# adolliou/euispice_coreg

Measured on AMD Instinct MI355X. Metric: lag-points/sec (whole node) on 2048² grid, 60×60 CRVAL sweep; argmax-shift match, higher is better.
Workload: dtype f64; 1 GPU; headline: Carrington 'fa' 2048x2048 grid lon(200,300) lat(-20,20), 60x60 CRVAL lags arange(-30,30,1) arcsec, small 2048^2 HRIEUV-like, ref 3072^2 FSI-like, order 2, solar_r 1.004; lag_points=3600, parallelism=single GPU, no collective, resident=True, sweeps_in_flight=2, small_stored_f32=True, use_lds=True

## Files before the change

### euispice_coreg_amd/_lib.py

```python
from __future__ import annotations

import ctypes as C
import os

import numpy as np

_HERE = os.path.dirname(os.path.abspath(__file__))
LIB_PATH = os.environ.get("COREG_HIP_LIB", os.path.join(_HERE, "libcoreg_hip.so"))

COREG_OK = 0
COREG_EINVAL, COREG_EHIP, COREG_ESTATE, COREG_ENOTIMPL, COREG_ENOMEM = -1, -2, -3, -4, -5
COREG_F32, COREG_F64 = 0, 1
PROJ_TAN, PROJ_CAR = 0, 1
METHOD_CORRELATION, METHOD_RESIDUS = 0, 1
CDELT_INTENDED, CDELT_REFERENCE = 0, 1


class CoregError(RuntimeError):
    def __init__(self, code, msg):
        super().__init__(f"libcoreg_hip error {code}: {msg}")
        self.code = code


class Wcs2d(C.Structure):
# ... 20 lines not shown
                ("lat0", C.c_double), ("lat1", C.c_double), ("n_lat", C.c_int32),
                ("lat_cos", C.POINTER(C.c_float)), ("lat_sin", C.POINTER(C.c_float))]


class Stats(C.Structure):
    _fields_ = [("sweep_kernel_ms", C.c_double), ("precompute_ms", C.c_double), ("total_gpu_ms", C.c_double),
                ("n_lags", C.c_int64), ("n_grid_points", C.c_int64), ("n_active_points", C.c_int64),
                ("n_sweep_launches", C.c_int64), ("small_is_f32", C.c_int32), ("used_lds", C.c_int32)]


class FitsPixels(C.Structure):
    _fields_ = [("data", C.c_void_p), ("bitpix", C.c_int32), ("reserved", C.c_int32), ("bscale", C.c_double),
                ("bzero", C.c_double)]


class FitsTiled(C.Structure):
    _fields_ = [("heap", C.c_void_p), ("heap_bytes", C.c_int64), ("tile_offset", C.c_void_p), ("tile_nbytes", C.c_void_p),
                ("n_tiles", C.c_int32), ("zbitpix", C.c_int32), ("naxis1", C.c_int32), ("naxis2", C.c_int32),
                ("ztile1", C.c_int32), ("ztile2", C.c_int32), ("blocksize", C.c_int32), ("bytepix", C.c_int32),
                ("quantize", C.c_int32), ("dither0", C.c_int32), ("has_blank", C.c_int32), ("blank", C.c_int32),
                ("zscale", C.c_void_p), ("zzero", C.c_void_p), ("zscale0", C.c_double), ("zzero0", C.c_double),
                ("bscale", C.c_double), ("bzero", C.c_double)]


def _is_tiled(img):
    return hasattr(img, "tile_nbytes") and hasattr(img, "ztile") and getattr(img, "on_gpu", False)


def _fits_tiled(ci):
    off = np.ascontiguousarray(ci.tile_offset, dtype=np.int64)
    nb = np.ascontiguousarray(ci.tile_nbytes, dtype=np.int32)
    keep = [off, nb, ci._heap]
    zs = zz = None
    if ci.zscale is not None and ci.zzero is not None:
        zs = np.ascontiguousarray(ci.zscale, dtype=np.float64)
        zz = np.ascontiguousarray(ci.zzero, dtype=np.float64)
        keep += [zs, zz]
    t = FitsTiled(ci._heap.ctypes.data, int(ci._heap.size), off.ctypes.data, nb.ctypes.data, int(ci.n_tiles), int(ci.zbitpix),
                  int(ci.shape[1]), int(ci.shape[0]), int(ci.ztile[0]), int(ci.ztile[1]), int(ci.blocksize), int(ci.bytepix),
                  int(ci.quantize), int(ci.dither0), int(bool(ci.has_blank)), int(ci.blank),
                  zs.ctypes.data if zs is not None else None, zz.ctypes.data if zz is not None else None,
                  float(ci.zscale0), float(ci.zzero0), float(ci.bscale), float(ci.bzero))
    return t, keep


def decode_tiled_host(ci, out):
    t, keep = _fits_tiled(ci)
    status = np.zeros(ci.n_tiles, dtype=np.int32)
    rc = load_library().coreg_decode_tiled_host(C.byref(t), out.ctypes.data, COREG_F32 if out.dtype == np.float32 else COREG_F64,
                                                status.ctypes.data)
    if rc != COREG_OK:
        raise CoregError(rc, "coreg_decode_tiled_host: bad arguments (unsupported tiling / codec parameters)")
    del keep
    return status


def encode_tiled_host(pixels, tile, bytepix=4, blocksize=32, quantize=0, dither0=1, scale=1.0):
    a = np.ascontiguousarray(pixels)
    if a.ndim != 2:
        raise ValueError("image must be 2-D")
    ny, nx = a.shape
    tx, ty = int(tile[0]), int(tile[1])
    nt = (-(-nx // tx)) * (-(-ny // ty))
    if a.dtype == np.float32:
        dt = COREG_F32
    elif a.dtype == np.float64:
        dt = COREG_F64
    elif a.dtype == np.int32:
        dt = 2
    else:
        raise TypeError("pixels must be float32, float64 or int32 (stored integers)")
    is_float = dt != 2
    n_blocks = nt * (-(-(tx * ty) // int(blocksize)) + 1)
    cap = a.size * int(bytepix) + n_blocks + 8 * nt + 64
    heap = np.empty(cap, dtype=np.uint8)
    nbytes = np.zeros(nt, dtype=np.int32)
    offs = np.zeros(nt, dtype=np.int64)
    zs = np.zeros(nt, dtype=np.float64) if is_float else None
    zz = np.zeros(nt, dtype=np.float64) if is_float else None
    used = C.c_longlong(0)
    rc = load_library().coreg_encode_tiled_host(a.ctypes.data, dt, ny, nx, tx, ty, int(bytepix), int(blocksize), int(quantize),
                                                int(dither0), float(scale), heap.ctypes.data, cap, nbytes.ctypes.data,
                                                offs.ctypes.data, zs.ctypes.data if is_float else None,
                                                zz.ctypes.data if is_float else None, C.byref(used))
    if rc != COREG_OK:
        raise CoregError(rc, "coreg_encode_tiled_host: bad arguments, or a tile's range does not fit 32-bit integers at "
                             "this scale")
    return heap[:used.value].copy(), nbytes, offs, zs, zz


def _is_raw(img):
    return hasattr(img, "bitpix") and hasattr(img, "ptr")


def _fits_pixels(raw) -> FitsPixels:
    if len(raw.shape) != 2:
        raise ValueError("image must be 2-D")
    return FitsPixels(raw.ptr, int(raw.bitpix), 0, float(raw.bscale), float(raw.bzero))


_P = C.c_void_p
_WP = C.POINTER(Wcs2d)
SYMBOLS = [
    ("coreg_version", C.c_char_p, []),
    ("coreg_create", C.c_int, [C.POINTER(_P), C.c_int]),
    ("coreg_destroy", None, [_P]),
    ("coreg_last_error", C.c_char_p, [_P]),
    ("coreg_set_stream", C.c_int, [_P, _P]),
    ("coreg_synchronize", C.c_int, [_P]),
    ("coreg_set_small", C.c_int, [_P, _P, C.c_int32, C.c_int32]),
    ("coreg_set_small_f32", C.c_int, [_P, _P, C.c_int32, C.c_int32]),
    ("coreg_set_small_fits", C.c_int, [_P, C.POINTER(FitsPixels), C.c_int32, C.c_int32]),
    ("coreg_prepare_reference_carrington_fits", C.c_int,
     [_P, C.POINTER(FitsPixels), C.c_int32, C.c_int32, _WP, C.POINTER(CarrGrid), C.c_double, C.c_int]),
    ("coreg_prepare_reference_helioprojective_fits", C.c_int,
     [_P, C.POINTER(FitsPixels), C.c_int32, C.c_int32, _WP, _WP, C.c_int]),
    ("coreg_set_small_tiled", C.c_int, [_P, C.POINTER(FitsTiled)]),
    ("coreg_prepare_reference_carrington_tiled", C.c_int,
     [_P, C.POINTER(FitsTiled), _WP, C.POINTER(CarrGrid), C.c_double, C.c_int]),
    ("coreg_prepare_reference_helioprojective_tiled", C.c_int, [_P, C.POINTER(FitsTiled), _WP, _WP, C.c_int]),
    ("coreg_decode_tiled_host", C.c_int, [C.POINTER(FitsTiled), _P, C.c_int, _P]),
    ("coreg_encode_tiled_host", C.c_int, [_P, C.c_int, C.c_int, C.c_int, C.c_int, C.c_int, C.c_int, C.c_int, C.c_int, C.c_int,
                                          C.c_double, _P, C.c_longlong, _P, _P, _P, _P, C.POINTER(C.c_longlong)]),
    ("coreg_threshold_small", C.c_int, [_P, C.c_int, C.c_double, C.c_int, C.c_double, C.POINTER(C.c_longlong)]),
    ("coreg_set_reference_on_grid", C.c_int, [_P, _P, C.c_int, C.c_int32, C.c_int32]),
    ("coreg_prepare_reference_carrington", C.c_int,
     [_P, _P, C.c_int32, C.c_int32, _WP, C.POINTER(CarrGrid), C.c_double, C.c_int]),
    ("coreg_prepare_reference_helioprojective", C.c_int, [_P, _P, C.c_int32, C.c_int32, _WP, _WP, C.c_int]),
    ("coreg_prepare_reference_carrington_f32", C.c_int,
     [_P, _P, C.c_int32, C.c_int32, _WP, C.POINTER(CarrGrid), C.c_double, C.c_int]),
    ("coreg_prepare_reference_helioprojective_f32", C.c_int, [_P, _P, C.c_int32, C.c_int32, _WP, _WP, C.c_int]),
    ("coreg_set_small_from_device", C.c_int, [_P, _P, C.c_int, C.c_int32, C.c_int32]),
    ("coreg_prepare_reference_carrington_from_device", C.c_int,
     [_P, _P, C.c_int, C.c_int32, C.c_int32, _WP, C.POINTER(CarrGrid), C.c_double, C.c_int]),
    ("coreg_prepare_reference_helioprojective_from_device", C.c_int,
     [_P, _P, C.c_int, C.c_int32, C.c_int32, _WP, _WP, C.c_int]),
    ("coreg_get_reference_on_grid", C.c_int, [_P, _P, C.c_int]),
    ("coreg_resample_carrington", C.c_int, [_P, _WP, C.POINTER(CarrGrid), C.c_double, C.c_int, _P]),
    ("coreg_resample_helioprojective", C.c_int, [_P, _WP, _WP, C.c_int, _P]),
    ("coreg_resample_helioprojective_f64", C.c_int, [_P, _WP, _WP, C.c_int, _P]),
    ("coreg_sweep_carrington", C.c_int,
     [_P, _WP, C.POINTER(CarrGrid), C.c_double, C.POINTER(Lags), C.c_int, C.c_int, C.c_int, C.c_int64, C.c_int64, _P,
      C.c_int]),
    ("coreg_sweep_helioprojective", C.c_int,
     [_P, _WP, _WP, C.POINTER(Lags), C.c_int, C.c_int, C.c_int, C.c_int64, C.c_int64, _P, C.c_int]),
    ("coreg_sums_size", C.c_int, [_P, C.POINTER(C.c_int64)]),
    ("coreg_copy_sums", C.c_int, [_P, _P, C.c_int]),
    ("coreg_finalize_sums", C.c_int, [_P, _P, C.c_int, _P, C.c_int]),
    ("coreg_get_pivots", C.c_int, [_P, C.POINTER(C.c_double)]),
    ("coreg_set_pivots", C.c_int, [_P, C.POINTER(C.c_double)]),
    ("coreg_last_stats", C.c_int, [_P, C.POINTER(Stats)]),
    ("coreg_last_visit_counts", C.c_int, [_P, C.POINTER(C.c_int64)]),
    ("coreg_last_tap_fix", C.c_int, [_P, C.POINTER(C.c_int64)]),
    ("coreg_set_option", C.c_int, [_P, C.c_char_p, C.c_int64]),
    ("coreg_shift_header", C.c_int,
     [_WP, C.c_double, C.c_double, C.c_double, C.c_double, C.c_double, C.c_int, _WP]),
    ("coreg_homography", C.c_int, [_WP, _WP, C.POINTER(C.c_double)]),
    ("coreg_lag_homography", C.c_int,
     [_WP, _WP, C.POINTER(Lags), C.POINTER(C.c_int32), C.c_int, C.POINTER(C.c_double)]),
    ("coreg_carrington_origin", C.c_int, [_WP, C.POINTER(C.c_double), C.POINTER(C.c_double)]),
    ("coreg_car_map", C.c_int, [_WP, _WP, C.c_int64, _P, _P, _P, _P]),
    ("coreg_wcslib_pixel_to_pixel", C.c_int, [_WP, _WP, C.c_int64, _P, _P, _P, _P, _P, _P]),
    ("coreg_car_tile_margin", C.c_int, [_WP, _WP, C.c_int32, C.c_double, C.POINTER(C.c_double)]),
    ("coreg_nansum_planes_be", C.c_int, [_P, C.c_int32, C.c_int64, _P, C.c_int32, _P]),
    ("coreg_fit_gaussian2d", C.c_int,
     [C.c_int32, _P, _P, _P, _P, _P, _P, C.c_int32, C.c_double, C.c_double, C.c_double, C.c_int32, _P,
      C.POINTER(C.c_int32), C.POINTER(C.c_int32)]),
    ("coreg_set_context_frames", C.c_int, [_P, C.c_int32, C.c_int32, C.c_int32, C.c_int, _WP, C.POINTER(_P)]),
    ("coreg_context_frame_from_small", C.c_int, [_P, C.c_int32]),
    ("coreg_sweep_context", C.c_int,
     [_P, _WP, _WP, C.POINTER(C.c_int32), C.POINTER(Lags), C.c_int, C.c_int, C.c_int, C.c_int, C.c_double, C.c_int,
      C.c_double, C.c_int64, C.c_int64, _P, C.c_int]),
    ("coreg_context_lag_headers", C.c_int,
     [_WP, _WP, C.c_double, C.c_double, C.c_double, C.c_double, C.c_double, C.c_int, _WP, _WP, _WP]),
    ("coreg_device_count", C.c_int, []),
    ("coreg_physical_device_count", C.c_int, []),
    ("coreg_multi_create", C.c_int, [C.POINTER(_P), C.c_int, C.POINTER(C.c_int)]),
    ("coreg_multi_destroy", None, [_P]),
    ("coreg_multi_size", C.c_int, [_P]),
    ("coreg_multi_handle", _P, [_P, C.c_int]),
    ("coreg_multi_last_error", C.c_char_p, [_P]),
    ("coreg_multi_collective", C.c_char_p, [_P]),
    ("coreg_multi_rccl_status", C.c_char_p, [_P]),
    ("coreg_multi_last_mode", C.c_int, [_P]),
    ("coreg_multi_set_option", C.c_int, [_P, C.c_char_p, C.c_int64]),
    ("coreg_multi_set_small", C.c_int, [_P, _P, C.c_int, C.c_int32, C.c_int32]),
    ("coreg_multi_set_small_fits", C.c_int, [_P, C.POINTER(FitsPixels), C.c_int32, C.c_int32]),
    ("coreg_multi_prepare_reference_carrington_fits", C.c_int,
     [_P, C.POINTER(FitsPixels), C.c_int32, C.c_int32, _WP, C.POINTER(CarrGrid), C.c_double, C.c_int]),
    ("coreg_multi_prepare_reference_helioprojective_fits", C.c_int,
     [_P, C.POINTER(FitsPixels), C.c_int32, C.c_int32, _WP, _WP, C.c_int]),
    ("coreg_multi_set_small_tiled", C.c_int, [_P, C.POINTER(FitsTiled)]),
    ("coreg_multi_prepare_reference_carrington_tiled", C.c_int,
     [_P, C.POINTER(FitsTiled), _WP, C.POINTER(CarrGrid), C.c_double, C.c_int]),
    ("coreg_multi_prepare_reference_helioprojective_tiled", C.c_int, [_P, C.POINTER(FitsTiled), _WP, _WP, C.c_int]),
    ("coreg_multi_threshold_small", C.c_int, [_P, C.c_int, C.c_double, C.c_int, C.c_double, C.POINTER(C.c_longlong)]),
    ("coreg_multi_set_reference_on_grid", C.c_int, [_P, _P, C.c_int, C.c_int32, C.c_int32]),
    ("coreg_multi_prepare_reference_carrington", C.c_int,
     [_P, _P, C.c_int, C.c_int32, C.c_int32, _WP, C.POINTER(CarrGrid), C.c_double, C.c_int]),
    ("coreg_multi_prepare_reference_helioprojective", C.c_int, [_P, _P, C.c_int, C.c_int32, C.c_int32, _WP, _WP, C.c_int]),
    ("coreg_multi_sweep_carrington", C.c_int,
     [_P, _WP, C.POINTER(CarrGrid), C.c_double, C.POINTER(Lags), C.c_int, C.c_int, C.c_int, _P]),
    ("coreg_multi_sweep_helioprojective", C.c_int, [_P, _WP, _WP, C.POINTER(Lags), C.c_int, C.c_int, C.c_int, _P]),
    ("coreg_multi_last_stats", C.c_int, [_P, C.c_int, C.POINTER(Stats)]),
    ("coreg_multi_plan", C.c_int,
     [C.c_int32, C.c_int32, C.c_int64, C.c_int32, C.c_int32, C.POINTER(C.c_int32), C.POINTER(C.c_int32),
      C.POINTER(C.c_int32), C.POINTER(C.c_int32)]),
]

_lib = None


def _preload_torch_hip_runtime():
    import importlib.util
    import sys
    if "torch" in sys.modules or os.environ.get("COREG_NO_TORCH_PRELOAD", "0") == "1":
        return
    try:
        spec = importlib.util.find_spec("torch")
    except (ImportError, ValueError):
        return
    if spec is None or not spec.submodule_search_locations:
        return
    libdir = os.path.join(list(spec.submodule_search_locations)[0], "lib")
    cand = os.path.join(libdir, "libamdhip64.so")
    if os.path.exists(cand):
        try:
            C.CDLL(cand, mode=C.RTLD_GLOBAL)
        except OSError:
            return
        rccl = os.path.join(libdir, "librccl.so")
        if os.path.exists(rccl):
            os.environ.setdefault("COREG_RCCL_LIB", rccl)


def load_library():
    global _lib
    if _lib is not None:
        return _lib
    _preload_torch_hip_runtime()
    if not os.path.exists(LIB_PATH):
        raise ImportError(
            f"{LIB_PATH} not found: the HIP extension has not been built. "
            "Run `python -c 'import __graft_entry__ as g; g.build()'` at the repo root "
            "(hipcc --offload-arch=gfx950). There is no CPU fallback.")
    lib = C.CDLL(LIB_PATH)
    for name, restype, argtypes in SYMBOLS:
        fn = getattr(lib, name)
        fn.restype = restype
        fn.argtypes = argtypes
    _lib = lib
    return lib


_UNIT_TO_DEG = {"deg": 1.0, "arcsec": 1.0 / 3600.0, "arcmin": 1.0 / 60.0, "rad": 180.0 / np.pi, "mas": 1.0 / 3.6e6}


def unit_to_deg(unit) -> float:
    u = str(unit).strip()
    if u not in _UNIT_TO_DEG:
        raise ValueError(f"unsupported CUNIT {unit!r}")
    return _UNIT_TO_DEG[u]


def wcs_from_header(hdr, carrington=False) -> Wcs2d:
    w = Wcs2d()
    if "ZNAXIS1" in hdr:
        w.naxis1, w.naxis2 = int(hdr["ZNAXIS1"]), int(hdr["ZNAXIS2"])
    else:
        w.naxis1, w.naxis2 = int(hdr.get("NAXIS1", 0)), int(hdr.get("NAXIS2", 0))
    w.crpix1, w.crpix2 = float(hdr["CRPIX1"]), float(hdr["CRPIX2"])
    w.crval1, w.crval2 = float(hdr["CRVAL1"]), float(hdr["CRVAL2"])
    w.cdelt1, w.cdelt2 = float(hdr["CDELT1"]), float(hdr["CDELT2"])
    w.pc1_1, w.pc1_2 = float(hdr.get("PC1_1", 1.0)), float(hdr.get("PC1_2", 0.0))
    w.pc2_1, w.pc2_2 = float(hdr.get("PC2_1", 0.0)), float(hdr.get("PC2_2", 1.0))
    w.crota = float(hdr["CROTA"] if "CROTA" in hdr else hdr.get("CROTA2", 0.0))
    u1 = hdr.get("CUNIT1", "deg")
    if str(u1).strip() != str(hdr.get("CUNIT2", u1)).strip():
        raise ValueError("CUNIT1 and CUNIT2 must be equal")
    w.unit_to_deg = unit_to_deg(u1)
    if str(hdr.get("CTYPE1", "")).strip().upper().endswith("-CAR"):
        w.proj = PROJ_CAR
        w.lonpole = float(hdr["LONPOLE"]) if "LONPOLE" in hdr else float("nan")
    else:
        w.proj = PROJ_TAN
        w.lonpole = float(hdr.get("LONPOLE", 180.0))
    w.latpole = float(hdr["LATPOLE"]) if "LATPOLE" in hdr else float("nan")
    if carrington:
        w.dsun_obs = float(hdr["DSUN_OBS"])
        w.crln_obs = float(hdr["CRLN_OBS"])
        w.crlt_obs = float(hdr["CRLT_OBS"])
    return w


def _dptr(a):
    return a.ctypes.data_as(C.POINTER(C.c_double))


class LagSet:

    def __init__(self, crval1, crval2, cdelt1, cdelt2, crota):
        def arr(v):
            return np.ascontiguousarray(np.atleast_1d(np.asarray([0.0] if v is None else v, dtype=np.float64)))

        self.arrays = [arr(crval1), arr(crval2), arr(cdelt1), arr(cdelt2), arr(crota)]
        a = self.arrays
# ... 176 lines not shown

    def get_reference_on_grid(self, shape, dtype):
        out = np.empty(shape, dtype=dtype)
        dt = COREG_F32 if out.dtype == np.float32 else COREG_F64
        self._chk(self._lib.coreg_get_reference_on_grid(self._h, out.ctypes.data, dt))
        return out

    def resample_carrington(self, hdr, grid: Grid, solar_r, order=2):
        w = wcs_from_header(hdr, carrington=True)
        out = np.empty((grid.n_lat, grid.n_lon), dtype=np.float64)
        self._chk(self._lib.coreg_resample_carrington(self._h, C.byref(w), C.byref(grid.c), float(solar_r), int(order),
                                                      out.ctypes.data))
        return out

    def resample_helioprojective(self, hdr_target, hdr, order=2, dtype=np.float32):
        wt, w = wcs_from_header(hdr_target), wcs_from_header(hdr)
        out = np.empty((wt.naxis2, wt.naxis1), dtype=dtype)
        fn = self._lib.coreg_resample_helioprojective if out.dtype == np.float32 else \
            self._lib.coreg_resample_helioprojective_f64
        self._chk(fn(self._h, C.byref(wt), C.byref(w), int(order), out.ctypes.data))
        return out

    def sweep_carrington(self, hdr_small, grid: Grid, solar_r, lags: LagSet, order=2, method=METHOD_CORRELATION,
                         cdelt_semantics=CDELT_INTENDED, lag_begin=0, lag_end=None, out_dev_ptr=None):
        lag_end = lags.size if lag_end is None else int(lag_end)
        w = wcs_from_header(hdr_small, carrington=True)
        if out_dev_ptr is None:
            out = np.empty(lag_end - lag_begin, dtype=np.float64)
            ptr, on_dev = out.ctypes.data, 0
        else:
            out, ptr, on_dev = None, int(out_dev_ptr), 1
        self._chk(self._lib.coreg_sweep_carrington(self._h, C.byref(w), C.byref(grid.c), float(solar_r),
                                                   C.byref(lags.c), int(order), int(method), int(cdelt_semantics),
                                                   int(lag_begin), lag_end, _P(ptr), on_dev))
        return out

    def sweep_helioprojective(self, hdr_target, hdr_small, lags: LagSet, order=2, method=METHOD_CORRELATION,
                              cdelt_semantics=CDELT_INTENDED, lag_begin=0, lag_end=None, out_dev_ptr=None):
        lag_end = lags.size if lag_end is None else int(lag_end)
        wt, w = wcs_from_header(hdr_target), wcs_from_header(hdr_small)
        if out_dev_ptr is None:
            out = np.empty(lag_end - lag_begin, dtype=np.float64)
            ptr, on_dev = out.ctypes.data, 0
        else:
            out, ptr, on_dev = None, int(out_dev_ptr), 1
        self._chk(self._lib.coreg_sweep_helioprojective(self._h, C.byref(wt), C.byref(w), C.byref(lags.c), int(order),
                                                        int(method), int(cdelt_semantics), int(lag_begin), lag_end,
                                                        _P(ptr), on_dev))
        return out

    def set_context_frames(self, frames, headers, dtype=None):
        frames = list(frames)
        if len(frames) != len(headers) or not frames:
            raise ValueError("one header per frame, at least one frame")

        def stored(f):
            if _is_tiled(f):
                return np.float32 if int(f.zbitpix) == -32 else np.float64
            if _is_raw(f):
                return np.float32 if int(f.bitpix) == -32 else np.float64
            return np.float32 if np.asarray(f).dtype == np.float32 else np.float64
        if dtype is None:
            dtype = np.float32 if all(stored(f) == np.float32 for f in frames) else np.float64
        dtype = np.dtype(dtype)
        shape = tuple(frames[0].shape)
        if any(tuple(f.shape) != shape for f in frames) or len(shape) != 2:
            raise ValueError("all frames must be 2-D images of one shape")
        hdrs = (Wcs2d * len(frames))(*[wcs_from_header(hh) for hh in headers])
        host = []
        ptrs = (_P * len(frames))()
        for k, f in enumerate(frames):
            if _is_tiled(f) or _is_raw(f):
                continue
            a = np.ascontiguousarray(f, dtype=dtype)
            host.append(a)
            ptrs[k] = a.ctypes.data
        self._chk(self._lib.coreg_set_context_frames(self._h, len(frames), shape[0], shape[1],
                                                     COREG_F32 if dtype == np.float32 else COREG_F64, hdrs, ptrs))
        for k, f in enumerate(frames):
            if _is_tiled(f) or _is_raw(f):
                self.set_small(f)
                self._chk(self._lib.coreg_context_frame_from_small(self._h, k))
        self._context_frames = (len(frames), shape, dtype)

    def sweep_context(self, hdr_target, hdr_small, col_frame, lags: LagSet, order=2, method=METHOD_CORRELATION,
                      cdelt_semantics=CDELT_INTENDED, vmin=None, vmax=None, lag_begin=0, lag_end=None, out_dev_ptr=None):
        lag_end = lags.size if lag_end is None else int(lag_end)
        wt, w = wcs_from_header(hdr_target), wcs_from_header(hdr_small)
        cf = np.ascontiguousarray(col_frame, dtype=np.int32)
        if cf.size != w.naxis1:
            raise ValueError("col_frame needs one entry per raster column")
        if out_dev_ptr is None:
            out = np.empty(lag_end - lag_begin, dtype=np.float64)
            ptr, on_dev = out.ctypes.data, 0
        else:
            out, ptr, on_dev = None, int(out_dev_ptr), 1
        self._chk(self._lib.coreg_sweep_context(
            self._h, C.byref(wt), C.byref(w), cf.ctypes.data_as(C.POINTER(C.c_int32)), C.byref(lags.c), int(order),
            int(method), int(cdelt_semantics), int(vmin is not None), float(0.0 if vmin is None else vmin),
            int(vmax is not None), float(0.0 if vmax is None else vmax), int(lag_begin), lag_end, _P(ptr), on_dev))
        return out

    def set_point_shard(self, rank, world):
        self.set_option("shard_world", int(world))
        self.set_option("shard_rank", int(rank))

    def sums_size(self) -> int:
        n = C.c_int64(0)
        self._chk(self._lib.coreg_sums_size(self._h, C.byref(n)))
        return int(n.value)

    def copy_sums(self, dst_ptr=None):
        if dst_ptr is not None:
            self._chk(self._lib.coreg_copy_sums(self._h, _P(int(dst_ptr)), 1))
            return None
        out = np.empty(self.sums_size(), dtype=np.float64)
        self._chk(self._lib.coreg_copy_sums(self._h, out.ctypes.data, 0))
        return out

    def finalize_sums(self, sums, n_out, out_dev_ptr=None):
        if isinstance(sums, np.ndarray):
            sums = np.ascontiguousarray(sums, dtype=np.float64)
            sptr, s_dev = sums.ctypes.data, 0
        else:
            sptr, s_dev = int(sums), 1
        if out_dev_ptr is None:
            out = np.empty(int(n_out), dtype=np.float64)
            self._chk(self._lib.coreg_finalize_sums(self._h, _P(sptr), s_dev, out.ctypes.data, 0))
            return out
        self._chk(self._lib.coreg_finalize_sums(self._h, _P(sptr), s_dev, _P(int(out_dev_ptr)), 1))
        return None

    def get_pivots(self):
        p = (C.c_double * 2)()
        self._chk(self._lib.coreg_get_pivots(self._h, p))
        return float(p[0]), float(p[1])

    def set_pivots(self, pivot_ref, pivot_small):
        p = (C.c_double * 2)(float(pivot_ref), float(pivot_small))
        self._chk(self._lib.coreg_set_pivots(self._h, p))

    def last_stats(self) -> dict:
        s = Stats()
        self._chk(self._lib.coreg_last_stats(self._h, C.byref(s)))
        return {f: getattr(s, f) for f, _ in Stats._fields_}

    def last_visit_counts(self) -> dict:
        c = (C.c_int64 * 6)()
        self._chk(self._lib.coreg_last_visit_counts(self._h, c))
        return {"visits": c[0], "lds": c[1], "interior": c[2], "all_finite": c[3], "refined_lag_points": c[4],
                "flagged_not_refined": c[5]}


    def last_tap_fix(self) -> dict:
        c = (C.c_int64 * 3)()
        self._chk(self._lib.coreg_last_tap_fix(self._h, c))
        return {"samples": c[0], "lag_points": c[1], "overflow": bool(c[2])}


class _HandleView(CoregHandle):

    def __init__(self, lib, ptr):
        self._lib = lib
        self._h = _P(ptr)
        self.reference_tag = None

    def close(self):
        self._h = None


MULTI_MODES = {0: "none", 1: "blocks", 2: "slices", 3: "points", 4: "combos"}


def device_count() -> int:
    return max(0, int(load_library().coreg_device_count()))


def physical_device_count() -> int:
    return max(0, int(load_library().coreg_physical_device_count()))


def multi_plan(n_crval1, n_crval2, n_inner, world, per_combo_launch=True):
    mode, gc, g1, g2 = C.c_int32(), C.c_int32(), C.c_int32(), C.c_int32()
    rc = load_library().coreg_multi_plan(int(n_crval1), int(n_crval2), int(n_inner), int(world), int(per_combo_launch),
                                         C.byref(mode), C.byref(gc), C.byref(g1), C.byref(g2))
    if rc != COREG_OK:
        raise CoregError(rc, "coreg_multi_plan: bad arguments")
    return MULTI_MODES[mode.value], gc.value, g1.value, g2.value


class MultiHandle:

    def __init__(self, n_devices=0, device_ids=None):
        self._lib = load_library()
        self._m = _P()
        ids = None
        if device_ids is not None:
            ids = (C.c_int * len(device_ids))(*[int(d) for d in device_ids])
            n_devices = len(device_ids)
        rc = self._lib.coreg_multi_create(C.byref(self._m), int(n_devices), ids)
        if rc != COREG_OK:
            self._m = None
            raise CoregError(rc, "coreg_multi_create failed (no HIP device visible?)")
        self.reference_tag = None
        self.size = int(self._lib.coreg_multi_size(self._m))
        self.primary = _HandleView(self._lib, self._lib.coreg_multi_handle(self._m, 0))

    def close(self):
        if getattr(self, "_m", None):
            self.primary.close()
            self._lib.coreg_multi_destroy(self._m)
            self._m = None

    def __del__(self):
        try:
            self.close()
        except Exception:
            pass

    def __enter__(self):
        return self

    def __exit__(self, *exc):
        self.close()

    def _chk(self, rc):
        if rc != COREG_OK:
            raise CoregError(rc, self._lib.coreg_multi_last_error(self._m).decode("utf-8", "replace"))

    @property
    def collective(self) -> str:
        return self._lib.coreg_multi_collective(self._m).decode()

    @property
    def rccl_status(self) -> str:
        return self._lib.coreg_multi_rccl_status(self._m).decode()

    @property
    def last_mode(self) -> str:
        return MULTI_MODES[int(self._lib.coreg_multi_last_mode(self._m))]

    def handle(self, k) -> CoregHandle:
        ptr = self._lib.coreg_multi_handle(self._m, int(k))
        if not ptr:
            raise IndexError(k)
        return _HandleView(self._lib, ptr)

    def set_option(self, name, value):
        self._chk(self._lib.coreg_multi_set_option(self._m, name.encode(), int(value)))

    def synchronize(self):
        for k in range(self.size):
            self.handle(k).synchronize()

    @staticmethod
    def _pixels(img):
        img = np.asarray(img)
        if img.ndim != 2:
            raise ValueError("image must be 2-D")
        if img.dtype == np.float32:
            return np.ascontiguousarray(img), COREG_F32
        return np.ascontiguousarray(img, dtype=np.float64), COREG_F64

    def set_small(self, img):
        if _is_tiled(img):
            t, keep = _fits_tiled(img)
            self._chk(self._lib.coreg_multi_set_small_tiled(self._m, C.byref(t)))
            return
        if _is_raw(img):
            px = _fits_pixels(img)
            self._chk(self._lib.coreg_multi_set_small_fits(self._m, C.byref(px), img.shape[0], img.shape[1]))
            return
        img, dt = self._pixels(img)
        self._chk(self._lib.coreg_multi_set_small(self._m, img.ctypes.data, dt, img.shape[0], img.shape[1]))

    def threshold_small(self, vmin=None, vmax=None) -> int:
        n = C.c_longlong(0)
        self._chk(self._lib.coreg_multi_threshold_small(self._m, int(vmin is not None), float(vmin or 0.0),
                                                        int(vmax is not None), float(vmax or 0.0), C.byref(n)))
        return int(n.value)

    def set_reference_on_grid(self, ref):
        ref = np.ascontiguousarray(ref)
        if ref.ndim != 2 or ref.dtype not in (np.float32, np.float64):
            raise ValueError("reference on grid must be a 2-D float32/float64 array")
        self.reference_tag = None
        self._chk(self._lib.coreg_multi_set_reference_on_grid(
            self._m, ref.ctypes.data, COREG_F32 if ref.dtype == np.float32 else COREG_F64, ref.shape[0], ref.shape[1]))

    def prepare_reference_carrington(self, large, hdr_large, grid: Grid, solar_r, order=2):
        w = wcs_from_header(hdr_large, carrington=True)
        self.reference_tag = None
        if _is_tiled(large):
            t, keep = _fits_tiled(large)
            self._chk(self._lib.coreg_multi_prepare_reference_carrington_tiled(self._m, C.byref(t), C.byref(w),
                                                                               C.byref(grid.c), float(solar_r), int(order)))
            return
        if _is_raw(large):
            px = _fits_pixels(large)
            self._chk(self._lib.coreg_multi_prepare_reference_carrington_fits(
                self._m, C.byref(px), large.shape[0], large.shape[1], C.byref(w), C.byref(grid.c), float(solar_r),
                int(order)))
            return
        large, dt = self._pixels(large)
        self._chk(self._lib.coreg_multi_prepare_reference_carrington(
            self._m, large.ctypes.data, dt, large.shape[0], large.shape[1], C.byref(w), C.byref(grid.c), float(solar_r),
# ... 234 lines not shown
```

### euispice_coreg_amd/csrc/abi_host.hpp

```cpp
#pragma once
extern "C" {
int coreg_shift_header(const coreg_wcs2d* ref, double d_crval1, double d_crval2, double d_cdelt1, double d_cdelt2,
                       double d_crota, int cdelt_semantics, coreg_wcs2d* out) {
    if (!ref || !out) return COREG_EINVAL;
    return shift_header(*ref, d_crval1, d_crval2, d_cdelt1, d_cdelt2, d_crota, cdelt_semantics, out);
}

int coreg_car_map(const coreg_wcs2d* from, const coreg_wcs2d* to, int64_t n, const double* px, const double* py,
                  double* ox, double* oy) {
    if (!from || !to || n < 0 || (n > 0 && (!px || !py || !ox || !oy))) return COREG_EINVAL;
    if (from->proj != COREG_PROJ_CAR || to->proj != COREG_PROJ_CAR) return COREG_EINVAL;
    CarMapHost m;
    if (m.init(*from, *to)) return 1;
    for (int64_t i = 0; i < n; ++i) m.apply(px[i], py[i], &ox[i], &oy[i]);
    return COREG_OK;
}

int coreg_last_visit_counts(coreg_handle* h, int64_t* counts6) {
    int64_t* counts5 = counts6;
    if (!h || !counts5) return COREG_EINVAL;
    RETCHK(bind_device(h));
    HIPCHK(hipStreamSynchronize(h->stream));
    long long info[8] = {0, 0, 0, 0, 0, 0, 0, 0};
    if (h->tile_info.p) HIPCHK(hipMemcpy(info, h->tile_info.p, 7 * sizeof(long long), hipMemcpyDeviceToHost));
    for (int k = 0; k < 4; ++k) counts5[k] = info[3 + k];
    long long refined[2] = {0, 0};
    if (h->counters.p) HIPCHK(hipMemcpy(refined, h->counters.p, sizeof(refined), hipMemcpyDeviceToHost));
    counts5[4] = refined[0];
    counts6[5] = refined[1];
    return COREG_OK;
}

int coreg_last_tap_fix(coreg_handle* h, int64_t* counts3) {
    if (!h || !counts3) return COREG_EINVAL;
    for (int k = 0; k < 3; ++k) counts3[k] = h->tap_last[k];
    return COREG_OK;
}

int coreg_car_tile_margin(const coreg_wcs2d* hdr_target, const coreg_wcs2d* hdr_shifted, int32_t tile_w,
                          double tile_abs_lat_rad, double* margin_px) {
    if (!hdr_target || !hdr_shifted || !margin_px || tile_w < 1 || tile_w > kTilePts) return COREG_EINVAL;
    if (hdr_target->proj != COREG_PROJ_CAR || hdr_shifted->proj != COREG_PROJ_CAR) return COREG_EINVAL;
    CarMapHost m;
    if (m.init(*hdr_target, *hdr_shifted)) return 1;
    *margin_px = car_tile_margin(car_box_c(*hdr_target, *hdr_shifted, tile_w), tile_abs_lat_rad + car_pole_sep(m.r));
    return COREG_OK;
}

int coreg_homography(const coreg_wcs2d* from, const coreg_wcs2d* to, double* h9) {
    if (!from || !to || !h9) return COREG_EINVAL;
    if (from->proj != COREG_PROJ_TAN || to->proj != COREG_PROJ_TAN) return COREG_ENOTIMPL;
    homography(*from, *to, h9);
    return COREG_OK;
}

int coreg_lag_homography(const coreg_wcs2d* hdr_target, const coreg_wcs2d* hdr_small, const coreg_lags* lags,
                         const int32_t idx[5], int cdelt_semantics, double* h9) {
    if (!hdr_target || !hdr_small || !lags || !idx || !h9) return COREG_EINVAL;
    if (hdr_target->proj != COREG_PROJ_TAN || hdr_small->proj != COREG_PROJ_TAN) return COREG_ENOTIMPL;
    if (idx[0] < 0 || idx[0] >= lags->n_crval1 || idx[1] < 0 || idx[1] >= lags->n_crval2 || idx[2] < 0 ||
        idx[2] >= lags->n_cdelt1 || idx[3] < 0 || idx[3] >= lags->n_cdelt2 || idx[4] < 0 || idx[4] >= lags->n_crota)
        return COREG_EINVAL;
    coreg_wcs2d hc;
    if (shift_header(*hdr_small, 0.0, 0.0, lags->cdelt1[idx[2]], lags->cdelt2[idx[3]], lags->crota[idx[4]],
                     cdelt_semantics, &hc))
        return 1;
    HomographyFamily fam;
    fam.init(*hdr_target, *hdr_small, lags->crval1, lags->n_crval1, lags->crval2, lags->n_crval2);
    fam.get(HomographyFamily::combo(hc), idx[0], idx[1], h9);
    return COREG_OK;
}

int coreg_wcslib_pixel_to_pixel(const coreg_wcs2d* from, const coreg_wcs2d* to, int64_t n, const double* px,
                                const double* py, double* ox, double* oy, double* lng, double* lat) {
    if (!from || !to || n < 0 || (n > 0 && (!px || !py || !ox || !oy))) return COREG_EINVAL;
    if (from->proj == COREG_PROJ_CAR && to->proj == COREG_PROJ_CAR) {
        WcslibCar a, b;
        a.init(*from);
        b.init(*to);
        if (!a.valid || !b.valid) return COREG_EINVAL;
        for (int64_t i = 0; i < n; ++i) {
            double l, t;
            a.p2s(px[i], py[i], &l, &t);
            if (lng) lng[i] = l;
            if (lat) lat[i] = t;
            b.s2p(l, t, &ox[i], &oy[i]);
        }
        return COREG_OK;
    }
    if (from->proj != COREG_PROJ_TAN || to->proj != COREG_PROJ_TAN) return COREG_ENOTIMPL;
    WcslibTan a, b;
    a.init(*from);
    b.init(*to);
    for (int64_t i = 0; i < n; ++i) {
        double l, t;
        a.p2s(px[i], py[i], &l, &t);
        if (lng) lng[i] = l;
        if (lat) lat[i] = t;
        b.s2p(ang2pipi_deg(l), ang2pipi_deg(t), &ox[i], &oy[i]);
    }
    return COREG_OK;
}

int coreg_carrington_origin(const coreg_wcs2d* hdr, double* x0, double* y0) {
    if (!hdr || !x0 || !y0) return COREG_EINVAL;
    carr_origin(*hdr, x0, y0);
    return COREG_OK;
}

int coreg_nansum_planes_be(const void* cube, int32_t bitpix, int64_t n_pixels, const int64_t* plane_index, int32_t n_sel,
                           double* out) {
    if (!cube || !out || n_pixels < 0 || n_sel < 0 || (n_sel > 0 && !plane_index) || (bitpix != -32 && bitpix != -64))
        return COREG_EINVAL;
    for (int k = 0; k < n_sel; ++k)
        if (plane_index[k] < 0) return COREG_EINVAL;
    auto work = [&](int64_t lo, int64_t hi) {
        for (int64_t p = lo; p < hi; ++p) out[p] = 0.0;
        for (int k = 0; k < n_sel; ++k) {
            if (bitpix == -32) {
                const uint32_t* src = (const uint32_t*)cube + (size_t)plane_index[k] * (size_t)n_pixels;
                for (int64_t p = lo; p < hi; ++p) {
                    const uint32_t u = __builtin_bswap32(src[p]);
                    float f;
                    std::memcpy(&f, &u, sizeof(f));
                    const double v = (double)f;
                    out[p] += (v != v) ? 0.0 : v;
                }
            } else {
                const uint64_t* src = (const uint64_t*)cube + (size_t)plane_index[k] * (size_t)n_pixels;
                for (int64_t p = lo; p < hi; ++p) {
                    const uint64_t u = __builtin_bswap64(src[p]);
                    double v;
                    std::memcpy(&v, &u, sizeof(v));
                    out[p] += (v != v) ? 0.0 : v;
                }
            }
        }
    };
    parallel_for(n_pixels, (unsigned)std::min<int64_t>(12, n_pixels * std::max(n_sel, 1) / (1 << 18)), 0, work);
    return COREG_OK;
}

int coreg_fit_gaussian2d(int32_t m, const double* x, const double* y, const double* z, const double* p0,
                         const double* lb, const double* ub, int32_t jac, double ftol, double xtol, double gtol,
                         int32_t max_nfev, double* popt, int32_t* nfev, int32_t* status) {
    if (!x || !y || !z || !p0 || !lb || !ub || !popt || !status || m < 1 || m > coregfit::MMAX) return COREG_EINVAL;
    coregfit::Problem P{m, x, y, z};
    int n = 0;
    const int st = coregfit::fit(P, p0, lb, ub, jac != 0, ftol > 0 ? ftol : 1e-8, xtol > 0 ? xtol : 1e-8,
                                 gtol > 0 ? gtol : 1e-8, max_nfev, popt, &n, nullptr);
    if (st == -2) return COREG_EINVAL;
    if (nfev) *nfev = n;
    *status = st;
    return COREG_OK;
}

}
```

### euispice_coreg_amd/csrc/abi_sweeps.hpp

```cpp
#pragma once
namespace {
struct SweepCall {
    const coreg_lags* lags = nullptr;
    LagDims d;
    int order = 0, method = 0, sem = 0;
    long long lag_begin = 0, lag_end = 0, n_out = 0;
    double* corr_out = nullptr;
    int out_on_device = 0;
    double* out_dev = nullptr;
    long long row() const { return (long long)d.n2 * d.nc; }
    int i1_lo() const { return (int)(lag_begin / row()); }
    int i1_hi() const { return (int)((lag_end - 1) / row()); }
};

template <typename OwnChecks>
int open_sweep(coreg_handle* h, ComboRange combo, OwnChecks own_checks, const coreg_lags* lags, int order, int method,
               int sem, int64_t lag_begin, int64_t lag_end, int grid_w, int grid_h, const char* grid_what,
               double* corr_out, int out_on_device, SweepCall* call) {
    if (method != COREG_METHOD_CORRELATION && method != COREG_METHOD_RESIDUS)
        return fail(h, COREG_ENOTIMPL, "method must be COREG_METHOD_CORRELATION or COREG_METHOD_RESIDUS");
    RETCHK(check_order(h, order));
    RETCHK(own_checks());
    RETCHK(check_lags(h, lags, &call->d, lag_begin, lag_end, combo));
    RETCHK(bind_device_nowait(h));
    if (h->ref.p && (h->gW != grid_w || h->gH != grid_h))
        return fail(h, COREG_EINVAL, std::string("reference-on-grid shape differs from ") + grid_what);
    call->lags = lags;
    call->order = order;
    call->method = method;
    call->sem = sem;
    call->lag_begin = lag_begin;
    call->lag_end = lag_end;
    call->n_out = lag_end - lag_begin;
    call->corr_out = corr_out;
    call->out_on_device = out_on_device;
    return begin_sweep(h, call->n_out, corr_out, out_on_device, &call->out_dev);
}

int close_sweep(coreg_handle* h, const SweepCall& call) {
    return end_sweep(h, call.n_out, call.corr_out, call.out_on_device, call.out_dev);
}

int close_empty_sweep(coreg_handle* h, const SweepCall& call) {
    RETCHK(fill_nan(h, call.out_dev, call.n_out));
    return close_sweep(h, call);
}

template <typename MapAt>
Geometry local_geometry(const coreg_wcs2d& target, const SweepCall& call, MapAt at) {
    const coreg_lags& l = *call.lags;
    int e1[3], e2[3];
    extreme_lags(l.crval1, call.d.n1, e1);
    extreme_lags(l.crval2, call.d.n2, e2);
    const double v1 = l.crval1[e1[1]], v2 = l.crval2[e2[1]];
    const double s1 = lag_step(l.crval1, call.d.n1), s2 = lag_step(l.crval2, call.d.n2);
    const double u = target.naxis1 * 0.5, v = target.naxis2 * 0.5;
    double x0, y0, xi, yi, xj, yj, xa, ya, xb, yb;
    Geometry g;
    if (!at(v1, v2, u, v, &x0, &y0) || !at(v1, v2, u + 1, v, &xi, &yi) || !at(v1, v2, u, v + 1, &xj, &yj) ||
        !at(v1 + s1, v2, u, v, &xa, &ya) || !at(v1, v2 + s2, u, v, &xb, &yb))
        return g;
    g.dx_di = xi - x0;
    g.dy_di = yi - y0;
    g.dx_dj = xj - x0;
    g.dy_dj = yj - y0;
    g.ax = xa - x0;
    g.ay = ya - y0;
    g.bx = xb - x0;
    g.by = yb - y0;
    return g;
}

Plan plan_sweep(coreg_handle* h, const Geometry& geo, const SweepCall& call) {
    return choose_plan(h, geo, call.i1_hi() - call.i1_lo() + 1, call.d.n2, h->opt_use_lds ? lds_window_elems(h) : (1LL << 40));
}

bool combo_slots(const SweepCall& call, const coreg_wcs2d& small, const Plan& plan, long long c, coreg_wcs2d* hc,
                 SlotList* slots) {
    const long long first = (call.lag_begin - c + call.d.nc - 1) / call.d.nc;
    if (first * call.d.nc + c >= call.lag_end) return false;
    int i3, i4, i5;
    call.d.inner(c, &i3, &i4, &i5);
    if (shift_header(small, 0.0, 0.0, call.lags->cdelt1[i3], call.lags->cdelt2[i4], call.lags->crota[i5], call.sem, hc))
        return false;
    build_slots(call.d, c, call.lag_begin, call.lag_end, plan.sw, plan.sh, slots);
    return slots->n_batches > 0;
}

template <int MODE>
int precompute(coreg_handle* h, const PrecomputeArgs& pa, int n_tiles, int n_groups, int n_batches, bool launch = true) {
    if (launch) RETCHK(launch_precompute<MODE>(h, pa, n_tiles, n_groups, n_batches));
    h->last_precompute = [pa, n_tiles, n_groups, n_batches](coreg_handle* hh) {
        return launch_precompute<MODE>(hh, pa, n_tiles, n_groups, n_batches);
    };
    return COREG_OK;
}

int finalize_pending(coreg_handle* h, const coreg_handle::PendingFinalize& pf, long long* refine_count, double* out_dev,
                     FinalizeArgs* f) {
    *f = FinalizeArgs{};
    RETCHK(fill_refine(h, &f->refine, pf.refine.mode, pf.refine.order, pf.refine.lane_params, pf.refine.car_inv,
                       pf.n_slots));
    f->refine.enabled = pf.refine.enabled;
    f->refine_count = refine_count;
    f->partials = h->sums.as<double>() + pf.slot_off;
    f->n_groups = 1;
    f->n_slots = pf.n_slots;
    f->part_stride = h->sums_slots;
    f->out_index = h->fin_outidx.as<long long>() + pf.slot_off;
    f->lag_begin = pf.lag_begin;
    f->out = out_dev;
    f->residus = pf.residus;
    f->n_required = (long long)h->gW * h->gH;
    hipLaunchKernelGGL(k_finalize, dim3((unsigned)((pf.n_slots + kFinSlots - 1) / kFinSlots)),
                       dim3(kFinSlots * kFinLanes), 0, h->stream, *f);
    return COREG_OK;
}
}

extern "C" {
int coreg_sweep_carrington(coreg_handle* h, const coreg_wcs2d* hdr_small, const coreg_carr_grid* grid, double solar_r,
                           const coreg_lags* lags, int order, int method, int cdelt_semantics, int64_t lag_begin,
                           int64_t lag_end, double* corr_out, int out_on_device) {
    if (!h) return COREG_EINVAL;
    const ComboRange combo = take_combo_range(h);
    trace("sweep_carrington: enter");
    if (!hdr_small || !grid) return fail(h, COREG_EINVAL, "sweep_carrington: null header/grid");
    auto own_checks = [&] {
        RETCHK(check_wcs(h, hdr_small, true));
        RETCHK(check_grid(h, grid));
        if (!std::isfinite(solar_r) || !(solar_r > 0.0)) return fail(h, COREG_EINVAL, "solar_r must be positive");
        return COREG_OK;
    };
    SweepCall call;
    RETCHK(open_sweep(h, combo, own_checks, lags, order, method, cdelt_semantics, lag_begin, lag_end, grid->n_lon,
                      grid->n_lat, "the Carrington grid", corr_out, out_on_device, &call));
    if (call.n_out == 0) return close_sweep(h, call);
    const LagDims& d = call.d;

    CarrDev cd;
    std::memset(&cd, 0, sizeof(cd));
    RETCHK(upload_carr_tables(h, *grid, *hdr_small, &cd));

    Geometry geo;
    {
        const CarrCommon c0 = carr_common(*hdr_small, solar_r);
        const int ic = grid->n_lon / 2, jc = grid->n_lat / 2;
        double a0, a1, b0, b1, c0x, c0y;
        carr_term_host(h->tabs, c0, ic, jc, &a0, &a1);
        carr_term_host(h->tabs, c0, std::min(ic + 1, grid->n_lon - 1), jc, &b0, &b1);
        carr_term_host(h->tabs, c0, ic, std::min(jc + 1, grid->n_lat - 1), &c0x, &c0y);
        geo.dx_di = b0 - a0;
        geo.dy_di = b1 - a1;
        geo.dx_dj = c0x - a0;
        geo.dy_dj = c0y - a1;
        const double s1 = lag_step(lags->crval1, d.n1), s2 = lag_step(lags->crval2, d.n2);
        geo.ax = c0.cr * s1 / hdr_small->cdelt1;
        geo.ay = c0.sr * s1 / hdr_small->cdelt2;
        geo.bx = c0.sr * s2 / hdr_small->cdelt1;
        geo.by = c0.cr * s2 / hdr_small->cdelt2;
    }
    const Plan plan = plan_sweep(h, geo, call);
    PrecomputeArgs pa;
    int n_tiles;
    RETCHK(setup_precompute(h, plan, method, &pa, &n_tiles));

    struct Launch {
        size_t slot_off;
        int n_batches;
        CarrCommon cc;
        double f0lo, f0hi, f1lo, f1hi;
    };
    std::vector<Launch> launches;
    std::vector<double> params;
    std::vector<long long> outidx;
    SlotList slots;
    for (long long c = 0; c < d.nc; ++c) {
        coreg_wcs2d hc;
        if (!combo_slots(call, *hdr_small, plan, c, &hc, &slots)) continue;
        const size_t ns = slots.i1.size();
        Launch L;
        L.slot_off = outidx.size();
        L.n_batches = slots.n_batches;
        L.cc = carr_common(hc, solar_r);
        const size_t pbase = params.size();
        params.resize(pbase + 2 * ns);
        double x0min = 1e300, x0max = -1e300, y0min = 1e300, y0max = -1e300;
        const double roll = hc.crota * kDeg2Rad;
        const double rc = std::cos(roll), rs = std::sin(roll);
        const double nan = std::numeric_limits<double>::quiet_NaN();
        for (size_t s = 0; s < ns; ++s) {
            if (slots.outidx[s] < 0) {
                params[pbase + s] = nan;
                params[pbase + ns + s] = nan;
                continue;
            }
            const double v1 = hdr_small->crval1 + lags->crval1[slots.i1[s]];
            const double v2 = hdr_small->crval2 + lags->crval2[slots.i2[s]];
            const double dx = rc * v1 + rs * v2;
            const double dy = -rs * v1 + rc * v2;
            const double x0 = (hc.crpix1 - 1) - dx / hc.cdelt1;
            const double y0 = (hc.crpix2 - 1) - dy / hc.cdelt2;
            params[pbase + s] = x0;
            params[pbase + ns + s] = y0;
            x0min = std::min(x0min, x0);
            x0max = std::max(x0max, x0);
            y0min = std::min(y0min, y0);
            y0max = std::max(y0max, y0);
        }
        outidx.insert(outidx.end(), slots.outidx.begin(), slots.outidx.end());
        L.f0lo = -x0max;
        L.f0hi = (double)(h->sW - 1) - x0min;
        L.f1lo = -y0max;
        L.f1hi = (double)(h->sH - 1) - y0min;
        launches.push_back(L);
    }
    if (launches.empty()) return close_empty_sweep(h, call);
    RETCHK(upload_plan(h, params, outidx, call.out_dev, call.n_out));
    RETCHK(prepare_sharded(h, outidx.size(), call.n_out, lag_begin));
    for (const Launch& L : launches) {
        set_carr_common(&cd, L.cc);
        pa.carr = cd;
        pa.f0lo = L.f0lo;
        pa.f0hi = L.f0hi;
        pa.f1lo = L.f1lo;
        pa.f1hi = L.f1hi;
        {
            const double dm1 = L.cc.dist - 1.0;
            pa.tile_skip = (h->opt_tile_skip && dm1 > 0.0) ? 1 : 0;
            const double per_rad = pa.tile_skip ? (1.0 / dm1 + 1.0 / (dm1 * dm1)) * kRad2Deg * 3600.0 : 0.0;
            pa.lip_x = per_rad / std::fabs(L.cc.cdelt1) * (1.0 + 1e-9);
            pa.lip_y = per_rad / std::fabs(L.cc.cdelt2) * (1.0 + 1e-9);
            pa.dlon = grid->n_lon > 1 ? (std::fabs(grid->lon1 - grid->lon0) / (grid->n_lon - 1) * 1.001 + 1e-4) * kDeg2Rad : 0.0;
            pa.dlat = grid->n_lat > 1 ? (std::fabs(grid->lat1 - grid->lat0) / (grid->n_lat - 1) * 1.001 + 1e-4) * kDeg2Rad : 0.0;
        }
        RETCHK(precompute<MODE_TRANSLATE>(h, pa, n_tiles, pick_groups(h, L.n_batches, n_tiles), L.n_batches));
        RETCHK(launch_sweep(h, MODE_TRANSLATE, order, method, h->lane_params.as<double>() + 2 * L.slot_off,
                            h->out_index.as<long long>() + L.slot_off, L.n_batches, n_tiles, lag_begin, call.out_dev,
// ... 521 lines not shown
```

### euispice_coreg_amd/csrc/host_plan.hpp

```cpp
#pragma once
namespace {
template <typename Fn>
void parallel_for(long long n, unsigned max_threads, long long grain, Fn fn) {
    if (n <= 0) return;
    const long long nt_max = std::max<long long>(1, std::min(max_threads, std::thread::hardware_concurrency()));
    if (grain <= 0) grain = (n + nt_max - 1) / nt_max;
    const long long nt = std::min(nt_max, (n + grain - 1) / grain);
    if (nt <= 1) {
        fn(0ll, n);
        return;
    }
    std::atomic<long long> next(0);
    auto worker = [&] {
        for (long long lo = next.fetch_add(grain); lo < n; lo = next.fetch_add(grain)) fn(lo, std::min(n, lo + grain));
    };
    std::vector<std::thread> th;
    for (long long t = 1; t < nt; ++t) th.emplace_back(worker);
    worker();
    for (auto& x : th) x.join();
}

struct LagDims {
    int n1, n2, n3, n4, n5;
    long long nc;
    long long c0;
    long long total() const { return (long long)n1 * n2 * nc; }
    void inner(long long c, int* i3, int* i4, int* i5) const {
        const long long g = c + c0;
        *i5 = (int)(g % n5);
        *i4 = (int)((g / n5) % n4);
        *i3 = (int)(g / ((long long)n5 * n4));
    }
};

struct ComboRange {
    long long begin = 0, end = 0;
};
ComboRange take_combo_range(coreg_handle* h) {
    ComboRange r;
    r.begin = h->opt_combo_begin;
    r.end = h->opt_combo_end;
    h->opt_combo_begin = h->opt_combo_end = 0;
    return r;
}
int check_lags(coreg_handle* h, const coreg_lags* l, LagDims* d, int64_t begin, int64_t end, ComboRange combo = ComboRange()) {
    if (!l || !l->crval1 || !l->crval2 || !l->cdelt1 || !l->cdelt2 || !l->crota)
        return fail(h, COREG_EINVAL, "lags: null array");
    if (l->n_crval1 < 1 || l->n_crval2 < 1 || l->n_cdelt1 < 1 || l->n_cdelt2 < 1 || l->n_crota < 1)
        return fail(h, COREG_EINVAL, "lags: every axis needs at least one value");
    d->n1 = l->n_crval1;
    d->n2 = l->n_crval2;
    d->n3 = l->n_cdelt1;
    d->n4 = l->n_cdelt2;
    d->n5 = l->n_crota;
    d->nc = (long long)d->n3 * d->n4 * d->n5;
    d->c0 = 0;
    {
        const long long cb = combo.begin, ce = combo.end;
        if (cb != 0 || ce != 0) {
            if (cb < 0 || ce <= cb || ce > d->nc)
                return fail(h, COREG_EINVAL, "combo_begin/combo_end outside [0, n_cdelt1 * n_cdelt2 * n_crota]");
            d->c0 = cb;
            d->nc = ce - cb;
        }
    }
    if (begin < 0 || end > d->total() || begin > end)
        return fail(h, COREG_EINVAL, "lag_begin/lag_end outside [0, n_lags]");
    const double* ax[5] = {l->crval1, l->crval2, l->cdelt1, l->cdelt2, l->crota};
    const int32_t na[5] = {l->n_crval1, l->n_crval2, l->n_cdelt1, l->n_cdelt2, l->n_crota};
    for (int k = 0; k < 5; ++k)
        for (int32_t i = 0; i < na[k]; ++i)
            if (!std::isfinite(ax[k][i])) return fail(h, COREG_EINVAL, "lags: a non-finite value");
    return COREG_OK;
}

static int check_wcs(coreg_handle* h, const coreg_wcs2d* w, bool carrington_transform) {
    const char* why = wcs_problem(*w, carrington_transform);
    return why ? fail(h, COREG_EINVAL, why) : COREG_OK;
}
static bool too_many(long long a, long long b) { return a * b > 2147483647ll; }
static int check_grid(coreg_handle* h, const coreg_carr_grid* g) {
    if (g->n_lon >= 1 && g->n_lat >= 1 && too_many(g->n_lon, g->n_lat))
        return fail(h, COREG_EINVAL, "Carrington grid: more than 2^31 - 1 points");
    const char* why = grid_problem(*g);
    return why ? fail(h, COREG_EINVAL, why) : COREG_OK;
}

struct Geometry {
    double dx_di = 1, dx_dj = 0, dy_di = 0, dy_dj = 1;
    double ax = 0, ay = 0, bx = 0, by = 0;
};
struct Plan {
    int tile_w = 32;
    int sw = 16, sh = 16;
    double window = 0;
    double win_w = 0, win_h = 0;
};

Plan choose_plan(coreg_handle* h, const Geometry& g, int m1, int n2, long long lds_elems) {
    Plan best, fallback;
    double best_cost = std::numeric_limits<double>::max(), fb_win = std::numeric_limits<double>::max();
    const int sw_hi = h->opt_patch_w > 0 ? std::min<int>((int)h->opt_patch_w, kBlock) : kBlock;
    for (int tw = 4; tw <= 256; tw *= 2) {
        if (h->opt_tile_w > 0 && tw != h->opt_tile_w) continue;
        const int th = kTilePts / tw;
        if (th < 1) continue;
        const double tex = tw * std::fabs(g.dx_di) + th * std::fabs(g.dx_dj);
        const double tey = tw * std::fabs(g.dy_di) + th * std::fabs(g.dy_dj);
        for (int sw = 1; sw <= std::min(m1, sw_hi); ++sw) {
            int sh = std::min(n2, kBlock / sw);
            if (sh < 1) break;
            const int cols = (m1 + sw - 1) / sw, rows = (n2 + sh - 1) / sh;
            sh = (n2 + rows - 1) / rows;
            const int sw2 = (m1 + cols - 1) / cols;
            const double ex = tex + sw2 * std::fabs(g.ax) + sh * std::fabs(g.bx) + 6.0;
            const double ey = tey + sw2 * std::fabs(g.ay) + sh * std::fabs(g.by) + 6.0;
            const double win = (ex + 1.0) * ey;
            if (win < fb_win) {
                fb_win = win;
                fallback.tile_w = tw;
                fallback.sw = sw2;
                fallback.sh = sh;
                fallback.window = win;
                fallback.win_w = ex + 1.0;
                fallback.win_h = ey;
            }
            if (win > 0.94 * (double)lds_elems) continue;
            const double cost = (double)cols * rows * (1.0 + 0.08 * win / (double)lds_elems);
            if (cost < best_cost) {
                best_cost = cost;
                best.tile_w = tw;
                best.sw = sw2;
                best.sh = sh;
                best.window = win;
                best.win_w = ex + 1.0;
                best.win_h = ey;
            }
        }
    }
    const Plan& r = best_cost < std::numeric_limits<double>::max() ? best : fallback;
    if (std::getenv("COREG_DEBUG_PLAN"))
        std::fprintf(stderr, "[coreg plan] tile %d x %d, lag patch %d x %d, window estimate %.0f (%.1f x %.1f) of %lld elements; "
                     "geometry d/di (%.3f, %.3f) d/dj (%.3f, %.3f) lag1 (%.3f, %.3f) lag2 (%.3f, %.3f)\n", r.tile_w,
                     kTilePts / r.tile_w, r.sw, r.sh, r.window, r.win_w, r.win_h, lds_elems, g.dx_di, g.dy_di, g.dx_dj, g.dy_dj, g.ax, g.ay,
                     g.bx, g.by);
    return r;
}

void extreme_lags(const double* v, int n, int out[3]) {
    int lo = 0, hi = 0;
    for (int i = 1; i < n; ++i) {
        if (v[i] < v[lo] || v[lo] != v[lo]) lo = i;
        if (v[i] > v[hi] || v[hi] != v[hi]) hi = i;
    }
    const double mid = 0.5 * (v[lo] + v[hi]);
    int m = lo;
    for (int i = 0; i < n; ++i)
        if (std::fabs(v[i] - mid) < std::fabs(v[m] - mid)) m = i;
    out[0] = lo;
    out[1] = m;
    out[2] = hi;
}

double lag_step(const double* v, int n) {
    if (n < 2) return 0.0;
    double lo = v[0], hi = v[0];
    for (int i = 1; i < n; ++i) {
        lo = std::min(lo, v[i]);
        hi = std::max(hi, v[i]);
    }
    return (hi - lo) / (double)(n - 1);
}

struct SlotList {
    std::vector<int> i1, i2;
    std::vector<long long> outidx;
    int n_batches = 0;
};

void build_slots(const LagDims& d, long long c, long long begin, long long end, int sw, int sh, SlotList* s) {
    s->i1.clear();
    s->i2.clear();
    s->outidx.clear();
    s->n_batches = 0;
    {
        const size_t cap = (size_t)((d.n1 + sw - 1) / sw + 1) * ((d.n2 + sh - 1) / sh) * kBlock;
        s->i1.reserve(cap);
        s->i2.reserve(cap);
        s->outidx.reserve(cap);
    }
    const long long row = (long long)d.n2 * d.nc;
    const int i1_lo = (int)(begin / row);
    const int i1_hi = (int)((end - 1) / row);
    const int m1 = i1_hi - i1_lo + 1;
    for (int p1 = 0; p1 * sw < m1; ++p1)
        for (int p2 = 0; p2 * sh < d.n2; ++p2) {
            bool any = false;
            const size_t at = s->i1.size();
            for (int t = 0; t < kBlock; ++t) {
                int lx = t % sw, ly = t / sw;
                bool valid = ly < sh;
                if (!valid) lx = ly = 0;
                int i1 = i1_lo + p1 * sw + lx, i2 = p2 * sh + ly;
                if (i1 > i1_hi) {
                    i1 = i1_hi;
                    valid = false;
                }
                if (i2 > d.n2 - 1) {
                    i2 = d.n2 - 1;
                    valid = false;
                }
                const long long idx = ((long long)i1 * d.n2 + i2) * d.nc + c;
                if (idx < begin || idx >= end) valid = false;
                s->i1.push_back(i1);
                s->i2.push_back(i2);
                s->outidx.push_back(valid ? idx : -1);
                any |= valid;
            }
            if (!any) {
                s->i1.resize(at);
                s->i2.resize(at);
                s->outidx.resize(at);
            } else {
                s->n_batches++;
            }
        }
}

int pick_groups(coreg_handle* h, int n_batches, int n_tiles) {
    if (h->opt_shard_world > 1) {
        const long long per_rank = 8 * std::max<long long>(1, std::llround(256.0 / (8.0 * n_batches)));
        return (int)std::min<long long>(per_rank * h->opt_shard_world, 1000 / (8 * h->opt_shard_world) * 8 * h->opt_shard_world);
    }
    long long g = h->opt_n_groups > 0 ? h->opt_n_groups : (4096 + n_batches - 1) / n_batches;
    (void)n_tiles;
    g = std::max<long long>(8, std::min<long long>(h->opt_n_groups > 0 ? 1000 : 256, ((g + 7) / 8) * 8));
    return (int)g;
}

void pick_taper(const coreg_handle* h, int n_groups, int n_batches, int* tmin, int* tfrac) {
    *tmin = (int)h->opt_taper_min;
    if (h->opt_taper_frac >= 0) {
        *tfrac = (int)h->opt_taper_frac;
        return;
    }
    const double rounds = (double)n_groups * n_batches / 256.0;
    *tfrac = (rounds >= (double)h->opt_taper_rounds && n_groups >= 128 && h->opt_shard_world <= 1) ? 512 : 0;
}

template <int MODE>
int launch_precompute(coreg_handle* h, const PrecomputeArgs& a, int n_tiles, int n_groups, int n_batches) {
    EventPair* ev = next_event(h, h->ev_pre, h->ev_pre_used);
    if (!ev) return fail(h, COREG_EHIP, "hipEventCreate failed");
    int tmin, tfrac;
    pick_taper(h, n_groups, n_batches, &tmin, &tfrac);
    PrecomputeArgs b = a;
    b.prologue = h->pending_prologue;
    const bool with_prologue = b.prologue.src != nullptr;
    std::memset(&h->pending_prologue, 0, sizeof(h->pending_prologue));
    HIPCHK(hipEventRecord(ev->a, h->stream));
    if (h->ref_dtype == COREG_F32)
        hipLaunchKernelGGL((k_precompute<MODE, float>), dim3(n_tiles), dim3(256), 0, h->stream, b);
    else
        hipLaunchKernelGGL((k_precompute<MODE, double>), dim3(n_tiles), dim3(256), 0, h->stream, b);
    (void)with_prologue;
    hipLaunchKernelGGL(k_tile_list, dim3(1), dim3(1024), 0, h->stream, (const int*)a.tile_count, n_tiles, n_groups,
                       h->tile_list.as<int>(), h->tile_cum.as<int>(), h->group_first.as<int>(),
                       h->tile_info.as<long long>(), tmin, tfrac);
    ev->b_is_next_sweep = true;
    ev->next_sweep_index = h->ev_sweep_used;
    HIPCHK(hipGetLastError());
    return COREG_OK;
}

int reserve_tiles(coreg_handle* h, int n_tiles) {
    const size_t pts = (size_t)n_tiles * kTilePts + (size_t)(kPointGroups + 1) * kChunk;
    HIPCHK(h->pts.reserve(pts * sizeof(Pt)));
    HIPCHK(h->tile_count.reserve(n_tiles * sizeof(int)));
    HIPCHK(h->tile_list.reserve(n_tiles * sizeof(int)));
    HIPCHK(h->tile_cum.reserve((n_tiles + 1) * sizeof(int)));
    HIPCHK(h->group_first.reserve(2 * 1024 * sizeof(int) + 64));
    HIPCHK(h->tile_info.reserve(8 * sizeof(long long)));
    HIPCHK(h->tile_bbox.reserve((size_t)n_tiles * 4 * sizeof(double)));
    return COREG_OK;
}

int setup_precompute(coreg_handle* h, const Plan& plan, int method, PrecomputeArgs* a, int* n_tiles) {
    std::memset(a, 0, sizeof(*a));
    a->tile_w = plan.tile_w;
    a->tile_h = kTilePts / plan.tile_w;
    a->tiles_x = (h->gW + a->tile_w - 1) / a->tile_w;
    a->tiles_y = (h->gH + a->tile_h - 1) / a->tile_h;
    *n_tiles = a->tiles_x * a->tiles_y;
    RETCHK(reserve_tiles(h, *n_tiles));
    a->ref = h->ref.p;
    a->gw = h->gW;
    a->gh = h->gH;
    a->pivot_a = h->pivots.as<double>();
    a->pts = h->pts.as<Pt>();
    a->tile_count = h->tile_count.as<int>();
    a->tile_bbox = h->tile_bbox.as<double>();
    a->residus = method == COREG_METHOD_RESIDUS ? 1 : 0;
    return COREG_OK;
}

long long lds_window_elems(const coreg_handle* h);

int pick_pitch(const coreg_handle* h, const Plan& plan, long long lds_elems, int order = 2) {
    if (h->opt_pitch == 0 || !h->opt_use_lds) return 0;
    static const int kPitches[] = {89, 121, 153, 185, 217};
    if (h->opt_pitch > 0) {
        for (int p : kPitches)
            if (p == h->opt_pitch) return p;
        return 0;
    }
    for (int p : kPitches)
        if ((double)p >= plan.win_w + (order > 2 ? 4.0 : 2.0) &&
            (double)p * (plan.win_h + (order > 2 ? 2.0 : 0.0)) <= 0.985 * (double)lds_elems)
            return p;
    return 0;
}

}
```

### euispice_coreg_amd/csrc/host_state.hpp

```cpp
#pragma once
namespace {

struct DevBuf {
    void* p = nullptr;
    size_t cap = 0;
    hipError_t reserve(size_t bytes) {
        if (bytes <= cap) return hipSuccess;
        if (p) {
            hipError_t e = hipFree(p);
            if (e != hipSuccess) return e;
            p = nullptr;
            cap = 0;
        }
        const size_t want = bytes + bytes / 4 + 256;
        hipError_t e = hipMalloc(&p, want);
        if (e != hipSuccess) return e;
        cap = want;
        return hipSuccess;
    }
    void release() {
        if (p) (void)hipFree(p);
        p = nullptr;
        cap = 0;
    }
    template <typename T>
    T* as() const {
        return (T*)p;
    }
};

struct PinBuf {
    void* p = nullptr;
    size_t cap = 0;
    hipError_t reserve(size_t bytes) {
        if (bytes <= cap) return hipSuccess;
        if (p) (void)hipHostFree(p);
        p = nullptr;
        cap = 0;
        const size_t want = bytes + bytes / 2 + 4096;
        hipError_t e = hipHostMalloc(&p, want, hipHostMallocDefault);
        if (e != hipSuccess) return e;
        cap = want;
        return hipSuccess;
    }
    void release() {
        if (p) (void)hipHostFree(p);
        p = nullptr;
        cap = 0;
    }
};

enum SrcKind {
    SRC_HOST = 0,
    SRC_PINNED = 1,
    SRC_DEVICE = 2,
};

struct PixFmt {
    int bitpix = 0;
    bool f32 = false;
    double bscale = 1.0, bzero = 0.0;
    bool raw() const { return bitpix != 0; }
    bool scaled() const { return bscale != 1.0 || bzero != 0.0; }
    size_t elem() const { return raw() ? (size_t)(bitpix < 0 ? -bitpix : bitpix) / 8 : (f32 ? 4 : 8); }
    bool swap_only() const { return bitpix == -32 && !scaled(); }
    static PixFmt native(bool is_f32) {
        PixFmt f;
        f.f32 = is_f32;
        return f;
    }
};

constexpr int kMaxDevices = 64;
std::mutex g_attr_mutex;

struct EventPair {
    hipEvent_t a = nullptr, b = nullptr;
    bool b_is_next_sweep = false;
    size_t next_sweep_index = 0;
};

}

struct KeptTapLists {
    DevBuf all;
    ~KeptTapLists() { all.release(); }
};
struct FixLaunch {
    std::vector<BorderFixArgs> border;
    std::vector<ParityFixArgs> parity;
    TapFixArgs tap = {};
    bool have_tap = false;
    int tap_segs = 0, tap_mode = 0;
    long long tap_count = 0;
    std::shared_ptr<KeptTapLists> kept;
    bool small_f32 = true;
    bool empty() const { return border.empty() && parity.empty() && !have_tap; }
};

struct ContextState;

struct coreg_handle {
    int device = 0;
    hipStream_t stream = nullptr;
    bool own_stream = false;
    std::string err;

    ContextState* ctx = nullptr;

    DevBuf small;
    int sW = 0, sH = 0;
    bool small_f32 = false;
    DevBuf ref;
    int gW = 0, gH = 0;
    int ref_dtype = -1;
    DevBuf pivots, red_sum, red_cnt;
    DevBuf t_sin_lon, t_cos_lon, t_cos_lat, t_sin_lat;
    CarrTables tabs;
    std::vector<double> tabs_key;
    PinBuf pin_img[2];
    hipEvent_t ev_img[2] = {nullptr, nullptr};
    int pin_img_next = 0;
    DevBuf pts, tile_count, tile_list, tile_cum, group_first, tile_info, tile_bbox;
    DevBuf rf_fix_slab;
    DevBuf counters;
    DevBuf lane_params, out_index, partials, out_dev, tmp_img;
    DevBuf up_f64, up_flag;
    DevBuf up_raw;
    DevBuf rice_blob, rice_rand, dec_img;
    PrologueArgs pending_prologue = {};
    DevBuf bbox_buf;
    hipStream_t aux_stream = nullptr;
    hipStream_t up_stream = nullptr;
    hipEvent_t ev_small = nullptr, ev_main = nullptr;
    bool small_pending = false;
    DevBuf red_sum_up, red_cnt_up;
    int64_t opt_overlap_upload = 1;
    int64_t opt_tap_nan_filter = 2;
    int64_t opt_async_upload = 0;
    std::thread up_thread;
    std::mutex up_m;
    std::condition_variable up_cv;
    std::function<hipError_t()> up_job;
    bool up_has = false, up_stop = false, up_busy = false;
    hipError_t up_rc = hipSuccess;
    PinBuf pin_small[2];
    hipEvent_t ev_pin_small[2] = {nullptr, nullptr};
    int pin_small_next = 0;
    std::map<std::vector<double>, std::vector<int>> border_cache;
    std::map<std::vector<double>, std::vector<unsigned char>> flags_cache;
    DevBuf border_flags, fix_partial;
    DevBuf border_dev;
    PinBuf pin_border;
    int64_t opt_border_fix = 1;
    int64_t opt_tap_fix = 1, opt_tap_cap = 1 << 24;
    DevBuf tap_count, tap_segq, tap_list, tap_skip, tap_seg_slot, tap_seg_begin, tap_pixel, tap_xw, tap_yw;
    long long tap_last[3] = {0, 0, 0};
    int64_t opt_shard_world = 1, opt_shard_rank = 0;
    int64_t opt_combo_begin = 0, opt_combo_end = 0;
    DevBuf sums;
    long long sums_slots = 0;
    struct PendingFinalize {
        long long slot_off, n_slots, lag_begin;
        const long long* outidx_dev;
        int residus;
        RefineArgs refine;
        std::function<int(coreg_handle*)> replay_precompute;
        FixLaunch fixes;
    };
    std::function<int(coreg_handle*)> last_precompute;
    DevBuf rf_flags, rf_pivots, rf_list, rf_head, rf_partial;
    std::vector<PendingFinalize> pending_fin;
    DevBuf fin_outidx;
    long long pending_n_out = 0;

    int64_t opt_crop_reference = 1;
    int64_t opt_taper_min = 128, opt_taper_frac = -1, opt_taper_rounds = 6;
    int64_t opt_use_lds = 1, opt_clean_path = 1, opt_refine = 1, opt_refine_cond_log10 = 5, opt_tile_w = 0, opt_n_groups = 0, opt_lds_bytes = (159 * 1024 * kPointGroups) / 4, opt_patch_w = 0, opt_h_series = 1, opt_h_incr = 1, opt_tile_skip = 1, opt_pitch = -1;

    coreg_stats stats;
    bool stats_pending = false;
    PinBuf pin_info;
    std::vector<EventPair> ev_sweep, ev_pre;
    size_t ev_sweep_used = 0, ev_pre_used = 0;
    hipEvent_t ev_t1 = nullptr;
    hipEvent_t ev_end[2] = {nullptr, nullptr};
    PinBuf pin_plan[2];
    int plan_slot = 0;
    bool plan_open = false;
};
```

### euispice_coreg_amd/csrc/host_sweep_io.hpp

```cpp
#pragma once
namespace {
int collect_stats(coreg_handle* h);

void reset_stats(coreg_handle* h, long long n_grid_points, long long n_lags) {
    std::memset(&h->stats, 0, sizeof(h->stats));
    h->stats.small_is_f32 = h->small_f32 ? 1 : 0;
    h->stats.n_grid_points = n_grid_points;
    h->stats.n_lags = n_lags;
}

int begin_sweep(coreg_handle* h, long long n_out, double* corr_out, int out_on_device, double** out_dev) {
    h->stats_pending = false;
    h->pending_fin.clear();
    h->sums_slots = 0;
    h->pending_n_out = 0;
    h->tap_last[0] = h->tap_last[1] = h->tap_last[2] = 0;
    std::memset(&h->pending_prologue, 0, sizeof(h->pending_prologue));
    if (h->plan_open) {
        h->plan_open = false;
        RETCHK(bind_device(h));
        HIPCHK(hipStreamSynchronize(h->stream));
    }
    if (!h->small.p) return fail(h, COREG_ESTATE, "coreg_set_small has not been called");
    if (!h->ref.p) return fail(h, COREG_ESTATE, "no reference image on the target grid");
    if (!corr_out && n_out > 0) return fail(h, COREG_EINVAL, "corr_out is null");
    h->ev_sweep_used = 0;
    h->ev_pre_used = 0;
    reset_stats(h, (long long)h->gW * h->gH, n_out);
    if (out_on_device) {
        *out_dev = corr_out;
    } else {
        HIPCHK(h->out_dev.reserve((size_t)std::max<long long>(n_out, 1) * sizeof(double)));
        *out_dev = h->out_dev.as<double>();
    }
    return COREG_OK;
}

int fill_nan(coreg_handle* h, double* out_dev, long long n_out) {
    if (n_out > 0) {
        hipLaunchKernelGGL(k_fill, dim3((unsigned)((n_out + 255) / 256)), dim3(256), 0, h->stream, out_dev,
                           (long long)n_out, std::numeric_limits<double>::quiet_NaN());
        HIPCHK(hipGetLastError());
    }
    return COREG_OK;
}

int collect_stats(coreg_handle* h) {
    if (!h->stats_pending) return COREG_OK;
    HIPCHK(hipStreamSynchronize(h->stream));
    h->stats_pending = false;
    if (h->tile_info.p && h->stats.n_sweep_launches > 0) {
        long long info[3] = {0, 0, 0};
        HIPCHK(hipMemcpy(info, h->tile_info.p, sizeof(info), hipMemcpyDeviceToHost));
        h->stats.n_active_points = info[1];
    }
    float ms = 0.f;
    for (size_t i = 0; i < h->ev_sweep_used; ++i) {
        HIPCHK(hipEventElapsedTime(&ms, h->ev_sweep[i].a, h->ev_sweep[i].b));
        h->stats.sweep_kernel_ms += ms;
    }
    for (size_t i = 0; i < h->ev_pre_used; ++i) {
        const EventPair& e = h->ev_pre[i];
        if (e.b_is_next_sweep && e.next_sweep_index >= h->ev_sweep_used) continue;
        HIPCHK(hipEventElapsedTime(&ms, e.a, e.b_is_next_sweep ? h->ev_sweep[e.next_sweep_index].a : e.b));
        h->stats.precompute_ms += ms;
    }
    if (h->ev_pre_used > 0) {
        HIPCHK(hipEventElapsedTime(&ms, h->ev_pre[0].a, h->ev_t1));
        h->stats.total_gpu_ms = ms;
    }
    return COREG_OK;
}

int end_sweep(coreg_handle* h, long long n_out, double* corr_out, int out_on_device, double* out_dev) {
    h->ev_t1 = h->ev_end[h->plan_slot];
    HIPCHK(hipEventRecord(h->ev_t1, h->stream));
    h->plan_slot ^= 1;
    h->plan_open = false;
    if (!out_on_device && n_out > 0)
        HIPCHK(hipMemcpyAsync(corr_out, out_dev, (size_t)n_out * sizeof(double), hipMemcpyDeviceToHost, h->stream));
    h->stats_pending = true;
    trace("end_sweep: everything issued");
    if (!out_on_device) HIPCHK(hipStreamSynchronize(h->stream));
    trace("end_sweep: map on the host");
    return COREG_OK;
}

long long lds_window_elems(const coreg_handle* h) {
    const size_t lds_min = (size_t)(kPointGroups - 1) * kNumSums * kBlock * sizeof(double);
    return (long long)(std::max(lds_min, (size_t)h->opt_lds_bytes) / sizeof(double));
}

int upload_plan(coreg_handle* h, const std::vector<double>& params, const std::vector<long long>& outidx,
                double* out_dev, long long n_out) {
    const size_t bytes = params.size() * sizeof(double) + outidx.size() * sizeof(long long);
    HIPCHK(h->lane_params.reserve(params.size() * sizeof(double)));
    HIPCHK(h->out_index.reserve(outidx.size() * sizeof(long long)));
    PinBuf& pin = h->pin_plan[h->plan_slot];
    HIPCHK(hipEventSynchronize(h->ev_end[h->plan_slot]));
    h->plan_open = true;
    HIPCHK(pin.reserve(bytes));
    std::memcpy(pin.p, params.data(), params.size() * sizeof(double));
    std::memcpy((char*)pin.p + params.size() * sizeof(double), outidx.data(), outidx.size() * sizeof(long long));
    void* src_dev = nullptr;
    HIPCHK(hipHostGetDevicePointer(&src_dev, pin.p, 0));
    PrologueArgs& p = h->pending_prologue;
    p.src = (const double*)src_dev;
    p.dst_params = h->lane_params.as<double>();
    p.n_params = (long long)params.size();
    p.dst_outidx = h->out_index.as<long long>();
    p.n_outidx = (long long)outidx.size();
    p.out = out_dev;
    p.n_out = n_out;
    HIPCHK(h->counters.reserve(8 * sizeof(long long)));
    p.refine_count = h->counters.as<long long>();
    return COREG_OK;
}

int prepare_sharded(coreg_handle* h, size_t total_slots, long long n_out, long long lag_begin) {
    h->pending_fin.clear();
    h->sums_slots = 0;
    h->pending_n_out = n_out;
    (void)lag_begin;
    if (h->opt_shard_world <= 1) return COREG_OK;
    h->sums_slots = (long long)total_slots;
    HIPCHK(h->sums.reserve(std::max<size_t>(1, total_slots) * kNumSums * sizeof(double)));
    HIPCHK(h->fin_outidx.reserve(std::max<size_t>(1, total_slots) * sizeof(long long)));
    const PrologueArgs& pr = h->pending_prologue;
    if (!pr.src || (size_t)pr.n_outidx < total_slots) return fail(h, COREG_ESTATE, "prepare_sharded: no plan staged");
    HIPCHK(hipMemcpyAsync(h->fin_outidx.p, (const char*)h->pin_plan[h->plan_slot].p + (size_t)pr.n_params * sizeof(double),
                          total_slots * sizeof(long long), hipMemcpyHostToDevice, h->stream));
    return COREG_OK;
}

}
```

### euispice_coreg_amd/csrc/host_sweep_launch.hpp

```cpp
#pragma once
namespace {
int launch_sweep(coreg_handle* h, int mode, int order, int method, const double* params_dev,
                 const long long* outidx_dev, int n_batches, int n_tiles, long long lag_begin, double* out_dev,
                 const LaunchU* car_inv = nullptr, const BorderFix* fix = nullptr, long long sums_off = 0,
                 int pitch_sel = 0) {
    const long long n_slots = (long long)n_batches * kBlock;
    const int n_groups = pick_groups(h, n_batches, n_tiles);
    const bool sharded = h->opt_shard_world > 1;
    const int g_per = sharded ? n_groups / (int)h->opt_shard_world : n_groups;
    const int g_lo = sharded ? g_per * (int)h->opt_shard_rank : 0;
    const bool fixing = fix && (!fix->items.empty() || fix->tap_segs > 0) && (!sharded || h->opt_shard_rank == 0);
    HIPCHK(h->partials.reserve((size_t)(g_per + (fixing ? 1 : 0)) * kNumSums * n_slots * sizeof(double)));

    SweepArgs a;
    a.img = h->small.p;
    a.W = h->sW;
    a.H = h->sH;
    a.pts = h->pts.as<Pt>();
    a.tile_count = h->tile_count.as<int>();
    a.tile_list = h->tile_list.as<int>();
    a.tile_cum = h->tile_cum.as<int>();
    a.group_first = h->group_first.as<int>();
    a.tile_info = h->tile_info.as<long long>();
    a.tile_bbox = h->tile_bbox.as<double>();
    a.lane_params = params_dev;
    a.n_slots = n_slots;
    a.n_batches = n_batches;
    a.n_groups = n_groups;
    a.group_lo = g_lo;
    a.partials = h->partials.as<double>();
    a.pivots = h->pivots.as<double>();
    a.use_lds = h->opt_use_lds ? 1 : 0;
    a.clean_path = h->opt_clean_path ? 1 : 0;
    const size_t lds_min = (size_t)(kPointGroups - 1) * kNumSums * kBlock * sizeof(double);
    const size_t lds_bytes = std::max(lds_min, a.use_lds ? (size_t)h->opt_lds_bytes : 0);
    a.lds_elems = (int)(lds_bytes / sizeof(double));
    std::memset(&a.car_inv, 0, sizeof(a.car_inv));
    if (car_inv) a.car_inv = *car_inv;
    a.car_inv.order_rt = order;
    a.car_inv.h_incr = (int)h->opt_h_incr;

    const dim3 grid((unsigned)((long long)g_per * n_batches)), block(kSweepThreads);
    RETCHK(join_small(h));
    trace("launch_sweep: launching k_sweep");
    EventPair* ev = next_event(h, h->ev_sweep, h->ev_sweep_used);
    if (!ev) return fail(h, COREG_EHIP, "hipEventCreate failed");
#define SWP(M, O, TS, R, Q, P)                                                                                       \
    do {                                                                                                              \
        {                                                                                                             \
             \
             \
            static size_t attr_bytes[kMaxDevices] = {0};                                                              \
            std::lock_guard<std::mutex> lock(g_attr_mutex);                                                           \
            size_t& ab = attr_bytes[h->device % kMaxDevices];                                                         \
            if (lds_bytes > 48 * 1024 && lds_bytes > ab) {                                                            \
                HIPCHK(hipFuncSetAttribute((const void*)(k_sweep<M, O, TS, R, Q, P>),                                 \
                                           hipFuncAttributeMaxDynamicSharedMemorySize, (int)lds_bytes));              \
                ab = lds_bytes;                                                                                       \
            }                                                                                                         \
        }                                                                                                             \
        HIPCHK(hipEventRecord(ev->a, h->stream));                                                                     \
        hipLaunchKernelGGL((k_sweep<M, O, TS, R, Q, P>), grid, block, lds_bytes, h->stream, a);                       \
        HIPCHK(hipEventRecord(ev->b, h->stream));                                                                     \
    } while (0)
#define SW(M, O, TS, R, Q) SWP(M, O, TS, R, Q, 0)
#define SW_Q(M, O, TS, R)                                        \
    do {                                                         \
        if (method == COREG_METHOD_RESIDUS) SW(M, O, TS, R, true); \
        else SW(M, O, TS, R, false);                             \
    } while (0)
#define SW_T(M, O, R)                           \
    do {                                        \
        if (h->small_f32) SW_Q(M, O, float, R); \
        else SW_Q(M, O, double, R);             \
    } while (0)
    if (mode == MODE_TRANSLATE && order == 2 && h->small_f32 && method != COREG_METHOD_RESIDUS && pitch_sel > 0) {
        switch (pitch_sel) {
            case 89: SWP(MODE_TRANSLATE, 2, float, false, false, 89); break;
            case 121: SWP(MODE_TRANSLATE, 2, float, false, false, 121); break;
            case 153: SWP(MODE_TRANSLATE, 2, float, false, false, 153); break;
            case 185: SWP(MODE_TRANSLATE, 2, float, false, false, 185); break;
            case 217: SWP(MODE_TRANSLATE, 2, float, false, false, 217); break;
            default: SW(MODE_TRANSLATE, 2, float, false, false); break;
        }
    } else if (mode == MODE_TRANSLATE && order == 2 && !h->small_f32 && method != COREG_METHOD_RESIDUS &&
               (pitch_sel == 89 || pitch_sel == 121 || pitch_sel == 153)) {
        if (pitch_sel == 89) SWP(MODE_TRANSLATE, 2, double, false, false, 89);
        else if (pitch_sel == 121) SWP(MODE_TRANSLATE, 2, double, false, false, 121);
        else SWP(MODE_TRANSLATE, 2, double, false, false, 153);
    } else if ((mode == MODE_HOMOGRAPHY_SERIES || mode == MODE_HOMOGRAPHY) && order == 2 && h->small_f32 &&
               method != COREG_METHOD_RESIDUS && (pitch_sel == 89 || pitch_sel == 121)) {
        if (mode == MODE_HOMOGRAPHY_SERIES) {
            if (pitch_sel == 89) SWP(MODE_HOMOGRAPHY_SERIES, 2, float, true, false, 89);
            else SWP(MODE_HOMOGRAPHY_SERIES, 2, float, true, false, 121);
        } else {
            if (pitch_sel == 89) SWP(MODE_HOMOGRAPHY, 2, float, true, false, 89);
            else SWP(MODE_HOMOGRAPHY, 2, float, true, false, 121);
        }
    } else if (mode == MODE_TRANSLATE && order == 3 && h->small_f32 && method != COREG_METHOD_RESIDUS &&
               (pitch_sel == 89 || pitch_sel == 121 || pitch_sel == 153)) {
        if (pitch_sel == 89) SWP(MODE_TRANSLATE, 3, float, false, false, 89);
        else if (pitch_sel == 121) SWP(MODE_TRANSLATE, 3, float, false, false, 121);
        else SWP(MODE_TRANSLATE, 3, float, false, false, 153);
    } else if (mode == MODE_TRANSLATE) {
        if (order == 2) SW_T(MODE_TRANSLATE, 2, false);
        else if (order == 1) SW_T(MODE_TRANSLATE, 1, false);
        else if (order == 3) SW_T(MODE_TRANSLATE, 3, false);
        else SW_T(MODE_TRANSLATE, ORDER_RT, false);
    } else if (mode == MODE_CAR) {
        if (order == 2) SW_T(MODE_CAR, 2, true);
        else if (order == 1) SW_T(MODE_CAR, 1, true);
        else SW_T(MODE_CAR, ORDER_RT, true);
    } else if (mode == MODE_HOMOGRAPHY_SERIES && (order == 1 || order == 2 || order == 3)) {
        if (order == 2) SW_T(MODE_HOMOGRAPHY_SERIES, 2, true);
        else if (order == 3) SW_T(MODE_HOMOGRAPHY_SERIES, 3, true);
        else SW_T(MODE_HOMOGRAPHY_SERIES, 1, true);
    } else {
        if (order == 2) SW_T(MODE_HOMOGRAPHY, 2, true);
        else if (order == 1) SW_T(MODE_HOMOGRAPHY, 1, true);
        else if (order == 3) SW_T(MODE_HOMOGRAPHY, 3, true);
        else SW_T(MODE_HOMOGRAPHY, ORDER_RT, true);
    }
#undef SWP
#undef SW_Q
#undef SW_T
#undef SW
    HIPCHK(hipGetLastError());
    h->stats.n_sweep_launches++;
    h->stats.used_lds = a.use_lds;

    FixLaunch fl;
    fl.small_f32 = h->small_f32;
    if (fix && (!fix->items.empty() || fix->tap_segs > 0)) {
        BorderFixArgs b = {};
        b.img = h->small.p;
        b.W = h->sW;
        b.H = h->sH;
        b.ref = h->ref.p;
        b.ref_f32 = h->ref_dtype == COREG_F32 ? 1 : 0;
        b.gw = h->gW;
        b.order = order;
        b.round_f32 = mode == MODE_TRANSLATE ? 0 : 1;
        b.residus = method == COREG_METHOD_RESIDUS ? 1 : 0;
        b.pivots = h->pivots.as<double>();
        b.n_slots = n_slots;
        for (const BorderFix::Item& it : fix->items) {
            b.slot = it.slot;
            b.dropped = h->border_dev.as<int>() + it.first;
            b.n_dropped = it.n;
            b.hom = params_dev;
            if (it.flags_off >= 0) {
                ParityFixArgs p = {};
                p.img = b.img;
                p.W = b.W;
                p.H = b.H;
                p.ref = b.ref;
                p.ref_f32 = b.ref_f32;
                p.flags = h->border_flags.as<unsigned char>() + it.flags_off;
                p.gw = h->gW;
                p.gh = h->gH;
                p.order = order;
                p.round_f32 = b.round_f32;
                p.residus = b.residus;
                p.pivots = b.pivots;
                p.hom = params_dev;
                p.n_slots = n_slots;
                p.slot = it.slot;
                p.n_partial = 256;
                if (h->fix_partial.reserve((size_t)p.n_partial * kNumSums * sizeof(double)) != hipSuccess)
                    return fail(h, COREG_EHIP, "hipMalloc failed (parity fix)");
                p.partial = h->fix_partial.as<double>();
                fl.parity.push_back(p);
            }
            if (it.n == 0) continue;
            fl.border.push_back(b);
        }
        if (fix->tap_segs > 0) {
            TapFixArgs t = fix->tap;
            t.img = b.img;
            t.W = b.W;
            t.H = b.H;
            t.ref = b.ref;
            t.ref_f32 = b.ref_f32;
            t.gw = h->gW;
            t.order = order;
            t.round_f32 = b.round_f32;
            t.residus = b.residus;
// ... 89 lines not shown
```

### euispice_coreg_amd/csrc/kernels_common.hpp

```cpp
#pragma once
namespace coreg {

#ifndef COREG_TILE_PTS
#define COREG_TILE_PTS 1024
#endif
#ifndef COREG_POINT_GROUPS
#define COREG_POINT_GROUPS 4
#endif
constexpr int kTilePts = COREG_TILE_PTS;
constexpr int kBlock = 256;
constexpr int kPointGroups = COREG_POINT_GROUPS;
constexpr int kSweepThreads = kBlock * kPointGroups;
constexpr int kChunk = 4;
constexpr int kNumSums = 6;

struct __attribute__((aligned(32))) Pt {
    double b0, b1, a, pad;
};

enum { MODE_TRANSLATE = 0, MODE_HOMOGRAPHY = 1, MODE_HOMOGRAPHY_SERIES = 2, MODE_CAR = 3 };
struct LaunchU {
    double m00, m01, m10, m11, b0, b1;
    int order_rt;
    int h_incr;
    double box_c;
    double pole_sep;
};

__host__ __device__ inline double car_tile_margin(double box_c, double th_abs) {
    if (!(th_abs < 1.5)) return __builtin_inf();
    const double c = cos(th_abs);
    return 1.0 + box_c * 2.0 / (c * c);
}

struct CarrDev {
    const double* sin_lon;
    const double* cos_lon;
    const float* cos_lat;
    const float* sin_lat;
    int n_lon, n_lat;
    double dist, cb, sb, cr, sr, cdelt1, cdelt2;
};

struct H9 {
    double h[9];
};

__device__ __forceinline__ bool carr_term(const CarrDev& c, int i, int j, double& t0, double& t1) {
#pragma clang fp contract(off)
    const double cl = (double)c.cos_lat[j];
    const double y = (double)c.sin_lat[j];
    const double x = cl * c.sin_lon[i];
    const double z = cl * c.cos_lon[i];
    const double zz = z * c.cb + y * c.sb;
    const double yy = y * c.cb - z * c.sb;
    const bool vis = zz >= 0.0;
    const double yr = yy * c.cr - x * c.sr;
    const double xr = x * c.cr + yy * c.sr;
    const double zd = c.dist - zz;
    t0 = atan(xr / zd) * (180.0 / 3.14159265358979323846) * 3600.0 / c.cdelt1;
    t1 = atan(yr / zd) * (180.0 / 3.14159265358979323846) * 3600.0 / c.cdelt2;
    return vis;
}

__device__ __forceinline__ void apply_h(const H9& m, double x, double y, double& ox, double& oy) {
    const double w = fma(m.h[6], x, fma(m.h[7], y, m.h[8]));
    double r = __builtin_amdgcn_rcp(w);
    r = fma(r, fma(-w, r, 1.0), r);
    ox = fma(m.h[0], x, fma(m.h[1], y, m.h[2])) * r;
    oy = fma(m.h[3], x, fma(m.h[4], y, m.h[5])) * r;
}

__device__ __forceinline__ void apply_h_series(const H9& m, double x, double y, double& ox, double& oy) {
    const double eps = fma(m.h[6], x, m.h[7] * y);
    const double q = fma(eps, eps, -eps);
    const double xn = fma(m.h[0], x, fma(m.h[1], y, m.h[2]));
    const double yn = fma(m.h[3], x, fma(m.h[4], y, m.h[5]));
    ox = fma(xn, q, xn);
    oy = fma(yn, q, yn);
}
__device__ __forceinline__ void apply_car(const H9& m, const LaunchU& u, double phi, double theta, double& ox, double& oy) {
    double sp, cp, st, ct;
    sincos(phi, &sp, &cp);
    sincos(theta, &st, &ct);
    const double n0 = ct * cp, n1 = ct * sp, n2 = st;
    const double q0 = fma(m.h[0], n0, fma(m.h[1], n1, m.h[2] * n2));
    const double q1 = fma(m.h[3], n0, fma(m.h[4], n1, m.h[5] * n2));
    const double q2 = fma(m.h[6], n0, fma(m.h[7], n1, m.h[8] * n2));
    const double p = atan2(q1, q0);
    const double t = atan2(q2, sqrt(fma(q0, q0, q1 * q1)));
    ox = fma(u.m00, p, fma(u.m01, t, u.b0));
    oy = fma(u.m10, p, fma(u.m11, t, u.b1));
}
__device__ __forceinline__ void apply_car_vec(const H9& m, const LaunchU& u, double n0, double n1, double n2, double& ox,
                                              double& oy) {
    const double q0 = fma(m.h[0], n0, fma(m.h[1], n1, m.h[2] * n2));
    const double q1 = fma(m.h[3], n0, fma(m.h[4], n1, m.h[5] * n2));
    const double q2 = fma(m.h[6], n0, fma(m.h[7], n1, m.h[8] * n2));
    const double p = atan2(q1, q0);
    const double t = atan2(q2, sqrt(fma(q0, q0, q1 * q1)));
    ox = fma(u.m00, p, fma(u.m01, t, u.b0));
    oy = fma(u.m10, p, fma(u.m11, t, u.b1));
}
template <int MODE>
__device__ __forceinline__ void apply_map(const H9& m, const LaunchU& u, double x, double y, double& ox, double& oy) {
    if (MODE == MODE_CAR) apply_car(m, u, x, y, ox, oy);
    else if (MODE == MODE_HOMOGRAPHY_SERIES) apply_h_series(m, x, y, ox, oy);
    else apply_h(m, x, y, ox, oy);
}

template <int ORDER>
struct Spline;
template <>
struct Spline<2> {
    static constexpr int N = 3;
    static __device__ __forceinline__ void eval(double c, int& start, double w[3]) {
        const double f = floor(c + 0.5);
        const double t = c - f;
        const double u = t * t;
        w[1] = 0.75 - u;
        w[0] = fma(0.5, u, fma(-0.5, t, 0.125));
        w[2] = w[0] + t;
        start = (int)f - 1;
    }
};
template <int ORDER>
__device__ __forceinline__ void spline_weights_t(double t, double* w);
template <>
__device__ __forceinline__ void spline_weights_t<2>(double t, double* w) {
    const double u = t * t;
    w[1] = 0.75 - u;
    w[0] = fma(0.5, u, fma(-0.5, t, 0.125));
    w[2] = w[0] + t;
}
template <>
__device__ __forceinline__ void spline_weights_t<1>(double t, double* w) {
    w[0] = 1.0 - t;
    w[1] = t;
}

__device__ __forceinline__ void spline_weights6_o3(double y, double* w) {
    const double z = 1.0 - y;
    const double y2 = y * y, z2 = z * z;
    w[0] = z2 * z;
    w[1] = fma(3.0 * y2, y - 2.0, 4.0);
    w[2] = fma(3.0 * z2, z - 2.0, 4.0);
    w[3] = ((6.0 - w[0]) - w[1]) - w[2];
}
template <>
__device__ __forceinline__ void spline_weights_t<3>(double y, double* w) {
    spline_weights6_o3(y, w);
#pragma unroll
    for (int k = 0; k < 4; ++k) w[k] *= (1.0 / 6.0);
}
template <>
struct Spline<3> {
    static constexpr int N = 4;
    static __device__ __forceinline__ void eval(double c, int& start, double w[4]) {
        const double f = floor(c);
        spline_weights_t<3>(c - f, w);
        start = (int)f - 1;
    }
};

template <>
struct Spline<1> {
    static constexpr int N = 2;
// ... 202 lines not shown
```

### euispice_coreg_amd/csrc/kernels_prepare.hpp

```cpp
#pragma once
namespace coreg {
template <typename T>
__global__ void __launch_bounds__(256) k_sum_finite(const T* __restrict__ v, long long n, double* part_sum,
                                                    long long* part_cnt) {
    __shared__ double ss[256];
    __shared__ long long sc[256];
    double s = 0.0;
    long long c = 0;
    for (long long i = (long long)blockIdx.x * 256 + threadIdx.x; i < n; i += (long long)gridDim.x * 256) {
        const double x = (double)v[i];
        if (isfinite(x)) {
            s += x;
            ++c;
        }
    }
    ss[threadIdx.x] = s;
    sc[threadIdx.x] = c;
    __syncthreads();
    for (int o = 128; o > 0; o >>= 1) {
        if ((int)threadIdx.x < o) {
            ss[threadIdx.x] += ss[threadIdx.x + o];
            sc[threadIdx.x] += sc[threadIdx.x + o];
        }
        __syncthreads();
// ... 3 lines not shown
        part_cnt[blockIdx.x] = sc[0];
    }
}
__global__ void k_mean_final(const double* part_sum, const long long* part_cnt, int n, double* mean_out) {
    if (threadIdx.x == 0 && blockIdx.x == 0) {
        double s = 0.0;
        long long c = 0;
        for (int i = 0; i < n; ++i) {
            s += part_sum[i];
            c += part_cnt[i];
        }
        mean_out[0] = c > 0 ? s / (double)c : 0.0;
    }
}

__global__ void __launch_bounds__(256) k_f32_exact(const double* __restrict__ v, long long n, int* flag) {
    int bad = 0;
    for (long long i = (long long)blockIdx.x * 256 + threadIdx.x; i < n; i += (long long)gridDim.x * 256) {
        const double x = v[i];
        if (x == x && (double)(float)x != x) bad = 1;
    }
    if (bad) atomicOr(flag, 1);
}
__global__ void __launch_bounds__(256) k_f64_to_f32(const double* __restrict__ v, long long n, float* __restrict__ out) {
    for (long long i = (long long)blockIdx.x * 256 + threadIdx.x; i < n; i += (long long)gridDim.x * 256)
        out[i] = (float)v[i];
}

__global__ void __launch_bounds__(256) k_fits_swap32(unsigned int* __restrict__ v, long long n) {
    for (long long i = (long long)blockIdx.x * 256 + threadIdx.x; i < n; i += (long long)gridDim.x * 256)
        v[i] = __builtin_bswap32(v[i]);
}
__global__ void __launch_bounds__(256) k_fits_to_f64(const void* __restrict__ raw, int bitpix, int scaled, double bscale,
                                                     double bzero, long long n, double* __restrict__ out) {
#pragma clang fp contract(off)
    for (long long i = (long long)blockIdx.x * 256 + threadIdx.x; i < n; i += (long long)gridDim.x * 256) {
        double x;
        switch (bitpix) {
            case 8: x = (double)((const unsigned char*)raw)[i]; break;
            case 16: x = (double)(short)__builtin_bswap16(((const unsigned short*)raw)[i]); break;
            case 32: x = (double)(int)__builtin_bswap32(((const unsigned int*)raw)[i]); break;
            case 64: x = (double)(long long)__builtin_bswap64(((const unsigned long long*)raw)[i]); break;
            case -32: x = (double)__uint_as_float(__builtin_bswap32(((const unsigned int*)raw)[i])); break;
            default: x = __longlong_as_double((long long)__builtin_bswap64(((const unsigned long long*)raw)[i])); break;
        }
        if (scaled) x = x * bscale + bzero;
        out[i] = x;
    }
}

template <typename T>
__global__ void __launch_bounds__(256) k_threshold(T* __restrict__ v, long long n, int has_min, double vmin, int has_max,
                                                   double vmax) {
    for (long long i = (long long)blockIdx.x * 256 + threadIdx.x; i < n; i += (long long)gridDim.x * 256) {
        const double x = fabs((double)v[i]);
        if ((has_min && x < vmin) || (has_max && x > vmax)) v[i] = (T)__builtin_nan("");
    }
}

__global__ void k_fill(double* p, long long n, double v) {
    const long long i = (long long)blockIdx.x * blockDim.x + threadIdx.x;
    if (i < n) p[i] = v;
}

struct ResampleArgs {
    const void* img;
    int W, H;
    int gw, gh;
    CarrDev carr;
    double x0, y0;
    H9 hom;
    void* out;
    int order_rt;
    Crop crop;
    double* bbox;
    LaunchU car_fwd, car_inv;
};
template <int MODE>
__device__ __forceinline__ bool resample_coord(const ResampleArgs& a, long long idx, double& nx, double& ny) {
    const int i = (int)(idx % a.gw), j = (int)(idx / a.gw);
    bool ok = true;
    if (MODE == MODE_TRANSLATE) {
        double t0, t1;
        ok = carr_term(a.carr, i, j, t0, t1);
        nx = a.x0 + t0;
        ny = a.y0 + t1;
    } else if (MODE == MODE_CAR) {
        const double phi = fma(a.car_fwd.m00, (double)i, fma(a.car_fwd.m01, (double)j, a.car_fwd.b0));
        const double theta = fma(a.car_fwd.m10, (double)i, fma(a.car_fwd.m11, (double)j, a.car_fwd.b1));
        apply_car(a.hom, a.car_inv, phi, theta, nx, ny);
    } else {
        apply_h(a.hom, (double)i, (double)j, nx, ny);
    }
    if (!ok) nx = __builtin_nan("");
    return (nx >= 0.0) & (nx <= (double)(a.W - 1)) & (ny >= 0.0) & (ny <= (double)(a.H - 1));
}
template <int MODE>
__global__ void __launch_bounds__(256) k_resample_bbox(const ResampleArgs a) {
    __shared__ double red[4][4];
    const double inf = __builtin_inf();
    double mnx = inf, mxx = -inf, mny = inf, mxy = -inf;
    const long long n = (long long)a.gw * a.gh;
    for (long long idx = (long long)blockIdx.x * 256 + threadIdx.x; idx < n; idx += (long long)gridDim.x * 256) {
        double nx, ny;
        if (resample_coord<MODE>(a, idx, nx, ny)) {
            mnx = fmin(mnx, nx);
            mxx = fmax(mxx, nx);
            mny = fmin(mny, ny);
            mxy = fmax(mxy, ny);
        }
    }
    for (int o = 32; o > 0; o >>= 1) {
        mnx = fmin(mnx, __shfl_xor(mnx, o));
        mxx = fmax(mxx, __shfl_xor(mxx, o));
        mny = fmin(mny, __shfl_xor(mny, o));
        mxy = fmax(mxy, __shfl_xor(mxy, o));
    }
    const int lane = threadIdx.x & 63, wave = threadIdx.x >> 6;
    if (lane == 0) {
        red[wave][0] = mnx;
        red[wave][1] = mxx;
        red[wave][2] = mny;
        red[wave][3] = mxy;
    }
    __syncthreads();
    if (threadIdx.x == 0) {
        double* o = a.bbox + (size_t)blockIdx.x * 4;
        o[0] = fmin(fmin(red[0][0], red[1][0]), fmin(red[2][0], red[3][0]));
        o[1] = fmax(fmax(red[0][1], red[1][1]), fmax(red[2][1], red[3][1]));
        o[2] = fmin(fmin(red[0][2], red[1][2]), fmin(red[2][2], red[3][2]));
        o[3] = fmax(fmax(red[0][3], red[1][3]), fmax(red[2][3], red[3][3]));
    }
}
template <int MODE, int ORDER, typename TS, typename TO>
__global__ void __launch_bounds__(256) k_resample(const ResampleArgs a) {
    const long long idx = (long long)blockIdx.x * 256 + threadIdx.x;
    if (idx >= (long long)a.gw * a.gh) return;
    double nx, ny;
    bool inb = resample_coord<MODE>(a, idx, nx, ny);
    double v = __builtin_nan("");
    if (inb) {
        if constexpr (ORDER == ORDER_RT) v = spline_global_rt<TS>((const TS*)a.img, a.W, a.H, nx, ny, a.order_rt, inb, a.crop);
        else v = spline_global<ORDER, TS>((const TS*)a.img, a.W, a.H, nx, ny, inb, a.crop);
    }
    ((TO*)a.out)[idx] = (TO)v;
}

struct PrologueArgs {
    const double* src;
    double* dst_params;
    long long n_params;
    long long* dst_outidx;
    long long n_outidx;
    double* out;
    long long n_out;
    long long* refine_count;
};
__device__ __forceinline__ void run_prologue(const PrologueArgs& p) {
    if (!p.src) return;
    if (blockIdx.x == 0 && threadIdx.x == 0 && p.refine_count) p.refine_count[0] = p.refine_count[1] = 0;
    const long long stride = (long long)gridDim.x * blockDim.x;
    const long long i0 = (long long)blockIdx.x * blockDim.x + threadIdx.x;
    for (long long i = i0; i < p.n_params; i += stride) p.dst_params[i] = p.src[i];
    const long long* __restrict__ src_idx = (const long long*)(p.src + p.n_params);
    for (long long i = i0; i < p.n_outidx; i += stride) p.dst_outidx[i] = src_idx[i];
    const double nan = __builtin_nan("");
    for (long long i = i0; i < p.n_out; i += stride) p.out[i] = nan;
}

struct PrecomputeArgs {
    PrologueArgs prologue;
    const void* ref;
    int gw, gh;
    int tile_w, tile_h;
    int tiles_x, tiles_y;
    CarrDev carr;
    LaunchU car_fwd;
    double f0lo, f0hi, f1lo, f1hi;
    int residus;
    int tile_skip;
    double lip_x, lip_y;
    double dlon, dlat;
    const double* pivot_a;
    Pt* pts;
    int* tile_count;
    double* tile_bbox;
};
template <int MODE, typename TA>
__global__ void __launch_bounds__(256) k_precompute(const PrecomputeArgs a) {
    __shared__ int wave_cnt[4];
    __shared__ double red[4][4];
    run_prologue(a.prologue);
    const int tile = blockIdx.x;
    const int tx = tile % a.tiles_x, ty = tile / a.tiles_x;
    const int lane = threadIdx.x & 63, wave = threadIdx.x >> 6;
    const double pivot = a.pivot_a[0];
    const double inf = __builtin_inf();
    if (MODE == MODE_TRANSLATE && a.tile_skip) {
        __shared__ int s_skip;
        const int i0 = tx * a.tile_w, j0 = ty * a.tile_h;
        const int i1 = min(i0 + a.tile_w, a.gw) - 1, j1 = min(j0 + a.tile_h, a.gh) - 1;
        if (threadIdx.x == 0) {
            const int ic = (i0 + i1) / 2, jc = (j0 + j1) / 2;
            double t0, t1;
            carr_term(a.carr, ic, jc, t0, t1);
            const double ang = (double)max(ic - i0, i1 - ic) * a.dlon + (double)max(jc - j0, j1 - jc) * a.dlat;
            const double m0 = a.lip_x * ang + 1.0, m1 = a.lip_y * ang + 1.0;
            s_skip = (t0 + m0 < a.f0lo) || (t0 - m0 > a.f0hi) || (t1 + m1 < a.f1lo) || (t1 - m1 > a.f1hi);
        }
        __syncthreads();
        if (s_skip) {
            if (threadIdx.x == 0) a.tile_count[tile] = 0;
            return;
        }
    }
    double mn0 = inf, mx0 = -inf, mn1 = inf, mx1 = -inf;
    int base_pos = 0;
    const size_t tbase = (size_t)tile * kTilePts;
    for (int r = 0; r < kTilePts / 256; ++r) {
        const int k = r * 256 + threadIdx.x;
        const int gi = tx * a.tile_w + (k % a.tile_w);
        const int gj = ty * a.tile_h + (k / a.tile_w);
        bool valid = (gi < a.gw) & (gj < a.gh);
        double b0 = 0.0, b1 = 0.0, av = 0.0;
        if (valid) {
            av = (double)((const TA*)a.ref)[(size_t)gj * a.gw + gi];
            if (MODE == MODE_TRANSLATE) {
                valid = carr_term(a.carr, gi, gj, b0, b1);
            } else if (MODE == MODE_CAR) {
                b0 = fma(a.car_fwd.m00, (double)gi, fma(a.car_fwd.m01, (double)gj, a.car_fwd.b0));
                b1 = fma(a.car_fwd.m10, (double)gi, fma(a.car_fwd.m11, (double)gj, a.car_fwd.b1));
            } else {
                b0 = (double)gi;
                b1 = (double)gj;
            }
            valid = valid & isfinite(av) & (b0 >= a.f0lo) & (b0 <= a.f0hi) & (b1 >= a.f1lo) & (b1 <= a.f1hi);
        }
        const unsigned long long bal = __ballot(valid);
        const int rank = __popcll(bal & ((1ull << lane) - 1ull));
        if (lane == 0) wave_cnt[wave] = __popcll(bal);
        __syncthreads();
        int off = base_pos;
        for (int w = 0; w < wave; ++w) off += wave_cnt[w];
        const int tot = wave_cnt[0] + wave_cnt[1] + wave_cnt[2] + wave_cnt[3];
        if (valid) {
            Pt pt;
            pt.b0 = b0;
            pt.b1 = b1;
            pt.a = a.residus ? av : av - pivot;
            pt.pad = a.residus ? 1.0 / sqrt(av) : 0.0;
            if (MODE == MODE_CAR) {
                double sp, cp, st, ct;
                sincos(b0, &sp, &cp);
                sincos(b1, &st, &ct);
                pt.b0 = ct * cp;
                pt.b1 = ct * sp;
                pt.pad = st;
            }
            a.pts[tbase + off + rank] = pt;
            mn0 = fmin(mn0, b0);
            mx0 = fmax(mx0, b0);
            mn1 = fmin(mn1, b1);
            mx1 = fmax(mx1, b1);
        }
        base_pos += tot;
        __syncthreads();
    }
    if (MODE != MODE_CAR && !a.residus) {
        static_assert(kChunk >= 3, "run flag + the two chunk sums live in the pads of the chunk's first three points");
        Pt* tp = a.pts + tbase;
        for (int c = threadIdx.x; c < base_pos / kChunk; c += 256) {
            double sa = tp[c * kChunk].a, saa = sa * sa;
            bool run = MODE == MODE_HOMOGRAPHY || MODE == MODE_HOMOGRAPHY_SERIES;
#pragma unroll
            for (int k = 1; k < kChunk; ++k) {
                const double v = tp[c * kChunk + k].a;
                sa += v;
                saa = fma(v, v, saa);
                run = run && tp[c * kChunk + k].b0 == tp[c * kChunk].b0 + (double)k && tp[c * kChunk + k].b1 == tp[c * kChunk].b1;
            }
            tp[c * kChunk].pad = run ? 1.0 : 0.0;
            tp[c * kChunk + 1].pad = sa;
            tp[c * kChunk + 2].pad = saa;
        }
    }
    for (int o = 32; o > 0; o >>= 1) {
        mn0 = fmin(mn0, __shfl_xor(mn0, o));
        mx0 = fmax(mx0, __shfl_xor(mx0, o));
        mn1 = fmin(mn1, __shfl_xor(mn1, o));
        mx1 = fmax(mx1, __shfl_xor(mx1, o));
    }
    if (lane == 0) {
        red[wave][0] = mn0;
        red[wave][1] = mx0;
        red[wave][2] = mn1;
        red[wave][3] = mx1;
    }
    __syncthreads();
    if (threadIdx.x == 0) {
        a.tile_count[tile] = base_pos;
        double* bb = a.tile_bbox + (size_t)tile * 4;
        bb[0] = fmin(fmin(red[0][0], red[1][0]), fmin(red[2][0], red[3][0]));
        bb[1] = fmax(fmax(red[0][1], red[1][1]), fmax(red[2][1], red[3][1]));
        bb[2] = fmin(fmin(red[0][2], red[1][2]), fmin(red[2][2], red[3][2]));
        bb[3] = fmax(fmax(red[0][3], red[1][3]), fmax(red[2][3], red[3][3]));
    }
}

constexpr int kUnitPts = kChunk * kPointGroups;
__host__ __device__ inline long long group_start(int g, long long total, int n_groups, int taper_min, int taper_frac) {
    if (taper_frac <= 0) return (long long)g * total / n_groups;
    const int g0 = n_groups - (int)((long long)n_groups * taper_frac / 1024);
    const int nt = n_groups - 1 - g0;
    if (nt <= 0) return (long long)g * total / n_groups;
    const double m = (double)taper_min / 1024.0;
    auto cum = [&](int k) -> double {
        if (k <= g0) return (double)k;
        const double j = (double)(k - g0);
// ... 89 lines not shown
```

### euispice_coreg_amd/csrc/kernels_sweep.hpp

```cpp
#pragma once
namespace coreg {
struct SweepArgs {
    const void* img;
    int W, H;
    const Pt* pts;
    const int* tile_count;
    const int* tile_list;
    const int* tile_cum;
    const int* group_first;
    long long* tile_info;
    const double* tile_bbox;
    const double* lane_params;
    long long n_slots;
    int n_batches;
    int n_groups;
    int group_lo;
    double* partials;
    const double* pivots;
    int use_lds;
    int clean_path;
    int lds_elems;
    LaunchU car_inv;
};

struct Acc {
    int n;
    double a, b, aa, bb, ab;
};

template <int N>
struct Taps;
template <>
struct Taps<3> {
    double t[9];
    __device__ __forceinline__ void issue(unsigned a0, unsigned a1, unsigned a2) {
        asm volatile(
            "ds_read_b64 %0, %9\n\tds_read_b64 %1, %9 offset:8\n\tds_read_b64 %2, %9 offset:16\n\t"
            "ds_read_b64 %3, %10\n\tds_read_b64 %4, %10 offset:8\n\tds_read_b64 %5, %10 offset:16\n\t"
            "ds_read_b64 %6, %11\n\tds_read_b64 %7, %11 offset:8\n\tds_read_b64 %8, %11 offset:16"
            : "=&v"(t[0]), "=&v"(t[1]), "=&v"(t[2]), "=&v"(t[3]), "=&v"(t[4]), "=&v"(t[5]), "=&v"(t[6]), "=&v"(t[7]),
              "=&v"(t[8])
            : "v"(a0), "v"(a1), "v"(a2));
    }
    __device__ __forceinline__ void wait_after(double& w0, double& w1, double& w2, double& w3, double& w4, double& w5) {
        asm volatile("s_waitcnt lgkmcnt(0)"
                     : "+v"(t[0]), "+v"(t[1]), "+v"(t[2]), "+v"(t[3]), "+v"(t[4]), "+v"(t[5]), "+v"(t[6]), "+v"(t[7]),
                       "+v"(t[8]), "+v"(w0), "+v"(w1), "+v"(w2), "+v"(w3), "+v"(w4), "+v"(w5));
    }
    __device__ __forceinline__ void issue_before(unsigned a0, unsigned a1, unsigned a2, double& fx, double& fy) {
        asm volatile(
            "ds_read_b64 %0, %11\n\tds_read_b64 %1, %11 offset:8\n\tds_read_b64 %2, %11 offset:16\n\t"
            "ds_read_b64 %3, %12\n\tds_read_b64 %4, %12 offset:8\n\tds_read_b64 %5, %12 offset:16\n\t"
            "ds_read_b64 %6, %13\n\tds_read_b64 %7, %13 offset:8\n\tds_read_b64 %8, %13 offset:16"
            : "=&v"(t[0]), "=&v"(t[1]), "=&v"(t[2]), "=&v"(t[3]), "=&v"(t[4]), "=&v"(t[5]), "=&v"(t[6]), "=&v"(t[7]),
              "=&v"(t[8]), "+v"(fx), "+v"(fy)
            : "v"(a0), "v"(a1), "v"(a2));
    }
    __device__ __forceinline__ void wait() {
        asm volatile("s_waitcnt lgkmcnt(0)"
                     : "+v"(t[0]), "+v"(t[1]), "+v"(t[2]), "+v"(t[3]), "+v"(t[4]), "+v"(t[5]), "+v"(t[6]), "+v"(t[7]),
                       "+v"(t[8]));
    }
    template <int P>
    __device__ __forceinline__ void issue_before_imm(unsigned a0, double& fx, double& fy) {
        static_assert(P > 0 && (2 * P + 2) * 8 < 65536, "LDS immediate offsets are 16 bits");
        asm volatile(
            "ds_read_b64 %0, %11\n\tds_read_b64 %1, %11 offset:8\n\tds_read_b64 %2, %11 offset:16\n\t"
            "ds_read_b64 %3, %11 offset:%12\n\tds_read_b64 %4, %11 offset:%13\n\tds_read_b64 %5, %11 offset:%14\n\t"
            "ds_read_b64 %6, %11 offset:%15\n\tds_read_b64 %7, %11 offset:%16\n\tds_read_b64 %8, %11 offset:%17"
            : "=&v"(t[0]), "=&v"(t[1]), "=&v"(t[2]), "=&v"(t[3]), "=&v"(t[4]), "=&v"(t[5]), "=&v"(t[6]), "=&v"(t[7]),
              "=&v"(t[8]), "+v"(fx), "+v"(fy)
            : "v"(a0), "n"(P * 8), "n"(P * 8 + 8), "n"(P * 8 + 16), "n"(2 * P * 8), "n"(2 * P * 8 + 8),
              "n"(2 * P * 8 + 16));
    }
};
template <>
struct Taps<2> {
    double t[4];
    __device__ __forceinline__ void issue(unsigned a0, unsigned a1, unsigned) {
        asm volatile(
            "ds_read_b64 %0, %4\n\tds_read_b64 %1, %4 offset:8\n\t"
            "ds_read_b64 %2, %5\n\tds_read_b64 %3, %5 offset:8"
            : "=&v"(t[0]), "=&v"(t[1]), "=&v"(t[2]), "=&v"(t[3])
            : "v"(a0), "v"(a1));
    }
    __device__ __forceinline__ void issue_before(unsigned a0, unsigned a1, unsigned a2, double&, double&) {
        issue(a0, a1, a2);
    }
    __device__ __forceinline__ void wait_after(double&, double&, double&, double&, double&, double&) { wait(); }
    __device__ __forceinline__ void wait() {
        asm volatile("s_waitcnt lgkmcnt(0)" : "+v"(t[0]), "+v"(t[1]), "+v"(t[2]), "+v"(t[3]));
    }
};

template <>
struct Taps<4> {
    double t[16];
    __device__ __forceinline__ void issue_before(unsigned a0, unsigned a1, unsigned a2, unsigned a3, double& fx,
                                                 double& fy) {
        asm volatile(
            "ds_read_b64 %0, %18\n\tds_read_b64 %1, %18 offset:8\n\tds_read_b64 %2, %18 offset:16\n\t"
            "ds_read_b64 %3, %18 offset:24\n\t"
            "ds_read_b64 %4, %19\n\tds_read_b64 %5, %19 offset:8\n\tds_read_b64 %6, %19 offset:16\n\t"
            "ds_read_b64 %7, %19 offset:24\n\t"
            "ds_read_b64 %8, %20\n\tds_read_b64 %9, %20 offset:8\n\tds_read_b64 %10, %20 offset:16\n\t"
            "ds_read_b64 %11, %20 offset:24\n\t"
            "ds_read_b64 %12, %21\n\tds_read_b64 %13, %21 offset:8\n\tds_read_b64 %14, %21 offset:16\n\t"
            "ds_read_b64 %15, %21 offset:24"
            : "=&v"(t[0]), "=&v"(t[1]), "=&v"(t[2]), "=&v"(t[3]), "=&v"(t[4]), "=&v"(t[5]), "=&v"(t[6]), "=&v"(t[7]),
              "=&v"(t[8]), "=&v"(t[9]), "=&v"(t[10]), "=&v"(t[11]), "=&v"(t[12]), "=&v"(t[13]), "=&v"(t[14]),
              "=&v"(t[15]), "+v"(fx), "+v"(fy)
            : "v"(a0), "v"(a1), "v"(a2), "v"(a3));
    }
    template <int P>
    __device__ __forceinline__ void issue_before_imm(unsigned a0, double& fx, double& fy) {
        static_assert(P > 0 && (3 * P + 3) * 8 < 65536, "LDS immediate offsets are 16 bits");
        asm volatile(
            "ds_read_b64 %0, %18\n\tds_read_b64 %1, %18 offset:8\n\tds_read_b64 %2, %18 offset:16\n\t"
            "ds_read_b64 %3, %18 offset:24\n\t"
            "ds_read_b64 %4, %18 offset:%19\n\tds_read_b64 %5, %18 offset:%20\n\tds_read_b64 %6, %18 offset:%21\n\t"
            "ds_read_b64 %7, %18 offset:%22\n\t"
            "ds_read_b64 %8, %18 offset:%23\n\tds_read_b64 %9, %18 offset:%24\n\tds_read_b64 %10, %18 offset:%25\n\t"
            "ds_read_b64 %11, %18 offset:%26\n\t"
            "ds_read_b64 %12, %18 offset:%27\n\tds_read_b64 %13, %18 offset:%28\n\tds_read_b64 %14, %18 offset:%29\n\t"
            "ds_read_b64 %15, %18 offset:%30"
            : "=&v"(t[0]), "=&v"(t[1]), "=&v"(t[2]), "=&v"(t[3]), "=&v"(t[4]), "=&v"(t[5]), "=&v"(t[6]), "=&v"(t[7]),
              "=&v"(t[8]), "=&v"(t[9]), "=&v"(t[10]), "=&v"(t[11]), "=&v"(t[12]), "=&v"(t[13]), "=&v"(t[14]),
              "=&v"(t[15]), "+v"(fx), "+v"(fy)
            : "v"(a0), "n"(P * 8), "n"(P * 8 + 8), "n"(P * 8 + 16), "n"(P * 8 + 24), "n"(2 * P * 8), "n"(2 * P * 8 + 8),
              "n"(2 * P * 8 + 16), "n"(2 * P * 8 + 24), "n"(3 * P * 8), "n"(3 * P * 8 + 8), "n"(3 * P * 8 + 16),
              "n"(3 * P * 8 + 24));
    }
    __device__ __forceinline__ void wait_after(double* wx, double* wy) {
        asm volatile("s_waitcnt lgkmcnt(0)"
                     : "+v"(t[0]), "+v"(t[1]), "+v"(t[2]), "+v"(t[3]), "+v"(t[4]), "+v"(t[5]), "+v"(t[6]), "+v"(t[7]),
                       "+v"(t[8]), "+v"(t[9]), "+v"(t[10]), "+v"(t[11]), "+v"(t[12]), "+v"(t[13]), "+v"(t[14]),
                       "+v"(t[15]), "+v"(wx[0]), "+v"(wx[1]), "+v"(wx[2]), "+v"(wx[3]), "+v"(wy[0]), "+v"(wy[1]),
                       "+v"(wy[2]), "+v"(wy[3]));
    }
};

template <int PITCH, bool FOLDED = false>
__device__ __forceinline__ double gather_o3(unsigned win, int pitch, double cx, double cy, double offx, double offy) {
    int c0, r0;
    double fx, fy;
    if constexpr (FOLDED) {
        c0 = (int)cx;
        r0 = (int)cy;
        fx = __builtin_amdgcn_fract(cx);
        fy = __builtin_amdgcn_fract(cy);
    } else {
        const double flx = floor(cx), fly = floor(cy);
        c0 = (int)flx + (int)offx;
        r0 = (int)fly + (int)offy;
        fx = cx - flx;
        fy = cy - fly;
    }
    const unsigned a0 = win + 8u * (unsigned)(__mul24(r0, PITCH > 0 ? PITCH : pitch) + c0);
    Taps<4> tp;
    if constexpr (PITCH > 0) {
        tp.template issue_before_imm<PITCH>(a0, fx, fy);
    } else {
        const unsigned a1 = a0 + 8u * (unsigned)pitch;
        const unsigned a2 = a1 + 8u * (unsigned)pitch;
        const unsigned a3 = a2 + 8u * (unsigned)pitch;
// ... 103 lines not shown
        }
        if constexpr (CLEAN) {
            static_assert(!RESID && MODE != MODE_CAR, "no room for the chunk sums in Pt");
            acc.b += bm;
            acc.bb = fma(bm, bm, acc.bb);
            acc.ab = fma(av, bm, acc.ab);
        } else if (RESID) {
            const double d = (av - (ROUND ? v : v + pivot_b)) * (MODE == MODE_CAR ? 1.0 / sqrt(av) : isa);
            if (isfinite(d)) {
                acc.n += 1;
                acc.b += d;
                acc.bb = fma(d, d, acc.bb);
            }
        } else if (isfinite(v)) {
            acc.n += 1;
            acc.a += av;
            acc.b += bm;
            acc.aa = fma(av, av, acc.aa);
            acc.bb = fma(bm, bm, acc.bb);
            acc.ab = fma(av, bm, acc.ab);
        }
        return;
    }
    double nx, ny;
    if (MODE == MODE_TRANSLATE) {
        nx = px0 + b0;
        ny = py0 + b1;
    } else {
        if (MODE == MODE_CAR) apply_car_vec(hm, cu, b0, b1, isa, nx, ny);
        else apply_map<MODE>(hm, cu, b0, b1, nx, ny);
    }
    if (INTERIOR || ((nx >= 0.0) & (nx <= wmax) & (ny >= 0.0) & (ny <= hmax))) {
        int sx, sy;
        double wx[N], wy[N];
        double v = 0.0;
        if constexpr (ORDER == ORDER_RT) {
            if constexpr (LDS) {
                v = spline_lds_rt(win, pitch, ox, oy, nx, ny, cu.order_rt);
            } else {
                bool inb;
                v = spline_global_rt<TS>(img, W, H, nx, ny, cu.order_rt, inb);
            }
        } else if constexpr (LDS && ORDER == 2) {
            v = gather_o2<PITCH>(win, pitch, nx + pxw, ny + pyw);
        } else if constexpr (LDS && ORDER == 3) {
            v = gather_o3<PITCH>(win, pitch, nx, ny, pxw, pyw);
        } else if constexpr (LDS) {
            const double fx = floor(nx + (ORDER == 2 ? 0.5 : 0.0)), fy = floor(ny + (ORDER == 2 ? 0.5 : 0.0));
            const int r0 = (int)fy - (ORDER == 2 ? 1 : 0) - oy;
            const int c0 = (int)fx - (ORDER == 2 ? 1 : 0) - ox;
            const unsigned a0 = win + 8u * (unsigned)(__mul24(r0, pitch) + c0);
            const unsigned a1 = a0 + 8u * (unsigned)pitch;
            const unsigned a2 = a1 + 8u * (unsigned)pitch;
            Taps<N> tp;
            tp.issue(a0, a1, a2);
            Spline<ORDER>::eval(nx, sx, wx);
            Spline<ORDER>::eval(ny, sy, wy);
            tp.wait();
#pragma unroll
            for (int r = 0; r < N; ++r) {
                double row = 0.0;
#pragma unroll
                for (int c = 0; c < N; ++c) row = fma(tp.t[r * N + c], wx[c], row);
                v = fma(row, wy[r], v);
            }
        } else {
            Spline<ORDER>::eval(nx, sx, wx);
            Spline<ORDER>::eval(ny, sy, wy);
            int ix[N], iy[N];
#pragma unroll
            for (int k = 0; k < N; ++k) {
                ix[k] = mirror_tap<ORDER>(sx + k, W);
                iy[k] = mirror_tap<ORDER>(sy + k, H) * W;
            }
#pragma unroll
            for (int r = 0; r < N; ++r) {
                double row = 0.0;
#pragma unroll
                for (int c = 0; c < N; ++c) row = fma((double)img[iy[r] + ix[c]], wx[c], row);
                v = fma(row, wy[r], v);
            }
        }
        double bm;
        if (ROUND) {
            v = (double)(float)v;
            bm = v - pivot_b;
        } else {
            bm = LDS ? v : v - pivot_b;
        }
        if (RESID) {
            const double braw = (ROUND || !LDS) ? v : v + pivot_b;
            const double d = (av - braw) * (MODE == MODE_CAR ? 1.0 / sqrt(av) : isa);
            if (isfinite(d)) {
                acc.n += 1;
                acc.b += d;
                acc.bb = fma(d, d, acc.bb);
            }
        } else if (isfinite(v)) {
            acc.n += 1;
            acc.a += av;
            acc.b += bm;
            acc.aa = fma(av, av, acc.aa);
            acc.bb = fma(bm, bm, acc.bb);
            acc.ab = fma(av, bm, acc.ab);
        }
    }
}

#ifndef COREG_PT_SCALAR
#define COREG_PT_SCALAR 2
#endif
#ifndef COREG_PT_ANCHOR
#define COREG_PT_ANCHOR 1
#endif
typedef unsigned SPt __attribute__((ext_vector_type(8)));
__device__ __forceinline__ SPt spt_load(const Pt* __restrict__ p, double& anchor) {
    SPt r;
#if defined(__HIP_DEVICE_COMPILE__)
#if COREG_PT_ANCHOR
    asm volatile("s_load_dwordx8 %0, %2, 0x0" : "=s"(r), "+v"(anchor) : "s"(p));
#else
    asm volatile("s_load_dwordx8 %0, %1, 0x0" : "=s"(r) : "s"(p));
#endif
#else
    r = (SPt)(0u);
    (void)p;
    (void)anchor;
#endif
    return r;
}
__device__ __forceinline__ void spt_wait(SPt& r) {
#if defined(__HIP_DEVICE_COMPILE__)
    asm volatile("s_waitcnt lgkmcnt(0)" : "+s"(r));
#endif
}
__device__ __forceinline__ double spt_f64(const SPt& r, int i) {
    const unsigned long long u = ((unsigned long long)r[2 * i + 1] << 32) | (unsigned long long)r[2 * i];
    return __builtin_bit_cast(double, u);
}
__device__ __forceinline__ void load_pt_uniform(const Pt* __restrict__ p, Pt& out) {
#if defined(__HIP_DEVICE_COMPILE__) && COREG_PT_SCALAR
    typedef const __attribute__((address_space(4))) double* ConstF64;
    ConstF64 q = (ConstF64)(const double*)p;
    out.b0 = q[0];
    out.b1 = q[1];
    out.a = q[2];
    out.pad = q[3];
#else
    out = *p;
#endif
}

template <int MODE, int ORDER, typename TS, bool LDS, bool ROUND, bool RESID, bool INTERIOR = false, int PITCH = 0,
          bool CLEAN = false>
__device__ __forceinline__ void tile_points(Acc& acc, unsigned win, const TS* __restrict__ img, int pitch,
                                            int ox, int oy, int W, int H, double px0, double py0, double pxw,
                                            double pyw, const H9& hm, const LaunchU& cu, const Pt* __restrict__ pts, int p_begin, int p_end,
                                            double pivot_b, int pg) {
    const double wmax = (double)(W - 1), hmax = (double)(H - 1);
    const int n_full = p_end / kChunk;
#if defined(__HIP_DEVICE_COMPILE__) && COREG_PT_SCALAR == 2
    constexpr bool kIncr = INTERIOR && LDS && ORDER == 2 && !RESID &&
                           (MODE == MODE_HOMOGRAPHY || MODE == MODE_HOMOGRAPHY_SERIES);
    if constexpr (kIncr) {
        if (cu.h_incr) {
            H9 hv = hm;
            hv.h[0] = fma(pxw, hm.h[6], hm.h[0]);
            hv.h[1] = fma(pxw, hm.h[7], hm.h[1]);
            hv.h[2] = MODE == MODE_HOMOGRAPHY_SERIES ? hm.h[2] + pxw : fma(pxw, hm.h[8], hm.h[2]);
            hv.h[3] = fma(pyw, hm.h[6], hm.h[3]);
            hv.h[4] = fma(pyw, hm.h[7], hm.h[4]);
            hv.h[5] = MODE == MODE_HOMOGRAPHY_SERIES ? hm.h[5] + pyw : fma(pyw, hm.h[8], hm.h[5]);
            int c = p_begin / kChunk + pg;
            if (c < n_full) {
                double& anchor = hv.h[7];
                SPt cur = spt_load(pts + c * kChunk, anchor);
                spt_wait(cur);
                for (; c < n_full; c += kPointGroups) {
                    const Pt* __restrict__ q = pts + c * kChunk;
                    const bool run = cur[7] != 0u;
                    double xn = 0.0, yn = 0.0, ww = 0.0;
#pragma unroll
                    for (int k = 0; k < kChunk; ++k) {
                        SPt nxt = spt_load(k + 1 < kChunk ? q + k + 1 : q + kPointGroups * kChunk, anchor);
                        const double x = spt_f64(cur, 0), y = spt_f64(cur, 1);
                        if (k == 0 || !run) {
                            xn = fma(hv.h[0], x, fma(hv.h[1], y, hv.h[2]));
                            yn = fma(hv.h[3], x, fma(hv.h[4], y, hv.h[5]));
                            ww = MODE == MODE_HOMOGRAPHY_SERIES ? fma(hv.h[6], x, hv.h[7] * y)
                                                                : fma(hv.h[6], x, fma(hv.h[7], y, hv.h[8]));
                        } else {
                            xn += hv.h[0];
                            yn += hv.h[3];
                            ww += hv.h[6];
                        }
                        double ux, uy;
                        if (MODE == MODE_HOMOGRAPHY_SERIES) {
                            const double qq = fma(ww, ww, -ww);
                            ux = fma(xn, qq, xn);
                            uy = fma(yn, qq, yn);
                        } else {
                            double r = __builtin_amdgcn_rcp(ww);
                            r = fma(r, fma(-ww, r, 1.0), r);
                            ux = xn * r;
                            uy = yn * r;
                        }
                        point_lag<MODE, ORDER, TS, LDS, ROUND, RESID, INTERIOR, PITCH, CLEAN, true>(
                            acc, win, img, pitch, ox, oy, W, H, wmax, hmax, px0, py0, pxw, pyw, hv, cu, ux, uy,
                            spt_f64(cur, 2), spt_f64(cur, 3), pivot_b);
                        if constexpr (CLEAN) {
                            if (k == 1) acc.a += spt_f64(cur, 3);
                            if (k == 2) acc.aa += spt_f64(cur, 3);
                            if (k == kChunk - 1) acc.n += kChunk;
                        }
                        spt_wait(nxt);
                        cur = nxt;
                    }
                }
            }
            if (pg == n_full % kPointGroups) {
                for (int p = n_full * kChunk; p < p_end; ++p) {
                    Pt pt;
                    load_pt_uniform(pts + p, pt);
                    point_lag<MODE, ORDER, TS, LDS, ROUND, RESID, INTERIOR, PITCH>(acc, win, img, pitch, ox, oy, W, H, wmax,
                                                                                   hmax, px0, py0, pxw, pyw, hm, cu, pt.b0,
                                                                                   pt.b1, pt.a, pt.pad, pivot_b);
                }
            }
            return;
        }
    }
    {
        int c = p_begin / kChunk + pg;
        if (c < n_full) {
            H9 hml = hm;
            double& anchor = MODE == MODE_TRANSLATE ? (INTERIOR && LDS ? pxw : px0) : hml.h[MODE == MODE_CAR ? 0 : 7];
            SPt cur = spt_load(pts + c * kChunk, anchor);
            spt_wait(cur);
            for (; c < n_full; c += kPointGroups) {
                const Pt* __restrict__ q = pts + c * kChunk;
#pragma unroll
                for (int k = 0; k < kChunk; ++k) {
                    SPt nxt = spt_load(k + 1 < kChunk ? q + k + 1 : q + kPointGroups * kChunk, anchor);
                    point_lag<MODE, ORDER, TS, LDS, ROUND, RESID, INTERIOR, PITCH, CLEAN>(
                        acc, win, img, pitch, ox, oy, W, H, wmax, hmax, px0, py0, pxw, pyw, hml, cu, spt_f64(cur, 0),
                        spt_f64(cur, 1), spt_f64(cur, 2), spt_f64(cur, 3), pivot_b);
                    if constexpr (CLEAN) {
                        if (k == 1) acc.a += spt_f64(cur, 3);
                        if (k == 2) acc.aa += spt_f64(cur, 3);
                        if (k == kChunk - 1) acc.n += kChunk;
                    }
                    spt_wait(nxt);
                    cur = nxt;
                }
            }
        }
    }
#else
    for (int c = p_begin / kChunk + pg; c < n_full; c += kPointGroups) {
        const Pt* __restrict__ q = pts + c * kChunk;
        Pt pt[kChunk];
#pragma unroll
        for (int k = 0; k < kChunk; ++k) load_pt_uniform(q + k, pt[k]);
#pragma unroll
        for (int k = 0; k < kChunk; ++k)
            point_lag<MODE, ORDER, TS, LDS, ROUND, RESID, INTERIOR, PITCH, CLEAN>(acc, win, img, pitch, ox, oy, W, H, wmax,
                                                                                  hmax, px0, py0, pxw, pyw, hm, cu, pt[k].b0,
                                                                                  pt[k].b1, pt[k].a, pt[k].pad, pivot_b);
        if constexpr (CLEAN) {
            acc.n += kChunk;
            acc.a += pt[1].pad;
            acc.aa += pt[2].pad;
        }
    }
#endif
    if (pg == n_full % kPointGroups) {
        for (int p = n_full * kChunk; p < p_end; ++p) {
            Pt pt;
            load_pt_uniform(pts + p, pt);
            point_lag<MODE, ORDER, TS, LDS, ROUND, RESID, INTERIOR, PITCH>(acc, win, img, pitch, ox, oy, W, H, wmax, hmax,
                                                                           px0, py0, pxw, pyw, hm, cu, pt.b0, pt.b1, pt.a,
                                                                           pt.pad, pivot_b);
        }
    }
}

template <int MODE, int ORDER, typename TS, bool ROUND, bool RESID, int PITCH = 0>
__global__ void __launch_bounds__(kSweepThreads) k_sweep(const SweepArgs a) {
    extern __shared__ __align__(16) unsigned char lds_raw[];
    double* lds = (double*)lds_raw;
    constexpr int kWaves = kSweepThreads / 64;
    constexpr int kLagWaves = kBlock / 64;
    __shared__ double wred2[2][kLagWaves][4];
    __shared__ int wdirty[2][kWaves];
    constexpr bool kCleanPath = MODE != MODE_CAR && !RESID && ORDER != ORDER_RT && !(ROUND && sizeof(TS) == 8);
    int visit = 0;
    int n_vis = 0, n_vis_lds = 0, n_vis_int = 0, n_vis_clean = 0;

    const int b = blockIdx.x;
    const int slot8 = b & 7;
    const int q = b >> 3;
    const int batch = q % a.n_batches;
    const int group = a.group_lo + (q / a.n_batches) * 8 + slot8;

    const int lane = threadIdx.x & 63, wave = threadIdx.x >> 6;
    const int pg = __builtin_amdgcn_readfirstlane(threadIdx.x / kBlock);
    const long long slot = (long long)batch * kBlock + (threadIdx.x % kBlock);

    double px0 = 0.0, py0 = 0.0;
    H9 hm;
#pragma unroll
    for (int k = 0; k < 9; ++k) hm.h[k] = 0.0;
    if (MODE == MODE_TRANSLATE) {
        px0 = a.lane_params[slot];
        py0 = a.lane_params[a.n_slots + slot];
    } else {
#pragma unroll
        for (int k = 0; k < 9; ++k) hm.h[k] = a.lane_params[(long long)k * a.n_slots + slot];
    }

    const bool pad_lane = MODE == MODE_TRANSLATE ? (px0 != px0) : (hm.h[8] != hm.h[8]);

    Acc acc = {0, 0.0, 0.0, 0.0, 0.0, 0.0};

    const TS* __restrict__ img = (const TS*)a.img;
    const int W = a.W, H = a.H;
    const double inf = __builtin_inf();
    const int u_lo = a.group_first[1024 + group];
    const int u_hi = a.group_first[1024 + group + 1];
    const int n_list = (int)a.tile_info[0];
    const double pivot_b = a.pivots[1];
#if defined(__HIP_DEVICE_COMPILE__)
    const unsigned win = (unsigned)(uintptr_t)(__attribute__((address_space(3))) unsigned char*)lds_raw;
#else
    const unsigned win = 0;
#endif

    for (int tl = a.group_first[group]; tl < n_list && u_lo < u_hi; ++tl) {
        const int ubase = a.tile_cum[tl];
        if (ubase >= u_hi) break;
        const int tile = a.tile_list[tl];
        const int cnt = a.tile_count[tile];
        const int p_begin = max(u_lo - ubase, 0) * kUnitPts;
        const int p_end = min((u_hi - ubase) * kUnitPts, cnt);
        if (p_begin >= p_end) continue;
        const double* bb = a.tile_bbox + (size_t)tile * 4;
        const double bx0 = bb[0], bx1 = bb[1], by0 = bb[2], by1 = bb[3];

        double mnx, mxx, mny, mxy;
        if (MODE == MODE_TRANSLATE) {
            mnx = bx0 + px0;
            mxx = bx1 + px0;
            mny = by0 + py0;
            mxy = by1 + py0;
        } else {
            mnx = inf; mxx = -inf; mny = inf; mxy = -inf;
#pragma unroll
            for (int c = 0; c < 4; ++c) {
                double cx, cy;
                apply_map<MODE>(hm, a.car_inv, (c & 1) ? bx1 : bx0, (c & 2) ? by1 : by0, cx, cy);
                mnx = fmin(mnx, cx);
                mxx = fmax(mxx, cx);
                mny = fmin(mny, cy);
                mxy = fmax(mxy, cy);
            }
            if (MODE == MODE_CAR) {
                const double margin = car_tile_margin(a.car_inv.box_c, fmax(fabs(by0), fabs(by1)) + a.car_inv.pole_sep);
                mnx -= margin;
                mxx += margin;
                mny -= margin;
                mxy += margin;
            }
        }
        for (int o = 32; o > 0; o >>= 1) {
            mnx = fmin(mnx, __shfl_xor(mnx, o));
            mxx = fmax(mxx, __shfl_xor(mxx, o));
            mny = fmin(mny, __shfl_xor(mny, o));
            mxy = fmax(mxy, __shfl_xor(mxy, o));
        }
        double(*wred)[4] = wred2[visit & 1];
        int* wdirt = wdirty[visit & 1];
        ++visit;
        if (lane == 0 && wave < kLagWaves) {
            wred[wave][0] = mnx;
            wred[wave][1] = mxx;
            wred[wave][2] = mny;
            wred[wave][3] = mxy;
        }
        __syncthreads();
        mnx = fmin(fmin(wred[0][0], wred[1][0]), fmin(wred[2][0], wred[3][0]));
        mxx = fmax(fmax(wred[0][1], wred[1][1]), fmax(wred[2][1], wred[3][1]));
        mny = fmin(fmin(wred[0][2], wred[1][2]), fmin(wred[2][2], wred[3][2]));
        mxy = fmax(fmax(wred[0][3], wred[1][3]), fmax(wred[2][3], wred[3][3]));
        if (!(mxx >= 0.0) || !(mnx <= (double)(W - 1)) || !(mxy >= 0.0) || !(mny <= (double)(H - 1))) continue;
        constexpr double kClear = 1e-9;
        const bool interior = (mnx >= kClear) & (mxx <= (double)(W - 1) - kClear) & (mny >= kClear) &
                              (mxy <= (double)(H - 1) - kClear);
        constexpr bool kWide = ORDER == ORDER_RT || ORDER > 2;
        const int ord = ORDER == ORDER_RT ? a.car_inv.order_rt : ORDER;
        const int ap_lo = kWide ? ord / 2 + 1 : 1;
        const int ap_hi = kWide ? ord - ord / 2 + 1 : 2;
        const int ox = max((int)floor(fmax(mnx, 0.0)) - ap_lo, kWide ? -ap_lo : -1);
        const int oy = max((int)floor(fmax(mny, 0.0)) - ap_lo, kWide ? -ap_lo : -1);
        const int ex = min((int)floor(fmin(mxx, (double)(W - 1))) + ap_hi, kWide ? W - 1 + ap_hi : W);
        const int ey = min((int)floor(fmin(mxy, (double)(H - 1))) + ap_hi, kWide ? H - 1 + ap_hi : H);
        const int ww = ex - ox + 1, wh = ey - oy + 1;
        int pitch = PITCH > 0 ? PITCH : (ww | 1);
        if (PITCH == 0) {
            const int r = pitch & 31;
            const int up = r < 5 ? 5 - r : ((r > 11 && r < 21) ? 21 - r : (r > 27 ? 37 - r : 0));
            if ((long long)(pitch + up) * wh <= (long long)a.lds_elems) pitch += up;
        }
        const long long need = (long long)pitch * wh;
        const bool in_lds = a.use_lds && (need <= (long long)a.lds_elems) && (PITCH == 0 || ww <= PITCH);

        const Pt* __restrict__ pts = a.pts + (size_t)tile * kTilePts;

        bool swept = false;
        ++n_vis;
        {
          if (in_lds) {
            swept = true;
            ++n_vis_lds;
#ifndef COREG_STAGE_ROWS
#define COREG_STAGE_ROWS 8
#endif
#ifndef COREG_STAGE_COLS
#define COREG_STAGE_COLS 1
#endif
            constexpr int kStage = COREG_STAGE_ROWS, kCols = COREG_STAGE_COLS;
            const double scale = ORDER == 2 ? 0.25 : 1.0;
            const int wave_u = __builtin_amdgcn_readfirstlane(wave);
            double poison = 0.0;
            for (int r0 = wave_u; r0 < wh; r0 += kWaves * kStage) {
                for (int c0 = 0; c0 < ww; c0 += 64 * kCols) {
                    int gx[kCols];
#pragma unroll
                    for (int j = 0; j < kCols; ++j) {
                        const int c = c0 + 64 * j + lane;
                        gx[j] = kWide ? mirror_far(ox + min(c, ww - 1), W) : mirror_idx(ox + min(c, ww - 1), W);
                    }
                    TS v[kStage][kCols];
#pragma unroll
                    for (int k = 0; k < kStage; ++k) {
                        const int r = min(r0 + k * kWaves, wh - 1);
                        const int gy = kWide ? mirror_far(oy + r, H) : mirror_idx(oy + r, H);
                        const TS* __restrict__ row = img + (size_t)gy * W;
#pragma unroll
                        for (int j = 0; j < kCols; ++j) v[k][j] = row[gx[j]];
                    }
#pragma unroll
                    for (int j = 0; j < kCols; ++j) {
                        const int c = c0 + 64 * j + lane;
                        if (c < ww) {
#pragma unroll
                            for (int k = 0; k < kStage; ++k) {
                                const int r = r0 + k * kWaves;
                                if (r < wh) {
                                    const double e = (ROUND ? (double)v[k][j] : (double)v[k][j] - pivot_b) * scale;
                                    lds[r * pitch + c] = e;
                                    if (kCleanPath) poison = fma(e, 0.0, poison);
                                }
                            }
                        }
                    }
                }
            }
            if (kCleanPath && interior) {
                const int dirty = __ballot(poison != poison) != 0ull;
                if (lane == 0) wdirt[wave] = dirty;
            }
            __syncthreads();
            bool done = false;
            if constexpr (ORDER != ORDER_RT) {
                if (interior) {
                    done = true;
                    bool clean = false;
                    if constexpr (kCleanPath) clean = a.clean_path && __ballot(wdirt[lane % kWaves] != 0) == 0ull;
                    ++n_vis_int;
                    n_vis_clean += clean ? 1 : 0;
                    if (!pad_lane) {
                        const double offx = (ORDER == 2 ? 0.5 : 0.0) - (double)(ORDER / 2 + ox);
                        const double offy = (ORDER == 2 ? 0.5 : 0.0) - (double)(ORDER / 2 + oy);
                        const double pxw = MODE == MODE_TRANSLATE ? px0 + offx : offx;
                        const double pyw = MODE == MODE_TRANSLATE ? py0 + offy : offy;
                        if (kCleanPath && clean) {
                            tile_points<MODE, ORDER, TS, true, ROUND, RESID, true, PITCH, kCleanPath>(
                                acc, win, img, pitch, ox, oy, W, H, px0, py0, pxw, pyw, hm, a.car_inv, pts, p_begin, p_end,
                                pivot_b, pg);
                        } else {
                            tile_points<MODE, ORDER, TS, true, ROUND, RESID, true, PITCH>(acc, win, img, pitch, ox, oy, W, H,
                                                                                          px0, py0, pxw, pyw, hm, a.car_inv,
                                                                                          pts, p_begin, p_end, pivot_b, pg);
                        }
                    }
                }
            }
            if (!done) {
                const double offx = ORDER == 2 ? 0.5 - (double)(1 + ox) : (ORDER == 3 ? -(double)(1 + ox) : 0.0);
                const double offy = ORDER == 2 ? 0.5 - (double)(1 + oy) : (ORDER == 3 ? -(double)(1 + oy) : 0.0);
                tile_points<MODE, ORDER, TS, true, ROUND, RESID, false, PITCH>(acc, win, img, pitch, ox, oy, W, H, px0, py0,
                                                                               offx, offy, hm, a.car_inv, pts, p_begin,
                                                                               p_end, pivot_b, pg);
            }
          }
        }
        if (!swept) {
            tile_points<MODE, ORDER, TS, false, ROUND, RESID>(acc, win, img, 0, 0, 0, W, H, px0, py0, 0.0, 0.0, hm, a.car_inv, pts,
                                                              p_begin, p_end, pivot_b, pg);
        }
    }

    if (threadIdx.x == 0) {
        atomicAdd((unsigned long long*)a.tile_info + 3, (unsigned long long)n_vis);
        atomicAdd((unsigned long long*)a.tile_info + 4, (unsigned long long)n_vis_lds);
        atomicAdd((unsigned long long*)a.tile_info + 5, (unsigned long long)n_vis_int);
        atomicAdd((unsigned long long*)a.tile_info + 6, (unsigned long long)n_vis_clean);
    }
    __syncthreads();
    const int ls = threadIdx.x % kBlock;
    if (pg > 0) {
        double* st = lds + ((size_t)(pg - 1) * kNumSums) * kBlock + ls;
        st[0] = (double)acc.n;
        st[kBlock] = acc.a;
        st[2 * kBlock] = acc.b;
        st[3 * kBlock] = acc.aa;
        st[4 * kBlock] = acc.bb;
        st[5 * kBlock] = acc.ab;
    }
    __syncthreads();
    if (pg == 0) {
        double sn = (double)acc.n, sa = acc.a, sb = acc.b, saa = acc.aa, sbb = acc.bb, sab = acc.ab;
        for (int g = 0; g < kPointGroups - 1; ++g) {
            const double* st = lds + ((size_t)g * kNumSums) * kBlock + ls;
            sn += st[0];
            sa += st[kBlock];
            sb += st[2 * kBlock];
            saa += st[3 * kBlock];
            sbb += st[4 * kBlock];
            sab += st[5 * kBlock];
        }
        double* out = a.partials + (size_t)(group - a.group_lo) * kNumSums * a.n_slots + slot;
        out[0] = sn;
        out[a.n_slots] = sa;
        out[2 * a.n_slots] = sb;
        out[3 * a.n_slots] = saa;
        out[4 * a.n_slots] = sbb;
        out[5 * a.n_slots] = sab;
    }
}

}
```

### include/coreg_hip.h

```cpp
#ifndef COREG_HIP_H
#define COREG_HIP_H

#include <stdint.h>

#ifdef __cplusplus
extern "C" {
#endif

#define COREG_OK 0
#define COREG_EINVAL (-1)
#define COREG_EHIP (-2)
#define COREG_ESTATE (-3)
#define COREG_ENOTIMPL (-4)
#define COREG_ENOMEM (-5)

#define COREG_F32 0
#define COREG_F64 1
#define COREG_I32 2

#define COREG_PROJ_TAN 0
#define COREG_PROJ_CAR 1

#define COREG_METHOD_CORRELATION 0
#define COREG_METHOD_RESIDUS 1

#define COREG_CDELT_INTENDED 0
#define COREG_CDELT_REFERENCE 1

typedef struct coreg_handle coreg_handle;

typedef struct coreg_wcs2d {
    int32_t naxis1, naxis2;
    double crpix1, crpix2;
    double crval1, crval2;
    double cdelt1, cdelt2;
    double pc1_1, pc1_2, pc2_1, pc2_2;
    double crota;
    double unit_to_deg;
    double lonpole;
    double dsun_obs;
    double crln_obs;
    double crlt_obs;
    double latpole;
    int32_t proj;
    int32_t reserved;
} coreg_wcs2d;

typedef struct coreg_lags {
    const double* crval1; int32_t n_crval1;
    const double* crval2; int32_t n_crval2;
    const double* cdelt1; int32_t n_cdelt1;
    const double* cdelt2; int32_t n_cdelt2;
    const double* crota;  int32_t n_crota;
} coreg_lags;

typedef struct coreg_carr_grid {
    double lon0, lon1; int32_t n_lon;
    double lat0, lat1; int32_t n_lat;
    const float* lat_cos;
    const float* lat_sin;
} coreg_carr_grid;

typedef struct coreg_stats {
    double sweep_kernel_ms;
    double precompute_ms;
    double total_gpu_ms;
    int64_t n_lags;
    int64_t n_grid_points;
    int64_t n_active_points;
    int64_t n_sweep_launches;
    int32_t small_is_f32;
    int32_t used_lds;
} coreg_stats;

const char* coreg_version(void);

int coreg_create(coreg_handle** h, int device);
void coreg_destroy(coreg_handle* h);
const char* coreg_last_error(const coreg_handle* h);

int coreg_set_stream(coreg_handle* h, void* hip_stream);
int coreg_synchronize(coreg_handle* h);

int coreg_set_small(coreg_handle* h, const double* img, int32_t ny, int32_t nx);

int coreg_set_small_f32(coreg_handle* h, const float* img, int32_t ny, int32_t nx);

typedef struct coreg_fits_pixels {
    const void* data;
    int32_t bitpix;
    int32_t reserved;
    double bscale, bzero;
} coreg_fits_pixels;
int coreg_set_small_fits(coreg_handle* h, const coreg_fits_pixels* px, int32_t ny, int32_t nx);
int coreg_prepare_reference_carrington_fits(coreg_handle* h, const coreg_fits_pixels* px, int32_t ny, int32_t nx,
                                            const coreg_wcs2d* hdr_large, const coreg_carr_grid* grid, double solar_r,
                                            int order);
int coreg_prepare_reference_helioprojective_fits(coreg_handle* h, const coreg_fits_pixels* px, int32_t ny, int32_t nx,
                                                 const coreg_wcs2d* hdr_large, const coreg_wcs2d* hdr_small, int order);

typedef struct coreg_fits_tiled {
    const void* heap;
    int64_t heap_bytes;
    const int64_t* tile_offset;
    const int32_t* tile_nbytes;
    int32_t n_tiles;
    int32_t zbitpix;
    int32_t naxis1, naxis2, ztile1, ztile2;
    int32_t blocksize, bytepix;
    int32_t quantize;
    int32_t dither0;
    int32_t has_blank, blank;
    const double* zscale;
    const double* zzero;
    double zscale0, zzero0;
    double bscale, bzero;
} coreg_fits_tiled;
int coreg_set_small_tiled(coreg_handle* h, const coreg_fits_tiled* t);
int coreg_prepare_reference_carrington_tiled(coreg_handle* h, const coreg_fits_tiled* t, const coreg_wcs2d* hdr_large,
                                             const coreg_carr_grid* grid, double solar_r, int order);
int coreg_prepare_reference_helioprojective_tiled(coreg_handle* h, const coreg_fits_tiled* t, const coreg_wcs2d* hdr_large,
                                                  const coreg_wcs2d* hdr_small, int order);
int coreg_decode_tiled_host(const coreg_fits_tiled* t, void* out, int dtype, int32_t* tile_status);
int coreg_encode_tiled_host(const void* pixels, int dtype, int ny, int nx, int tile_x, int tile_y, int bytepix,
                            int blocksize, int quantize, int dither0, double scale, unsigned char* heap,
                            long long heap_cap, int32_t* tile_nbytes, int64_t* tile_offset, double* zscale, double* zzero,
                            long long* heap_used);

int coreg_threshold_small(coreg_handle* h, int has_min, double vmin, int has_max, double vmax, long long* n_finite);

int coreg_set_reference_on_grid(coreg_handle* h, const void* ref, int dtype, int32_t gy, int32_t gx);

int coreg_prepare_reference_carrington(coreg_handle* h, const double* large, int32_t ny, int32_t nx,
                                       const coreg_wcs2d* hdr_large, const coreg_carr_grid* grid, double solar_r,
                                       int order);
int coreg_prepare_reference_helioprojective(coreg_handle* h, const double* large, int32_t ny, int32_t nx,
                                            const coreg_wcs2d* hdr_large, const coreg_wcs2d* hdr_small, int order);
int coreg_prepare_reference_carrington_f32(coreg_handle* h, const float* large, int32_t ny, int32_t nx,
                                           const coreg_wcs2d* hdr_large, const coreg_carr_grid* grid, double solar_r,
                                           int order);
int coreg_prepare_reference_helioprojective_f32(coreg_handle* h, const float* large, int32_t ny, int32_t nx,
                                                const coreg_wcs2d* hdr_large, const coreg_wcs2d* hdr_small, int order);

int coreg_set_small_from_device(coreg_handle* h, const void* dev_img, int dtype, int32_t ny, int32_t nx);
int coreg_prepare_reference_carrington_from_device(coreg_handle* h, const void* dev_large, int dtype, int32_t ny,
                                                   int32_t nx, const coreg_wcs2d* hdr_large,
                                                   const coreg_carr_grid* grid, double solar_r, int order);
int coreg_prepare_reference_helioprojective_from_device(coreg_handle* h, const void* dev_large, int dtype, int32_t ny,
                                                        int32_t nx, const coreg_wcs2d* hdr_large,
                                                        const coreg_wcs2d* hdr_small, int order);

int coreg_get_reference_on_grid(coreg_handle* h, void* out, int dtype);

int coreg_resample_carrington(coreg_handle* h, const coreg_wcs2d* hdr, const coreg_carr_grid* grid, double solar_r,
                              int order, double* out);
int coreg_resample_helioprojective(coreg_handle* h, const coreg_wcs2d* hdr_target, const coreg_wcs2d* hdr,
                                   int order, float* out);
int coreg_resample_helioprojective_f64(coreg_handle* h, const coreg_wcs2d* hdr_target, const coreg_wcs2d* hdr,
                                       int order, double* out);

int coreg_sweep_carrington(coreg_handle* h, const coreg_wcs2d* hdr_small, const coreg_carr_grid* grid,
                           double solar_r, const coreg_lags* lags, int order, int method, int cdelt_semantics,
                           int64_t lag_begin, int64_t lag_end, double* corr_out, int out_on_device);
int coreg_sweep_helioprojective(coreg_handle* h, const coreg_wcs2d* hdr_target, const coreg_wcs2d* hdr_small,
                                const coreg_lags* lags, int order, int method, int cdelt_semantics,
                                int64_t lag_begin, int64_t lag_end, double* corr_out, int out_on_device);

int coreg_sums_size(coreg_handle* h, int64_t* n_doubles);
int coreg_copy_sums(coreg_handle* h, double* dst, int dst_on_device);
int coreg_finalize_sums(coreg_handle* h, const double* sums, int sums_on_device, double* corr_out, int out_on_device);

int coreg_get_pivots(coreg_handle* h, double* pivots2);
int coreg_set_pivots(coreg_handle* h, const double* pivots2);

int coreg_last_stats(coreg_handle* h, coreg_stats* out);

int coreg_last_visit_counts(coreg_handle* h, int64_t* counts6);
int coreg_last_tap_fix(coreg_handle* h, int64_t* counts3);

int coreg_set_option(coreg_handle* h, const char* name, int64_t value);

int coreg_shift_header(const coreg_wcs2d* ref, double d_crval1, double d_crval2, double d_cdelt1, double d_cdelt2,
                       double d_crota, int cdelt_semantics, coreg_wcs2d* out);
int coreg_homography(const coreg_wcs2d* from, const coreg_wcs2d* to, double* h9);
int coreg_lag_homography(const coreg_wcs2d* hdr_target, const coreg_wcs2d* hdr_small, const coreg_lags* lags,
                         const int32_t idx[5], int cdelt_semantics, double* h9);
int coreg_wcslib_pixel_to_pixel(const coreg_wcs2d* from, const coreg_wcs2d* to, int64_t n, const double* px,
                                const double* py, double* ox, double* oy, double* lng, double* lat);
int coreg_carrington_origin(const coreg_wcs2d* hdr, double* x0, double* y0);
int coreg_car_map(const coreg_wcs2d* from, const coreg_wcs2d* to, int64_t n, const double* px, const double* py,
                  double* ox, double* oy);
int coreg_car_tile_margin(const coreg_wcs2d* hdr_target, const coreg_wcs2d* hdr_shifted, int32_t tile_w,
                          double tile_abs_lat_rad, double* margin_px);


int coreg_nansum_planes_be(const void* cube, int32_t bitpix, int64_t n_pixels, const int64_t* plane_index, int32_t n_sel,
                           double* out);

int coreg_fit_gaussian2d(int32_t m, const double* x, const double* y, const double* z, const double* p0,
                         const double* lb, const double* ub, int32_t jac, double ftol, double xtol, double gtol,
                         int32_t max_nfev, double* popt, int32_t* nfev, int32_t* status);


int coreg_set_context_frames(coreg_handle* h, int32_t n_frames, int32_t ny, int32_t nx, int dtype,
                             const coreg_wcs2d* hdrs, const void* const* pixels);
int coreg_context_frame_from_small(coreg_handle* h, int32_t k);
int coreg_sweep_context(coreg_handle* h, const coreg_wcs2d* hdr_target, const coreg_wcs2d* hdr_small,
                        const int32_t* col_frame, const coreg_lags* lags, int order, int method, int cdelt_semantics,
                        int has_min, double vmin, int has_max, double vmax, int64_t lag_begin, int64_t lag_end,
                        double* corr_out, int out_on_device);
int coreg_context_lag_headers(const coreg_wcs2d* hdr_target, const coreg_wcs2d* hdr_small, double d_crval1,
                              double d_crval2, double d_cdelt1, double d_cdelt2, double d_crota, int cdelt_semantics,
                              coreg_wcs2d* ctx, coreg_wcs2d* grid, coreg_wcs2d* shifted);

typedef struct coreg_multi coreg_multi;
int coreg_device_count(void);
int coreg_physical_device_count(void);
int coreg_multi_create(coreg_multi** m, int n_devices, const int* device_ids);
void coreg_multi_destroy(coreg_multi* m);
int coreg_multi_size(const coreg_multi* m);
coreg_handle* coreg_multi_handle(coreg_multi* m, int k);
const char* coreg_multi_last_error(const coreg_multi* m);
const char* coreg_multi_collective(const coreg_multi* m);
const char* coreg_multi_rccl_status(const coreg_multi* m);
int coreg_multi_last_mode(const coreg_multi* m);
int coreg_multi_set_option(coreg_multi* m, const char* name, int64_t value);
int coreg_multi_set_small(coreg_multi* m, const void* img, int dtype, int32_t ny, int32_t nx);
int coreg_multi_set_small_fits(coreg_multi* m, const coreg_fits_pixels* px, int32_t ny, int32_t nx);
int coreg_multi_prepare_reference_carrington_fits(coreg_multi* m, const coreg_fits_pixels* px, int32_t ny, int32_t nx,
                                                  const coreg_wcs2d* hdr_large, const coreg_carr_grid* grid,
                                                  double solar_r, int order);
int coreg_multi_prepare_reference_helioprojective_fits(coreg_multi* m, const coreg_fits_pixels* px, int32_t ny,
                                                       int32_t nx, const coreg_wcs2d* hdr_large,
                                                       const coreg_wcs2d* hdr_small, int order);
int coreg_multi_set_small_tiled(coreg_multi* m, const coreg_fits_tiled* t);
int coreg_multi_prepare_reference_carrington_tiled(coreg_multi* m, const coreg_fits_tiled* t, const coreg_wcs2d* hdr_large,
                                                   const coreg_carr_grid* grid, double solar_r, int order);
int coreg_multi_prepare_reference_helioprojective_tiled(coreg_multi* m, const coreg_fits_tiled* t,
                                                        const coreg_wcs2d* hdr_large, const coreg_wcs2d* hdr_small,
                                                        int order);
int coreg_multi_threshold_small(coreg_multi* m, int has_min, double vmin, int has_max, double vmax, long long* n_finite);
int coreg_multi_set_reference_on_grid(coreg_multi* m, const void* ref, int dtype, int32_t gy, int32_t gx);
int coreg_multi_prepare_reference_carrington(coreg_multi* m, const void* large, int dtype, int32_t ny, int32_t nx,
                                             const coreg_wcs2d* hdr_large, const coreg_carr_grid* grid, double solar_r,
                                             int order);
int coreg_multi_prepare_reference_helioprojective(coreg_multi* m, const void* large, int dtype, int32_t ny, int32_t nx,
                                                  const coreg_wcs2d* hdr_large, const coreg_wcs2d* hdr_small, int order);
int coreg_multi_sweep_carrington(coreg_multi* m, const coreg_wcs2d* hdr_small, const coreg_carr_grid* grid, double solar_r,
                                 const coreg_lags* lags, int order, int method, int cdelt_semantics, double* corr_out);
int coreg_multi_sweep_helioprojective(coreg_multi* m, const coreg_wcs2d* hdr_target, const coreg_wcs2d* hdr_small,
                                      const coreg_lags* lags, int order, int method, int cdelt_semantics, double* corr_out);
int coreg_multi_last_stats(coreg_multi* m, int k, coreg_stats* out);
int coreg_multi_plan(int32_t n_crval1, int32_t n_crval2, int64_t n_inner, int32_t world, int32_t per_combo_launch,
                     int32_t* mode, int32_t* g_combo, int32_t* g1, int32_t* g2);

#ifdef __cplusplus
}
#endif
#endif
```

Baseline: 1.163 million lag-points/s.

## Recut edge lag batches and skip dead lag-waves in sweep kernel

Changes the lag-patch planner to cost each batch by its number of live 64-lane waves and optionally re-tile the ragged edge row and column of the lag plane with differently shaped patches. Live lags are packed at the start of each batch. The kernel appears to use per-batch lag-wave counts to skip dead waves and to shrink the point-group reduction slab. The aim is to cut wasted work on partially filled batches at the lag-plane edges, at the cost of a more complex planner, extra kernel template variants, and a new planning ABI plus a timing script.

```diff
diff --git a/euispice_coreg_amd/_lib.py b/euispice_coreg_amd/_lib.py
--- a/euispice_coreg_amd/_lib.py
+++ b/euispice_coreg_amd/_lib.py
@@ -196,6 +196,10 @@
     ("coreg_last_stats", C.c_int, [_P, C.POINTER(Stats)]),
     ("coreg_last_visit_counts", C.c_int, [_P, C.POINTER(C.c_int64)]),
     ("coreg_last_tap_fix", C.c_int, [_P, C.POINTER(C.c_int64)]),
+    ("coreg_last_plan_counts", C.c_int, [_P, C.POINTER(C.c_int64)]),
+    ("coreg_plan_lag_slots", C.c_int,
+     [C.c_int32, C.c_int32, C.c_int64, C.c_int64, C.POINTER(C.c_double), C.c_int64, C.c_int64, C.POINTER(C.c_int32),
+      C.POINTER(C.c_int64), C.POINTER(C.c_int32), C.POINTER(C.c_int32)]),
     ("coreg_set_option", C.c_int, [_P, C.c_char_p, C.c_int64]),
     ("coreg_shift_header", C.c_int,
      [_WP, C.c_double, C.c_double, C.c_double, C.c_double, C.c_double, C.c_int, _WP]),
@@ -678,6 +682,11 @@
                 "flagged_not_refined": c[5]}
 
 
+    def last_plan_counts(self) -> dict:
+        c = (C.c_int64 * 6)()
+        self._chk(self._lib.coreg_last_plan_counts(self._h, c))
+        return {"batches_by_lag_waves": (c[0], c[1], c[2], c[3]), "lag_waves": c[4], "lane_slots": c[5]}
+
     def last_tap_fix(self) -> dict:
         c = (C.c_int64 * 3)()
         self._chk(self._lib.coreg_last_tap_fix(self._h, c))
diff --git a/euispice_coreg_amd/csrc/abi_host.hpp b/euispice_coreg_amd/csrc/abi_host.hpp
--- a/euispice_coreg_amd/csrc/abi_host.hpp
+++ b/euispice_coreg_amd/csrc/abi_host.hpp
@@ -28,6 +28,46 @@
     if (h->counters.p) HIPCHK(hipMemcpy(refined, h->counters.p, sizeof(refined), hipMemcpyDeviceToHost));
     counts5[4] = refined[0];
     counts6[5] = refined[1];
+    return COREG_OK;
+}
+
+int coreg_last_plan_counts(coreg_handle* h, int64_t* counts6) {
+    if (!h || !counts6) return COREG_EINVAL;
+    for (int k = 0; k < 6; ++k) counts6[k] = h->plan_counts[k];
+    return COREG_OK;
+}
+
+int coreg_plan_lag_slots(int32_t n_crval1, int32_t n_crval2, int64_t lag_begin, int64_t lag_end, const double* geometry8,
+                         int64_t lds_elems, int64_t cap_slots, int32_t* plan3, int64_t* out_index, int32_t* lag_waves,
+                         int32_t* n_batches) {
+    if (n_crval1 < 1 || n_crval2 < 1 || !geometry8 || !plan3 || !n_batches || cap_slots < 0 || lds_elems < 1)
+        return COREG_EINVAL;
+    if (lag_begin < 0 || lag_begin >= lag_end || lag_end > (int64_t)n_crval1 * n_crval2) return COREG_EINVAL;
+    LagDims d = {n_crval1, n_crval2, 1, 1, 1, 1, 0};
+    Geometry g;
+    g.dx_di = geometry8[0];
+    g.dy_di = geometry8[1];
+    g.dx_dj = geometry8[2];
+    g.dy_dj = geometry8[3];
+    g.ax = geometry8[4];
+    g.ay = geometry8[5];
+    g.bx = geometry8[6];
+    g.by = geometry8[7];
+    const int m1 = (int)((lag_end - 1) / n_crval2) - (int)(lag_begin / n_crval2) + 1;
+    const Plan plan = choose_plan(nullptr, g, m1, n_crval2, lds_elems);
+    SlotList slots;
+    build_slots(d, 0, lag_begin, lag_end, plan, &slots);
+    plan3[0] = plan.tile_w;
+    plan3[1] = plan.sw;
+    plan3[2] = plan.sh;
+    *n_batches = slots.n_batches;
+    if ((int64_t)slots.outidx.size() > cap_slots) return COREG_EINVAL;
+    if (slots.n_batches > 0 && (!out_index || !lag_waves)) return COREG_EINVAL;
+    for (size_t s = 0; s < slots.outidx.size(); ++s) out_index[s] = slots.outidx[s];
+    for (int b = 0; b < slots.n_batches; ++b) {
+        lag_waves[b] = batch_lag_waves(slots.outidx.data() + (size_t)b * kBlock);
+        if (lag_waves[b] != slots.lag_waves[b]) return COREG_ESTATE;
+    }
     return COREG_OK;
 }
 
diff --git a/euispice_coreg_amd/csrc/abi_sweeps.hpp b/euispice_coreg_amd/csrc/abi_sweeps.hpp
--- a/euispice_coreg_amd/csrc/abi_sweeps.hpp
+++ b/euispice_coreg_amd/csrc/abi_sweeps.hpp
@@ -83,7 +83,7 @@
     call.d.inner(c, &i3, &i4, &i5);
     if (shift_header(small, 0.0, 0.0, call.lags->cdelt1[i3], call.lags->cdelt2[i4], call.lags->crota[i5], call.sem, hc))
         return false;
-    build_slots(call.d, c, call.lag_begin, call.lag_end, plan.sw, plan.sh, slots);
+    build_slots(call.d, c, call.lag_begin, call.lag_end, plan, slots);
     return slots->n_batches > 0;
 }
 
diff --git a/euispice_coreg_amd/csrc/host_plan.hpp b/euispice_coreg_amd/csrc/host_plan.hpp
--- a/euispice_coreg_amd/csrc/host_plan.hpp
+++ b/euispice_coreg_amd/csrc/host_plan.hpp
@@ -93,31 +93,82 @@
 struct Plan {
     int tile_w = 32;
     int sw = 16, sh = 16;
+    int sw_edge = 0, sh_edge = 0;
     double window = 0;
     double win_w = 0, win_h = 0;
 };
+
+int live_lag_waves(long long n_live) { return (int)((n_live + 63) / 64); }
+double batch_cost(long long n_live) {
+    static const double kCost[kBlock / 64 + 1] = {0.0, 0.53, 0.66, 0.93, 1.0};
+    return kCost[live_lag_waves(n_live)];
+}
+
+struct LagRect {
+    int a1, w, a2, h;
+};
+void plan_rects(int m1, int n2, int sw, int sh, int sw_edge, int sh_edge, std::vector<LagRect>* out) {
+    out->clear();
+    const int cols = (m1 + sw - 1) / sw, rows = (n2 + sh - 1) / sh;
+    const int ew = m1 - (cols - 1) * sw, eh = n2 - (rows - 1) * sh;
+    const bool recut_col = sh_edge > 0 && ew < sw, recut_row = sw_edge > 0 && eh < sh;
+    for (int p1 = 0; p1 < cols - (recut_col ? 1 : 0); ++p1)
+        for (int p2 = 0; p2 < rows - (recut_row ? 1 : 0); ++p2)
+            out->push_back({p1 * sw, std::min(sw, m1 - p1 * sw), p2 * sh, std::min(sh, n2 - p2 * sh)});
+    if (recut_row) {
+        const int x_end = recut_col ? (cols - 1) * sw : m1;
+        for (int x = 0; x < x_end; x += sw_edge) out->push_back({x, std::min(sw_edge, x_end - x), (rows - 1) * sh, eh});
+    }
+    if (recut_col)
+        for (int y = 0; y < n2; y += sh_edge) out->push_back({(cols - 1) * sw, ew, y, std::min(sh_edge, n2 - y)});
+}
+double rects_cost(const std::vector<LagRect>& rects, int* lag_waves = nullptr) {
+    double cost = 0.0;
+    int lw = 0;
+    for (const LagRect& r : rects) {
+        cost += batch_cost((long long)r.w * r.h);
+        lw += live_lag_waves((long long)r.w * r.h);
+    }
+    if (lag_waves) *lag_waves = lw;
+    return cost;
+}
+
+int pitch_for(double win_w, double win_h, long long lds_elems, int order) {
+    static const int kPitches[] = {89, 121, 153, 185, 217};
+    for (int p : kPitches)
+        if ((double)p >= win_w + (order > 2 ? 4.0 : 2.0) && (double)p * (win_h + (order > 2 ? 2.0 : 0.0)) <= 0.985 * (double)lds_elems)
+            return p;
+    return 0;
+}
 
 Plan choose_plan(coreg_handle* h, const Geometry& g, int m1, int n2, long long lds_elems) {
     Plan best, fallback;
     double best_cost = std::numeric_limits<double>::max(), fb_win = std::numeric_limits<double>::max();
-    const int sw_hi = h->opt_patch_w > 0 ? std::min<int>((int)h->opt_patch_w, kBlock) : kBlock;
+    const int sw_hi = h && h->opt_patch_w > 0 ? std::min<int>((int)h->opt_patch_w, kBlock) : kBlock;
+    std::vector<LagRect> rects;
     for (int tw = 4; tw <= 256; tw *= 2) {
-        if (h->opt_tile_w > 0 && tw != h->opt_tile_w) continue;
+        if (h && h->opt_tile_w > 0 && tw != h->opt_tile_w) continue;
         const int th = kTilePts / tw;
         if (th < 1) continue;
         const double tex = tw * std::fabs(g.dx_di) + th * std::fabs(g.dx_dj);
         const double tey = tw * std::fabs(g.dy_di) + th * std::fabs(g.dy_dj);
-        for (int sw = 1; sw <= std::min(m1, sw_hi); ++sw) {
-            int sh = std::min(n2, kBlock / sw);
+        auto ext_x = [&](int w, int hh) { return tex + w * std::fabs(g.ax) + hh * std::fabs(g.bx) + 6.0; };
+        auto ext_y = [&](int w, int hh) { return tey + w * std::fabs(g.ay) + hh * std::fabs(g.by) + 6.0; };
+        auto fits = [&](int w, int hh) { return (ext_x(w, hh) + 1.0) * ext_y(w, hh) <= 0.94 * (double)lds_elems; };
+        for (int sw2 = 1; sw2 <= std::min(m1, sw_hi); ++sw2)
+          for (int even = 0; even < 2; ++even) {
+            int sh = std::min(n2, kBlock / sw2);
             if (sh < 1) break;
-            const int cols = (m1 + sw - 1) / sw, rows = (n2 + sh - 1) / sh;
-            sh = (n2 + rows - 1) / rows;
-            const int sw2 = (m1 + cols - 1) / cols;
-            const double ex = tex + sw2 * std::fabs(g.ax) + sh * std::fabs(g.bx) + 6.0;
-            const double ey = tey + sw2 * std::fabs(g.ay) + sh * std::fabs(g.by) + 6.0;
+            if (even) {
+                const int rows = (n2 + sh - 1) / sh, sh_even = (n2 + rows - 1) / rows;
+                if (sh_even == sh) continue;
+                sh = sh_even;
+            }
+            const double ex = ext_x(sw2, sh), ey = ext_y(sw2, sh);
             const double win = (ex + 1.0) * ey;
             if (win < fb_win) {
                 fb_win = win;
+                fallback = Plan();
                 fallback.tile_w = tw;
                 fallback.sw = sw2;
                 fallback.sh = sh;
@@ -125,25 +176,68 @@
                 fallback.win_w = ex + 1.0;
                 fallback.win_h = ey;
             }
-            if (win > 0.94 * (double)lds_elems) continue;
-            const double cost = (double)cols * rows * (1.0 + 0.08 * win / (double)lds_elems);
-            if (cost < best_cost) {
-                best_cost = cost;
-                best.tile_w = tw;
-                best.sw = sw2;
-                best.sh = sh;
-                best.window = win;
-                best.win_w = ex + 1.0;
-                best.win_h = ey;
+            if (!fits(sw2, sh)) continue;
+            const int cols = (m1 + sw2 - 1) / sw2, rows = (n2 + sh - 1) / sh;
+            const int ew = m1 - (cols - 1) * sw2, eh = n2 - (rows - 1) * sh;
+            for (int recut = 0; recut < 2; ++recut) {
+                Plan p;
+                p.tile_w = tw;
+                p.sw = sw2;
+                p.sh = sh;
+                p.window = win;
+                p.win_w = ex + 1.0;
+                p.win_h = ey;
+                if (recut) {
+                    if (ew < sw2) {
+                        int he = std::min(n2, kBlock / ew);
+                        while (he > 1 && !fits(ew, he)) --he;
+                        const int k = (n2 + he - 1) / he;
+                        p.sh_edge = (n2 + k - 1) / k;
+                    }
+                    if (eh < sh) {
+                        int we = std::min(sw2, kBlock / eh);
+                        while (we > 1 && !fits(we, eh)) --we;
+                        const int x_end = p.sh_edge > 0 ? (cols - 1) * sw2 : m1;
+                        if (x_end > 0) {
+                            const int k = (x_end + we - 1) / we;
+                            p.sw_edge = (x_end + k - 1) / k;
+                        }
+                    }
+                    if (p.sh_edge == 0 && p.sw_edge == 0) continue;
+                    if (p.sh_edge > 0) {
+                        p.win_w = std::max(p.win_w, ext_x(ew, p.sh_edge) + 1.0);
+                        p.win_h = std::max(p.win_h, ext_y(ew, p.sh_edge));
+                        p.window = std::max(p.window, (ext_x(ew, p.sh_edge) + 1.0) * ext_y(ew, p.sh_edge));
+                    }
+                    if (p.sw_edge > 0) {
+                        p.win_w = std::max(p.win_w, ext_x(p.sw_edge, eh) + 1.0);
+                        p.win_h = std::max(p.win_h, ext_y(p.sw_edge, eh));
+                        p.window = std::max(p.window, (ext_x(p.sw_edge, eh) + 1.0) * ext_y(p.sw_edge, eh));
+                    }
+                    if (pitch_for(p.win_w, p.win_h, lds_elems, 3) != pitch_for(ex + 1.0, ey, lds_elems, 3)) continue;
+                }
+                plan_rects(m1, n2, p.sw, p.sh, p.sw_edge, p.sh_edge, &rects);
+                const double cost = rects_cost(rects) + (double)rects.size() * 0.08 * p.window / (double)lds_elems;
+                if (cost < best_cost) {
+                    best_cost = cost;
+                    best = p;
+                }
             }
         }
     }
     const Plan& r = best_cost < std::numeric_limits<double>::max() ? best : fallback;
-    if (std::getenv("COREG_DEBUG_PLAN"))
+    if (std::getenv("COREG_DEBUG_PLAN")) {
+        int lag_waves = 0;
+        plan_rects(m1, n2, r.sw, r.sh, r.sw_edge, r.sh_edge, &rects);
+        const double cost = rects_cost(rects, &lag_waves);
+        std::fprintf(stderr, "[coreg plan] lag plane %d x %d: %d batches, %d live lag-waves, %.2f full-batch times; edge column "
+                     "in heights of %d, edge row in widths of %d (0: like the rest)\n", m1, n2, (int)rects.size(), lag_waves, cost,
+                     r.sh_edge, r.sw_edge);
         std::fprintf(stderr, "[coreg plan] tile %d x %d, lag patch %d x %d, window estimate %.0f (%.1f x %.1f) of %lld elements; "
                      "geometry d/di (%.3f, %.3f) d/dj (%.3f, %.3f) lag1 (%.3f, %.3f) lag2 (%.3f, %.3f)\n", r.tile_w,
                      kTilePts / r.tile_w, r.sw, r.sh, r.window, r.win_w, r.win_h, lds_elems, g.dx_di, g.dy_di, g.dx_dj, g.dy_dj, g.ax, g.ay,
                      g.bx, g.by);
+    }
     return r;
 }
 
@@ -175,56 +269,51 @@
 struct SlotList {
     std::vector<int> i1, i2;
     std::vector<long long> outidx;
+    std::vector<int> lag_waves;
     int n_batches = 0;
 };
 
-void build_slots(const LagDims& d, long long c, long long begin, long long end, int sw, int sh, SlotList* s) {
+int batch_lag_waves(const long long* outidx) {
+    int last = 0;
+    for (int t = 0; t < kBlock; ++t)
+        if (outidx[t] >= 0) last = t;
+    return last / 64 + 1;
+}
+
+void build_slots(const LagDims& d, long long c, long long begin, long long end, const Plan& plan, SlotList* s) {
     s->i1.clear();
     s->i2.clear();
     s->outidx.clear();
+    s->lag_waves.clear();
     s->n_batches = 0;
-    {
-        const size_t cap = (size_t)((d.n1 + sw - 1) / sw + 1) * ((d.n2 + sh - 1) / sh) * kBlock;
-        s->i1.reserve(cap);
-        s->i2.reserve(cap);
-        s->outidx.reserve(cap);
-    }
     const long long row = (long long)d.n2 * d.nc;
     const int i1_lo = (int)(begin / row);
     const int i1_hi = (int)((end - 1) / row);
     const int m1 = i1_hi - i1_lo + 1;
-    for (int p1 = 0; p1 * sw < m1; ++p1)
-        for (int p2 = 0; p2 * sh < d.n2; ++p2) {
-            bool any = false;
-            const size_t at = s->i1.size();
-            for (int t = 0; t < kBlock; ++t) {
-                int lx = t % sw, ly = t / sw;
-                bool valid = ly < sh;
-                if (!valid) lx = ly = 0;
-                int i1 = i1_lo + p1 * sw + lx, i2 = p2 * sh + ly;
-                if (i1 > i1_hi) {
-                    i1 = i1_hi;
-                    valid = false;
-                }
-                if (i2 > d.n2 - 1) {
-                    i2 = d.n2 - 1;
-                    valid = false;
-                }
+    std::vector<LagRect> rects;
+    plan_rects(m1, d.n2, plan.sw, plan.sh, plan.sw_edge, plan.sh_edge, &rects);
+    s->i1.reserve(rects.size() * kBlock);
+    s->i2.reserve(rects.size() * kBlock);
+    s->outidx.reserve(rects.size() * kBlock);
+    for (const LagRect& r : rects) {
+        const size_t at = s->i1.size();
+        for (int ly = 0; ly < r.h; ++ly)
+            for (int lx = 0; lx < r.w; ++lx) {
+                const int i1 = i1_lo + r.a1 + lx, i2 = r.a2 + ly;
                 const long long idx = ((long long)i1 * d.n2 + i2) * d.nc + c;
-                if (idx < begin || idx >= end) valid = false;
+                if (idx < begin || idx >= end) continue;
                 s->i1.push_back(i1);
                 s->i2.push_back(i2);
-                s->outidx.push_back(valid ? idx : -1);
-                any |= valid;
+                s->outidx.push_back(idx);
             }
-            if (!any) {
-                s->i1.resize(at);
-                s->i2.resize(at);
-                s->outidx.resize(at);
-            } else {
-                s->n_batches++;
-            }
-        }
+        const size_t n_live = s->i1.size() - at;
+        if (n_live == 0) continue;
+        s->i1.resize(at + kBlock, s->i1[at]);
+        s->i2.resize(at + kBlock, s->i2[at]);
+        s->outidx.resize(at + kBlock, -1);
+        s->lag_waves.push_back(live_lag_waves((long long)n_live));
+        s->n_batches++;
+    }
 }
 
 int pick_groups(coreg_handle* h, int n_batches, int n_tiles) {
@@ -274,7 +363,7 @@
 }
 
 int reserve_tiles(coreg_handle* h, int n_tiles) {
-    const size_t pts = (size_t)n_tiles * kTilePts + (size_t)(kPointGroups + 1) * kChunk;
+    const size_t pts = (size_t)n_tiles * kTilePts + (size_t)(kMaxPointGroups + 1) * kChunk;
     HIPCHK(h->pts.reserve(pts * sizeof(Pt)));
     HIPCHK(h->tile_count.reserve(n_tiles * sizeof(int)));
     HIPCHK(h->tile_list.reserve(n_tiles * sizeof(int)));
@@ -308,17 +397,12 @@
 
 int pick_pitch(const coreg_handle* h, const Plan& plan, long long lds_elems, int order = 2) {
     if (h->opt_pitch == 0 || !h->opt_use_lds) return 0;
-    static const int kPitches[] = {89, 121, 153, 185, 217};
     if (h->opt_pitch > 0) {
-        for (int p : kPitches)
+        for (int p : {89, 121, 153, 185, 217})
             if (p == h->opt_pitch) return p;
         return 0;
     }
-    for (int p : kPitches)
-        if ((double)p >= plan.win_w + (order > 2 ? 4.0 : 2.0) &&
-            (double)p * (plan.win_h + (order > 2 ? 2.0 : 0.0)) <= 0.985 * (double)lds_elems)
-            return p;
-    return 0;
-}
-
-}
+    return pitch_for(plan.win_w, plan.win_h, lds_elems, order);
+}
+
+}
diff --git a/euispice_coreg_amd/csrc/host_state.hpp b/euispice_coreg_amd/csrc/host_state.hpp
--- a/euispice_coreg_amd/csrc/host_state.hpp
+++ b/euispice_coreg_amd/csrc/host_state.hpp
@@ -124,7 +124,9 @@
     DevBuf pts, tile_count, tile_list, tile_cum, group_first, tile_info, tile_bbox;
     DevBuf rf_fix_slab;
     DevBuf counters;
-    DevBuf lane_params, out_index, partials, out_dev, tmp_img;
+    DevBuf lane_params, out_index, batch_lw, partials, out_dev, tmp_img;
+    std::vector<int> plan_lag_waves;
+    int64_t plan_counts[6] = {0, 0, 0, 0, 0, 0};
     DevBuf up_f64, up_flag;
     DevBuf up_raw;
     DevBuf rice_blob, rice_rand, dec_img;
diff --git a/euispice_coreg_amd/csrc/host_sweep_io.hpp b/euispice_coreg_amd/csrc/host_sweep_io.hpp
--- a/euispice_coreg_amd/csrc/host_sweep_io.hpp
+++ b/euispice_coreg_amd/csrc/host_sweep_io.hpp
@@ -87,21 +87,27 @@
 }
 
 long long lds_window_elems(const coreg_handle* h) {
-    const size_t lds_min = (size_t)(kPointGroups - 1) * kNumSums * kBlock * sizeof(double);
+    const size_t lds_min = kSweepEpilogueLds;
     return (long long)(std::max(lds_min, (size_t)h->opt_lds_bytes) / sizeof(double));
 }
 
 int upload_plan(coreg_handle* h, const std::vector<double>& params, const std::vector<long long>& outidx,
                 double* out_dev, long long n_out) {
-    const size_t bytes = params.size() * sizeof(double) + outidx.size() * sizeof(long long);
+    const size_t n_batches = outidx.size() / kBlock;
+    h->plan_lag_waves.resize(n_batches);
+    for (size_t b = 0; b < n_batches; ++b) h->plan_lag_waves[b] = batch_lag_waves(outidx.data() + b * kBlock);
+    const size_t bytes = params.size() * sizeof(double) + outidx.size() * sizeof(long long) + n_batches * sizeof(int);
     HIPCHK(h->lane_params.reserve(params.size() * sizeof(double)));
     HIPCHK(h->out_index.reserve(outidx.size() * sizeof(long long)));
+    HIPCHK(h->batch_lw.reserve(std::max<size_t>(1, n_batches) * sizeof(int)));
     PinBuf& pin = h->pin_plan[h->plan_slot];
     HIPCHK(hipEventSynchronize(h->ev_end[h->plan_slot]));
     h->plan_open = true;
     HIPCHK(pin.reserve(bytes));
     std::memcpy(pin.p, params.data(), params.size() * sizeof(double));
     std::memcpy((char*)pin.p + params.size() * sizeof(double), outidx.data(), outidx.size() * sizeof(long long));
+    std::memcpy((char*)pin.p + params.size() * sizeof(double) + outidx.size() * sizeof(long long), h->plan_lag_waves.data(),
+                n_batches * sizeof(int));
     void* src_dev = nullptr;
     HIPCHK(hipHostGetDevicePointer(&src_dev, pin.p, 0));
     PrologueArgs& p = h->pending_prologue;
@@ -110,6 +116,7 @@
     p.n_params = (long long)params.size();
     p.dst_outidx = h->out_index.as<long long>();
     p.n_outidx = (long long)outidx.size();
+    p.dst_batch_lw = h->batch_lw.as<int>();
     p.out = out_dev;
     p.n_out = n_out;
     HIPCHK(h->counters.reserve(8 * sizeof(long long)));
diff --git a/euispice_coreg_amd/csrc/host_sweep_launch.hpp b/euispice_coreg_amd/csrc/host_sweep_launch.hpp
--- a/euispice_coreg_amd/csrc/host_sweep_launch.hpp
+++ b/euispice_coreg_amd/csrc/host_sweep_launch.hpp
@@ -24,6 +24,24 @@
     a.tile_info = h->tile_info.as<long long>();
     a.tile_bbox = h->tile_bbox.as<double>();
     a.lane_params = params_dev;
+    {
+        const size_t b0 = (size_t)(outidx_dev - h->out_index.as<long long>()) / kBlock;
+        if (outidx_dev < h->out_index.as<long long>() || b0 + n_batches > h->plan_lag_waves.size())
+            return fail(h, COREG_ESTATE, "launch_sweep: no plan staged for these slots");
+        a.batch_lw = h->batch_lw.as<int>() + b0;
+        std::memset(h->plan_counts, 0, sizeof(h->plan_counts));
+        for (int b = 0; b < n_batches; ++b) {
+            const int lw = h->plan_lag_waves[b0 + b];
+            h->plan_counts[lw - 1]++;
+            h->plan_counts[4] += lw;
+        }
+        h->plan_counts[5] = n_slots;
+        if (std::getenv("COREG_DEBUG_PLAN"))
+            std::fprintf(stderr, "[coreg plan] launch of %d batches: %lld / %lld / %lld / %lld of 1 / 2 / 3 / 4 live lag-waves, "
+                         "%lld lag-waves in %lld lane slots\n", n_batches, (long long)h->plan_counts[0],
+                         (long long)h->plan_counts[1], (long long)h->plan_counts[2], (long long)h->plan_counts[3],
+                         (long long)h->plan_counts[4], (long long)h->plan_counts[5]);
+    }
     a.n_slots = n_slots;
     a.n_batches = n_batches;
     a.n_groups = n_groups;
@@ -32,7 +50,7 @@
     a.pivots = h->pivots.as<double>();
     a.use_lds = h->opt_use_lds ? 1 : 0;
     a.clean_path = h->opt_clean_path ? 1 : 0;
-    const size_t lds_min = (size_t)(kPointGroups - 1) * kNumSums * kBlock * sizeof(double);
+    const size_t lds_min = kSweepEpilogueLds;
     const size_t lds_bytes = std::max(lds_min, a.use_lds ? (size_t)h->opt_lds_bytes : 0);
     a.lds_elems = (int)(lds_bytes / sizeof(double));
     std::memset(&a.car_inv, 0, sizeof(a.car_inv));
diff --git a/euispice_coreg_amd/csrc/kernels_common.hpp b/euispice_coreg_amd/csrc/kernels_common.hpp
--- a/euispice_coreg_amd/csrc/kernels_common.hpp
+++ b/euispice_coreg_amd/csrc/kernels_common.hpp
@@ -11,8 +11,10 @@
 constexpr int kBlock = 256;
 constexpr int kPointGroups = COREG_POINT_GROUPS;
 constexpr int kSweepThreads = kBlock * kPointGroups;
+constexpr int kMaxPointGroups = kSweepThreads / 64;
 constexpr int kChunk = 4;
 constexpr int kNumSums = 6;
+constexpr size_t kSweepEpilogueLds = (size_t)(kMaxPointGroups - 1) * kNumSums * 64 * sizeof(double);
 
 struct __attribute__((aligned(32))) Pt {
     double b0, b1, a, pad;
diff --git a/euispice_coreg_amd/csrc/kernels_prepare.hpp b/euispice_coreg_amd/csrc/kernels_prepare.hpp
--- a/euispice_coreg_amd/csrc/kernels_prepare.hpp
+++ b/euispice_coreg_amd/csrc/kernels_prepare.hpp
@@ -179,6 +179,7 @@
     long long n_params;
     long long* dst_outidx;
     long long n_outidx;
+    int* dst_batch_lw;
     double* out;
     long long n_out;
     long long* refine_count;
@@ -191,6 +192,8 @@
     for (long long i = i0; i < p.n_params; i += stride) p.dst_params[i] = p.src[i];
     const long long* __restrict__ src_idx = (const long long*)(p.src + p.n_params);
     for (long long i = i0; i < p.n_outidx; i += stride) p.dst_outidx[i] = src_idx[i];
+    const int* __restrict__ src_lw = (const int*)(src_idx + p.n_outidx);
+    for (long long i = i0; i < p.n_outidx / kBlock; i += stride) p.dst_batch_lw[i] = src_lw[i];
     const double nan = __builtin_nan("");
     for (long long i = i0; i < p.n_out; i += stride) p.out[i] = nan;
 }
diff --git a/euispice_coreg_amd/csrc/kernels_sweep.hpp b/euispice_coreg_amd/csrc/kernels_sweep.hpp
--- a/euispice_coreg_amd/csrc/kernels_sweep.hpp
+++ b/euispice_coreg_amd/csrc/kernels_sweep.hpp
@@ -11,6 +11,7 @@
     long long* tile_info;
     const double* tile_bbox;
     const double* lane_params;
+    const int* batch_lw;
     long long n_slots;
     int n_batches;
     int n_groups;
@@ -420,11 +421,12 @@
 }
 
 template <int MODE, int ORDER, typename TS, bool LDS, bool ROUND, bool RESID, bool INTERIOR = false, int PITCH = 0,
-          bool CLEAN = false>
+          bool CLEAN = false, int NPG = 0>
 __device__ __forceinline__ void tile_points(Acc& acc, unsigned win, const TS* __restrict__ img, int pitch,
                                             int ox, int oy, int W, int H, double px0, double py0, double pxw,
                                             double pyw, const H9& hm, const LaunchU& cu, const Pt* __restrict__ pts, int p_begin, int p_end,
-                                            double pivot_b, int pg) {
+                                            double pivot_b, int pg, int n_pg_rt) {
+    const int n_pg = NPG > 0 ? NPG : n_pg_rt;
     const double wmax = (double)(W - 1), hmax = (double)(H - 1);
     const int n_full = p_end / kChunk;
 #if defined(__HIP_DEVICE_COMPILE__) && COREG_PT_SCALAR == 2
@@ -444,13 +446,13 @@
                 double& anchor = hv.h[7];
                 SPt cur = spt_load(pts + c * kChunk, anchor);
                 spt_wait(cur);
-                for (; c < n_full; c += kPointGroups) {
+                for (; c < n_full; c += n_pg) {
                     const Pt* __restrict__ q = pts + c * kChunk;
                     const bool run = cur[7] != 0u;
                     double xn = 0.0, yn = 0.0, ww = 0.0;
 #pragma unroll
                     for (int k = 0; k < kChunk; ++k) {
-                        SPt nxt = spt_load(k + 1 < kChunk ? q + k + 1 : q + kPointGroups * kChunk, anchor);
+                        SPt nxt = spt_load(k + 1 < kChunk ? q + k + 1 : q + n_pg * kChunk, anchor);
                         const double x = spt_f64(cur, 0), y = spt_f64(cur, 1);
                         if (k == 0 || !run) {
                             xn = fma(hv.h[0], x, fma(hv.h[1], y, hv.h[2]));
@@ -486,7 +488,7 @@
                     }
                 }
             }
-            if (pg == n_full % kPointGroups) {
+            if (pg == n_full % n_pg) {
                 for (int p = n_full * kChunk; p < p_end; ++p) {
                     Pt pt;
                     load_pt_uniform(pts + p, pt);
@@ -505,11 +507,11 @@
             double& anchor = MODE == MODE_TRANSLATE ? (INTERIOR && LDS ? pxw : px0) : hml.h[MODE == MODE_CAR ? 0 : 7];
             SPt cur = spt_load(pts + c * kChunk, anchor);
             spt_wait(cur);
-            for (; c < n_full; c += kPointGroups) {
+            for (; c < n_full; c += n_pg) {
                 const Pt* __restrict__ q = pts + c * kChunk;
 #pragma unroll
                 for (int k = 0; k < kChunk; ++k) {
-                    SPt nxt = spt_load(k + 1 < kChunk ? q + k + 1 : q + kPointGroups * kChunk, anchor);
+                    SPt nxt = spt_load(k + 1 < kChunk ? q + k + 1 : q + n_pg * kChunk, anchor);
                     point_lag<MODE, ORDER, TS, LDS, ROUND, RESID, INTERIOR, PITCH, CLEAN>(
                         acc, win, img, pitch, ox, oy, W, H, wmax, hmax, px0, py0, pxw, pyw, hml, cu, spt_f64(cur, 0),
                         spt_f64(cur, 1), spt_f64(cur, 2), spt_f64(cur, 3), pivot_b);
@@ -525,7 +527,7 @@
         }
     }
 #else
-    for (int c = p_begin / kChunk + pg; c < n_full; c += kPointGroups) {
+    for (int c = p_begin / kChunk + pg; c < n_full; c += n_pg) {
         const Pt* __restrict__ q = pts + c * kChunk;
         Pt pt[kChunk];
 #pragma unroll
@@ -542,7 +544,7 @@
         }
     }
 #endif
-    if (pg == n_full % kPointGroups) {
+    if (pg == n_full % n_pg) {
         for (int p = n_full * kChunk; p < p_end; ++p) {
             Pt pt;
             load_pt_uniform(pts + p, pt);
@@ -572,19 +574,28 @@
     const int group = a.group_lo + (q / a.n_batches) * 8 + slot8;
 
     const int lane = threadIdx.x & 63, wave = threadIdx.x >> 6;
-    const int pg = __builtin_amdgcn_readfirstlane(threadIdx.x / kBlock);
-    const long long slot = (long long)batch * kBlock + (threadIdx.x % kBlock);
-
-    double px0 = 0.0, py0 = 0.0;
+    const int wave_s = __builtin_amdgcn_readfirstlane(wave);
+    const int n_lw = min(max(a.batch_lw[batch], 1), kLagWaves);
+    const int n_pg = kWaves / n_lw;
+    const int pg = n_lw == 3 ? wave_s / 3 : wave_s >> (n_lw >> 1);
+    const int lw = wave_s - pg * n_lw;
+    const bool dealt = pg < n_pg;
+    const bool full = n_pg == kPointGroups;
+    const long long slot = (long long)batch * kBlock + (dealt ? lw : 0) * 64 + lane;
+
+    const double nan = __builtin_nan("");
+    double px0 = nan, py0 = nan;
     H9 hm;
 #pragma unroll
-    for (int k = 0; k < 9; ++k) hm.h[k] = 0.0;
-    if (MODE == MODE_TRANSLATE) {
-        px0 = a.lane_params[slot];
-        py0 = a.lane_params[a.n_slots + slot];
-    } else {
-#pragma unroll
-        for (int k = 0; k < 9; ++k) hm.h[k] = a.lane_params[(long long)k * a.n_slots + slot];
+    for (int k = 0; k < 9; ++k) hm.h[k] = nan;
+    if (dealt) {
+        if (MODE == MODE_TRANSLATE) {
+            px0 = a.lane_params[slot];
+            py0 = a.lane_params[a.n_slots + slot];
+        } else {
+#pragma unroll
+            for (int k = 0; k < 9; ++k) hm.h[k] = a.lane_params[(long long)k * a.n_slots + slot];
+        }
     }
 
     const bool pad_lane = MODE == MODE_TRANSLATE ? (px0 != px0) : (hm.h[8] != hm.h[8]);
@@ -753,13 +764,23 @@
                         const double pxw = MODE == MODE_TRANSLATE ? px0 + offx : offx;
                         const double pyw = MODE == MODE_TRANSLATE ? py0 + offy : offy;
                         if (kCleanPath && clean) {
-                            tile_points<MODE, ORDER, TS, true, ROUND, RESID, true, PITCH, kCleanPath>(
-                                acc, win, img, pitch, ox, oy, W, H, px0, py0, pxw, pyw, hm, a.car_inv, pts, p_begin, p_end,
-                                pivot_b, pg);
+                            if (full)
+                                tile_points<MODE, ORDER, TS, true, ROUND, RESID, true, PITCH, kCleanPath, kPointGroups>(
+                                    acc, win, img, pitch, ox, oy, W, H, px0, py0, pxw, pyw, hm, a.car_inv, pts, p_begin,
+                                    p_end, pivot_b, pg, n_pg);
+                            else
+                                tile_points<MODE, ORDER, TS, true, ROUND, RESID, true, PITCH, kCleanPath>(
+                                    acc, win, img, pitch, ox, oy, W, H, px0, py0, pxw, pyw, hm, a.car_inv, pts, p_begin,
+                                    p_end, pivot_b, pg, n_pg);
                         } else {
-                            tile_points<MODE, ORDER, TS, true, ROUND, RESID, true, PITCH>(acc, win, img, pitch, ox, oy, W, H,
-                                                                                          px0, py0, pxw, pyw, hm, a.car_inv,
-                                                                                          pts, p_begin, p_end, pivot_b, pg);
+                            if (full)
+                                tile_points<MODE, ORDER, TS, true, ROUND, RESID, true, PITCH, false, kPointGroups>(
+                                    acc, win, img, pitch, ox, oy, W, H, px0, py0, pxw, pyw, hm, a.car_inv, pts, p_begin,
+                                    p_end, pivot_b, pg, n_pg);
+                            else
+                                tile_points<MODE, ORDER, TS, true, ROUND, RESID, true, PITCH>(
+                                    acc, win, img, pitch, ox, oy, W, H, px0, py0, pxw, pyw, hm, a.car_inv, pts, p_begin,
+                                    p_end, pivot_b, pg, n_pg);
                         }
                     }
                 }
@@ -767,15 +788,20 @@
             if (!done) {
                 const double offx = ORDER == 2 ? 0.5 - (double)(1 + ox) : (ORDER == 3 ? -(double)(1 + ox) : 0.0);
                 const double offy = ORDER == 2 ? 0.5 - (double)(1 + oy) : (ORDER == 3 ? -(double)(1 + oy) : 0.0);
-                tile_points<MODE, ORDER, TS, true, ROUND, RESID, false, PITCH>(acc, win, img, pitch, ox, oy, W, H, px0, py0,
-                                                                               offx, offy, hm, a.car_inv, pts, p_begin,
-                                                                               p_end, pivot_b, pg);
+                if (full)
+                    tile_points<MODE, ORDER, TS, true, ROUND, RESID, false, PITCH, false, kPointGroups>(
+                        acc, win, img, pitch, ox, oy, W, H, px0, py0, offx, offy, hm, a.car_inv, pts, p_begin, p_end, pivot_b,
+                        pg, n_pg);
+                else
+                    tile_points<MODE, ORDER, TS, true, ROUND, RESID, false, PITCH>(
+                        acc, win, img, pitch, ox, oy, W, H, px0, py0, offx, offy, hm, a.car_inv, pts, p_begin, p_end, pivot_b,
+                        pg, n_pg);
             }
           }
         }
         if (!swept) {
             tile_points<MODE, ORDER, TS, false, ROUND, RESID>(acc, win, img, 0, 0, 0, W, H, px0, py0, 0.0, 0.0, hm, a.car_inv, pts,
-                                                              p_begin, p_end, pivot_b, pg);
+                                                              p_begin, p_end, pivot_b, pg, n_pg);
         }
     }
 
@@ -786,27 +812,33 @@
         atomicAdd((unsigned long long*)a.tile_info + 6, (unsigned long long)n_vis_clean);
     }
     __syncthreads();
-    const int ls = threadIdx.x % kBlock;
-    if (pg > 0) {
-        double* st = lds + ((size_t)(pg - 1) * kNumSums) * kBlock + ls;
-        st[0] = (double)acc.n;
-        st[kBlock] = acc.a;
-        st[2 * kBlock] = acc.b;
-        st[3 * kBlock] = acc.aa;
-        st[4 * kBlock] = acc.bb;
-        st[5 * kBlock] = acc.ab;
+    struct __align__(16) Sums6 {
+        double v[kNumSums];
+    };
+    Sums6* slab = (Sums6*)lds_raw;
+    const int nl = n_lw * 64;
+    const int ls = lw * 64 + lane;
+    if (dealt && pg > 0) {
+        Sums6 mine = {{(double)acc.n, acc.a, acc.b, acc.aa, acc.bb, acc.ab}};
+        slab[(pg - 1) * nl + ls] = mine;
     }
     __syncthreads();
-    if (pg == 0) {
+    if (threadIdx.x < kBlock && threadIdx.x >= nl) {
+        double* out = a.partials + (size_t)(group - a.group_lo) * kNumSums * a.n_slots + (long long)batch * kBlock + threadIdx.x;
+#pragma unroll
+        for (int k = 0; k < kNumSums; ++k) out[k * a.n_slots] = 0.0;
+    }
+    if (dealt && pg == 0) {
         double sn = (double)acc.n, sa = acc.a, sb = acc.b, saa = acc.aa, sbb = acc.bb, sab = acc.ab;
-        for (int g = 0; g < kPointGroups - 1; ++g) {
-            const double* st = lds + ((size_t)g * kNumSums) * kBlock + ls;
-            sn += st[0];
-            sa += st[kBlock];
-            sb += st[2 * kBlock];
-            saa += st[3 * kBlock];
-            sbb += st[4 * kBlock];
-            sab += st[5 * kBlock];
+#pragma unroll 1
+        for (int g = 0; g < n_pg - 1; ++g) {
+            const Sums6 st = slab[g * nl + ls];
+            sn += st.v[0];
+            sa += st.v[1];
+            sb += st.v[2];
+            saa += st.v[3];
+            sbb += st.v[4];
+            sab += st.v[5];
         }
         double* out = a.partials + (size_t)(group - a.group_lo) * kNumSums * a.n_slots + slot;
         out[0] = sn;
diff --git a/include/coreg_hip.h b/include/coreg_hip.h
--- a/include/coreg_hip.h
+++ b/include/coreg_hip.h
@@ -176,6 +176,10 @@
 int coreg_last_stats(coreg_handle* h, coreg_stats* out);
 
 int coreg_last_visit_counts(coreg_handle* h, int64_t* counts6);
+int coreg_last_plan_counts(coreg_handle* h, int64_t* counts6);
+int coreg_plan_lag_slots(int32_t n_crval1, int32_t n_crval2, int64_t lag_begin, int64_t lag_end, const double* geometry8,
+                         int64_t lds_elems, int64_t cap_slots, int32_t* plan3, int64_t* out_index, int32_t* lag_waves,
+                         int32_t* n_batches);
 int coreg_last_tap_fix(coreg_handle* h, int64_t* counts3);
 
 int coreg_set_option(coreg_handle* h, const char* name, int64_t value);
diff --git a/profiles/small_sweep_timing.py b/profiles/small_sweep_timing.py
--- /dev/null
+++ b/profiles/small_sweep_timing.py
@@ -0,0 +1,38 @@
+#!/usr/bin/env python3
+import json
+import os
+import sys
+import time
+
+import numpy as np
+
+ROOT = os.path.dirname(os.path.dirname(os.path.abspath(__file__)))
+sys.path.insert(0, ROOT)
+from euispice_coreg_amd import _lib, synthetic
+
+small, hs, large, hl, _ = synthetic.make_scene()
+small32, large32 = small.astype(np.float32), large.astype(np.float32)
+grid = _lib.Grid((200, 300), (-20, 20), (2048, 2048))
+h = _lib.CoregHandle(0)
+h.set_small(small32)
+h.prepare_reference_carrington(large32, hl, grid, 1.004, 2)
+
+for n in [int(a) for a in sys.argv[1:]] or (11, 7, 60):
+    ax = 17.0 + 1.0 * (np.arange(n) - n // 2) if n != 60 else np.arange(-30, 30, 1.0)
+    ay = -9.0 + 1.0 * (np.arange(n) - n // 2) if n != 60 else np.arange(-30, 30, 1.0)
+    lags = _lib.LagSet(ax, ay, None, None, None)
+    ks, ws = [], []
+    for it in range(25):
+        t0 = time.perf_counter()
+        out = h.sweep_carrington(hs, grid, 1.004, lags)
+        ws.append(1e3 * (time.perf_counter() - t0))
+        ks.append(h.last_stats()["sweep_kernel_ms"])
+    ks, ws = ks[5:], ws[5:]
+    rec = {"lags": [n, n], "tree": ROOT,
+           "kernel_ms": {"median": float(np.median(ks)), "min": float(min(ks)), "max": float(max(ks))},
+           "call_ms": {"median": float(np.median(ws)), "min": float(min(ws)), "max": float(max(ws))},
+           "argmax": [int(i) for i in np.unravel_index(np.nanargmax(out), (n, n))],
+           "corr_max": float(np.nanmax(out))}
+    if hasattr(h, "last_plan_counts"):
+        rec["plan"] = h.last_plan_counts()
+    print(json.dumps(rec), flush=True)
```

Measured after the change: 1.189 million lag-points/s (median of 6 runs). 2.2% higher.
